# gleb-kov/wordpiece

Hardware: AMD Instinct MI355X
Metric: input MB/s tokenized (bert-base-cased vocab; offline stand-in: synthetic BERT-like vocab) (higher is better)
Workload: dtype int32

## Files before the change

### include/wordpiece_amd.h

```cpp
#ifndef WORDPIECE_AMD_H
#define WORDPIECE_AMD_H

#include <stddef.h>
#include <stdint.h>

#ifdef __cplusplus
extern "C" {
#endif

#define WP_OK 0
#define WP_ERR_EMPTY_WORD 1
#define WP_ERR_TOO_LARGE 2
#define WP_ERR_HIP 3
#define WP_ERR_NO_DEVICE 4
#define WP_ERR_IO 5
#define WP_ERR_ARG 6

typedef struct wp_vocab wp_vocab;

int wp_vocab_create(const char *const *lines, const size_t *line_bytes, size_t n_lines,
                    wp_vocab **out);
int wp_vocab_create_packed(const char *buf, const int64_t *offsets, int64_t n_lines,
                           wp_vocab **out);
int wp_vocab_from_file(const char *vocab_file, wp_vocab **out);
// ... 32 lines not shown
#define WP_TRUNC_ONLY_SECOND 2
typedef struct { int32_t max_len, cls_id, sep_id, pad_id, pairs, truncation, stride, unit; } wp_inputs_spec;
typedef struct { int32_t *input_ids, *token_type_ids, *lengths, *sample; uint32_t *offsets; } wp_inputs;
int wp_linear_encode_inputs(wp_vocab *v, const char *utf8, size_t nbytes, const int64_t *doc_off, size_t n_docs,
                            const wp_inputs_spec *spec, wp_inputs *out, size_t *n_out, size_t *n_samples);
int wp_linear_encode_inputs_device(wp_vocab *v, const void *d_utf8, size_t nbytes, const int64_t *d_doc_off, size_t n_docs,
                                   const wp_inputs_spec *spec, const wp_inputs *d_out, size_t capacity_rows,
                                   size_t *n_out, size_t *n_samples);

typedef struct { int32_t max_len, cls_id, sep_id, pad_id, mask_id, ignore_id, whole_word, reserved;
                 uint64_t select_q32, mask_q32, random_q32, seed, row_base; } wp_mask_spec;
int wp_word_ids(wp_vocab *v, const int32_t *input_ids, const int32_t *lengths, size_t n_rows, const wp_mask_spec *spec,
                int32_t **word_ids);
int wp_word_ids_device(wp_vocab *v, const int32_t *d_input_ids, const int32_t *d_lengths, size_t n_rows,
                       const wp_mask_spec *spec, int32_t *d_word_ids);
int wp_mlm_mask(wp_vocab *v, const int32_t *input_ids, const int32_t *lengths, size_t n_rows, const wp_mask_spec *spec,
                int32_t **masked, int32_t **labels, int32_t **word_ids);
int wp_mlm_mask_device(wp_vocab *v, const int32_t *d_input_ids, const int32_t *d_lengths, size_t n_rows,
                       const wp_mask_spec *spec, int32_t *d_masked, int32_t *d_labels, int32_t *d_word_ids);
typedef struct {
  int64_t n_rows;
  int64_t n_words;
  int64_t n_selected;
  int64_t n_selected_units;
  int64_t n_masked, n_random, n_kept;
  int32_t whole_word, reserved;
} wp_mask_stats;
int wp_get_mask_stats(const wp_vocab *v, wp_mask_stats *out);

typedef struct { int32_t max_len, cleanup, terminator, n_skip; int32_t skip_ids[8]; } wp_detok_spec;
int wp_detokenize(wp_vocab *v, const int32_t *ids, const int64_t *row_splits, const int32_t *lengths, size_t n_rows,
                  const wp_detok_spec *spec, char **text, int64_t **text_off, size_t *n_bytes);
int wp_detokenize_device(wp_vocab *v, const int32_t *d_ids, const int64_t *d_row_splits, const int32_t *d_lengths,
                         size_t n_rows, const wp_detok_spec *spec, const void **d_text, const int64_t **d_text_off,
                         size_t *n_bytes);
int64_t wp_detok_piece(const wp_vocab *v, int64_t id, int form, int cleanup, char *buf, size_t cap);
typedef struct { int64_t n_rows, n_cells, n_kept, n_skipped, n_dropped, n_bytes; } wp_detok_stats;
int wp_get_detok_stats(const wp_vocab *v, wp_detok_stats *out);

int wp_linear_encode_multi(wp_vocab *v, const char *utf8, size_t nbytes, const int *devices,
                           int n_devices, int32_t **ids, size_t *n_ids);

int wp_linear_encode_batch(wp_vocab *v, const char *const *texts, const size_t *nbytes, size_t n_texts,
                           int32_t **ids, size_t *n_ids);

typedef int (*wp_text_source)(void *user, size_t index, const char **utf8, size_t *nbytes);
typedef void (*wp_ids_sink)(void *user, size_t index, const int32_t *ids, size_t n_ids);
int wp_linear_encode_stream(wp_vocab *v, wp_text_source next, wp_ids_sink out, void *user);

int wp_reserve(wp_vocab *v, size_t nbytes);

int wp_trim(wp_vocab *v);

int wp_linear_encode_file(const char *text_file, const char *vocab_file, int32_t **ids,
                          size_t *n_ids);
int wp_linear_encode_external(const char *text_file, const char *vocab_file, const char *out_file,
                              size_t memory_limit);

int wp_fast_encode(wp_vocab *v, const char *utf8, size_t nbytes, int32_t **ids, size_t *n_ids);
int wp_fast_encode_device(wp_vocab *v, const void *d_utf8, size_t nbytes, const int32_t **d_ids,
                          size_t *n_ids);
int wp_fast_encode_file(const char *text_file, const char *vocab_file, int32_t **ids, size_t *n_ids);
int wp_fast_encode_external(const char *text_file, const char *vocab_file, const char *out_file,
                            size_t memory_limit);
int64_t wp_vocab_token_utf8(const wp_vocab *v, int64_t i, char *buf, size_t cap);

#define WP_OPT_FULL_DEPTH 1
#define WP_OPT_DEVICE 2
#define WP_OPT_KEEP_DEBUG 3
#define WP_OPT_STAGE_TIMING 4
#define WP_OPT_LCP_KASAI 5
#define WP_OPT_COVER_ANCHORS 7
#define WP_OPT_ARENA_GUARD 8
#define WP_OPT_DEVICES 9
#define WP_OPT_VOCAB_IN_S 10
#define WP_OPT_SPARSE_EMIT 11
#define WP_OPT_INDEXED_ROUND0 12
#define WP_OPT_SORT_BLANKS 13
#define WP_OPT_NORMALIZE 14
#define WP_NORM_CLEAN 1
#define WP_NORM_LOWER 2
#define WP_NORM_STRIP_ACCENTS 4
#define WP_NORM_BERT_UNCASED 7
int wp_set_option(wp_vocab *v, int option, int64_t value);

int wp_normalize_cp(int flags, uint32_t cp, uint32_t out[3]);
int wp_normalize_device(wp_vocab *v, const void *d_utf8, size_t nbytes, int flags, const void **d_out, size_t *out_bytes);
int wp_normalize(wp_vocab *v, const char *utf8, size_t nbytes, int flags, char **out, size_t *out_bytes);

typedef struct {
  int64_t n_bytes, n_text, n_total, alphabet, longest_token, n_ids;
  int32_t symbol_bits, symbols_per_key, rounds, sorted_depth, full_depth;
  int64_t radix_pass_elems;
  int32_t radix_passes;
  int64_t active_per_round[40];
  double ms_total, ms_decode, ms_sa, ms_lcp, ms_scan, ms_walk;
  double ms_radix_scatter;
  int64_t n_anchors;
  int32_t anchor_mode;
  double ms_h2d, ms_d2h;
  int64_t radix_digit_bytes;
  double ms_host_total;
  int32_t guard_zones;
  int32_t n_devices;
  int32_t vocab_in_s;
  int32_t reserved0;
  int64_t needed_after_round0;
  int32_t key_bits;
  int32_t staged_emit;
  int32_t rank_in_pass;
  int32_t trie_refine;
  int64_t arena_bytes;
  int32_t list_retries;
  int32_t hist_in_keys;
  int64_t radix_pass_bytes;
  int64_t round0_candidates;
  int32_t round0_keys_only;
  int32_t offsets_unit;
  int64_t round0_sorted;
  int64_t n_rows, rows_truncated;
  int32_t rows_route;
} wp_stats;
int wp_get_stats(const wp_vocab *v, wp_stats *out);
typedef struct {
  int32_t normalize;
  int64_t norm_bytes;
  double ms_normalize;
} wp_norm_stats;
int wp_get_norm_stats(const wp_vocab *v, wp_norm_stats *out);
typedef struct {
  int64_t n_wide_words;
  int64_t n_long_words;
  int32_t lean;
  int32_t max_anchor_gap;
} wp_walk_stats;
int wp_get_walk_stats(const wp_vocab *v, wp_walk_stats *out);
typedef struct {
  int64_t n_groups;
  int64_t n_entries;
  int64_t n_large_groups;
  int64_t n_large_entries;
  int64_t trie_nodes;
  int32_t sort_bits;
  int32_t key_lookup;
  int32_t symbol_bytes;
  int32_t reserved;
} wp_refine_stats;
int wp_get_refine_stats(const wp_vocab *v, wp_refine_stats *out);
typedef struct {
  int64_t n_samples, n_out;
  int64_t n_cut;
  int64_t n_windowed;
  int32_t pairs, truncation, stride, reserved;
} wp_inputs_stats;
int wp_get_inputs_stats(const wp_vocab *v, wp_inputs_stats *out);

int wp_linear_debug_fetch(const wp_vocab *v, int which, int32_t *out, size_t capacity,
                          size_t *n_out);

void wp_free(void *p);
const char *wp_last_error(void);
int wp_device_count(void);

#ifdef __cplusplus
}
#endif
#endif
```

### wordpiece_amd/__init__.py

```python
import ctypes as C
import os
import weakref

import numpy as np

_HERE = os.path.dirname(os.path.abspath(__file__))
LIB_PATH = os.environ.get("WP_LIB") or os.path.join(_HERE, "libwordpiece_amd.so")

WP_OPT_FULL_DEPTH, WP_OPT_DEVICE, WP_OPT_KEEP_DEBUG, WP_OPT_STAGE_TIMING, WP_OPT_LCP_KASAI = 1, 2, 3, 4, 5
WP_OPT_COVER_ANCHORS, WP_OPT_ARENA_GUARD, WP_OPT_DEVICES, WP_OPT_VOCAB_IN_S = 7, 8, 9, 10
WP_OPT_SPARSE_EMIT = 11
WP_OPT_INDEXED_ROUND0 = 12
WP_OPT_SORT_BLANKS = 13
WP_OPT_NORMALIZE = 14
WP_NORM_CLEAN, WP_NORM_LOWER, WP_NORM_STRIP_ACCENTS, WP_NORM_BERT_UNCASED = 1, 2, 4, 7
WP_OFFSETS_BYTES, WP_OFFSETS_CODE_POINTS = 0, 1
_OFFSET_UNITS = {"byte": WP_OFFSETS_BYTES, "char": WP_OFFSETS_CODE_POINTS}
WP_TRUNC_LONGEST_FIRST, WP_TRUNC_ONLY_FIRST, WP_TRUNC_ONLY_SECOND = 0, 1, 2
_TRUNCATIONS = {"longest_first": WP_TRUNC_LONGEST_FIRST, "only_first": WP_TRUNC_ONLY_FIRST,
                "only_second": WP_TRUNC_ONLY_SECOND}

ABI_SYMBOLS = [
    "wp_vocab_create", "wp_vocab_create_packed", "wp_vocab_from_file", "wp_vocab_destroy", "wp_vocab_size",
    "wp_vocab_unk_id", "wp_vocab_token_flags", "wp_vocab_token_len", "wp_linear_encode",
    "wp_linear_encode_device", "wp_linear_encode_file", "wp_linear_encode_external", "wp_set_option",
    "wp_get_stats", "wp_linear_debug_fetch", "wp_free", "wp_last_error", "wp_device_count",
    "wp_linear_encode_multi", "wp_reserve", "wp_fast_encode", "wp_fast_encode_device", "wp_fast_encode_file",
    "wp_fast_encode_external", "wp_vocab_token_utf8", "wp_trim", "wp_linear_encode_batch", "wp_linear_encode_stream",
    "wp_linear_encode_offsets", "wp_linear_encode_offsets_device",
    "wp_linear_encode_rows", "wp_linear_encode_rows_device", "wp_linear_encode_padded", "wp_linear_encode_padded_device",
    "wp_normalize_cp", "wp_normalize_device", "wp_normalize", "wp_get_norm_stats", "wp_get_walk_stats",
    "wp_get_refine_stats",
    "wp_linear_encode_inputs", "wp_linear_encode_inputs_device", "wp_get_inputs_stats",
    "wp_word_ids", "wp_word_ids_device", "wp_mlm_mask", "wp_mlm_mask_device", "wp_get_mask_stats",
    "wp_detokenize", "wp_detokenize_device", "wp_detok_piece", "wp_get_detok_stats",
]


class WordPieceError(RuntimeError):
    """Mirrors the std::runtime_error the reference throws (message = wp_last_error())."""


class Stats(C.Structure):
    _fields_ = [("n_bytes", C.c_int64), ("n_text", C.c_int64), ("n_total", C.c_int64), ("alphabet", C.c_int64),
                ("longest_token", C.c_int64), ("n_ids", C.c_int64),
                ("symbol_bits", C.c_int32), ("symbols_per_key", C.c_int32), ("rounds", C.c_int32),
                ("sorted_depth", C.c_int32), ("full_depth", C.c_int32),
                ("radix_pass_elems", C.c_int64), ("radix_passes", C.c_int32),
                ("active_per_round", C.c_int64 * 40),
                ("ms_total", C.c_double), ("ms_decode", C.c_double), ("ms_sa", C.c_double), ("ms_lcp", C.c_double),
                ("ms_scan", C.c_double), ("ms_walk", C.c_double), ("ms_radix_scatter", C.c_double),
                ("n_anchors", C.c_int64), ("anchor_mode", C.c_int32), ("ms_h2d", C.c_double), ("ms_d2h", C.c_double),
                ("radix_digit_bytes", C.c_int64), ("ms_host_total", C.c_double), ("guard_zones", C.c_int32),
                ("n_devices", C.c_int32), ("vocab_in_s", C.c_int32), ("reserved0", C.c_int32),
                ("needed_after_round0", C.c_int64), ("key_bits", C.c_int32), ("staged_emit", C.c_int32),
                ("rank_in_pass", C.c_int32), ("trie_refine", C.c_int32), ("arena_bytes", C.c_int64),
                ("list_retries", C.c_int32), ("hist_in_keys", C.c_int32), ("radix_pass_bytes", C.c_int64),
                ("round0_candidates", C.c_int64), ("round0_keys_only", C.c_int32), ("offsets_unit", C.c_int32),
                ("round0_sorted", C.c_int64), ("n_rows", C.c_int64), ("rows_truncated", C.c_int64),
                ("rows_route", C.c_int32)]

    def as_dict(self):
        d = {k: getattr(self, k) for k, _ in self._fields_ if k != "active_per_round"}
        d["active_per_round"] = [int(x) for x in self.active_per_round[:max(self.rounds, 0)]]
        return d


class NormStats(C.Structure):
    _fields_ = [("normalize", C.c_int32), ("norm_bytes", C.c_int64), ("ms_normalize", C.c_double)]


class WalkStats(C.Structure):
    _fields_ = [("n_wide_words", C.c_int64), ("n_long_words", C.c_int64), ("lean", C.c_int32),
                ("max_anchor_gap", C.c_int32)]


class RefineStats(C.Structure):
    _fields_ = [("n_groups", C.c_int64), ("n_entries", C.c_int64), ("n_large_groups", C.c_int64),
                ("n_large_entries", C.c_int64), ("trie_nodes", C.c_int64), ("sort_bits", C.c_int32),
                ("key_lookup", C.c_int32), ("symbol_bytes", C.c_int32), ("reserved", C.c_int32)]


class InputsSpec(C.Structure):
    _fields_ = [("max_len", C.c_int32), ("cls_id", C.c_int32), ("sep_id", C.c_int32), ("pad_id", C.c_int32),
                ("pairs", C.c_int32), ("truncation", C.c_int32), ("stride", C.c_int32), ("unit", C.c_int32)]


class Inputs(C.Structure):
    _fields_ = [("input_ids", C.c_void_p), ("token_type_ids", C.c_void_p), ("lengths", C.c_void_p), ("sample", C.c_void_p),
                ("offsets", C.c_void_p)]


class InputsStats(C.Structure):
    _fields_ = [("n_samples", C.c_int64), ("n_out", C.c_int64), ("n_cut", C.c_int64), ("n_windowed", C.c_int64),
                ("pairs", C.c_int32), ("truncation", C.c_int32), ("stride", C.c_int32), ("reserved", C.c_int32)]


class MaskSpec(C.Structure):
    _fields_ = [("max_len", C.c_int32), ("cls_id", C.c_int32), ("sep_id", C.c_int32), ("pad_id", C.c_int32),
                ("mask_id", C.c_int32), ("ignore_id", C.c_int32), ("whole_word", C.c_int32), ("reserved", C.c_int32),
                ("select_q32", C.c_uint64), ("mask_q32", C.c_uint64), ("random_q32", C.c_uint64), ("seed", C.c_uint64),
                ("row_base", C.c_uint64)]


class MaskStats(C.Structure):
    _fields_ = [("n_rows", C.c_int64), ("n_words", C.c_int64), ("n_selected", C.c_int64), ("n_selected_units", C.c_int64),
                ("n_masked", C.c_int64), ("n_random", C.c_int64), ("n_kept", C.c_int64), ("whole_word", C.c_int32),
                ("reserved", C.c_int32)]


class DetokSpec(C.Structure):
    _fields_ = [("max_len", C.c_int32), ("cleanup", C.c_int32), ("terminator", C.c_int32), ("n_skip", C.c_int32),
                ("skip_ids", C.c_int32 * 8)]


class DetokStats(C.Structure):
    _fields_ = [("n_rows", C.c_int64), ("n_cells", C.c_int64), ("n_kept", C.c_int64), ("n_skipped", C.c_int64),
                ("n_dropped", C.c_int64), ("n_bytes", C.c_int64)]


_TEXT_SOURCE = C.CFUNCTYPE(C.c_int, C.c_void_p, C.c_size_t, C.POINTER(C.c_void_p), C.POINTER(C.c_size_t))
_IDS_SINK = C.CFUNCTYPE(None, C.c_void_p, C.c_size_t, C.POINTER(C.c_int32), C.c_size_t)

_lib = None


def lib():
    global _lib
    if _lib is None:
        if not os.path.exists(LIB_PATH):
            raise WordPieceError("HIP extension missing: %s (run `python -m wordpiece_amd.build`)" % LIB_PATH)
        L = C.CDLL(LIB_PATH)
        vp, i32p = C.c_void_p, C.POINTER(C.c_int32)
        L.wp_vocab_create.argtypes = [C.POINTER(C.c_char_p), C.POINTER(C.c_size_t), C.c_size_t, C.POINTER(vp)]
        L.wp_vocab_create_packed.argtypes = [C.c_char_p, C.POINTER(C.c_int64), C.c_int64, C.POINTER(vp)]
        L.wp_vocab_from_file.argtypes = [C.c_char_p, C.POINTER(vp)]
        L.wp_vocab_destroy.argtypes = [vp]
        L.wp_vocab_destroy.restype = None
        L.wp_vocab_size.argtypes = [vp]
        L.wp_vocab_size.restype = C.c_int64
        L.wp_vocab_unk_id.argtypes = [vp]
        L.wp_vocab_unk_id.restype = C.c_int32
        L.wp_vocab_token_flags.argtypes = [vp, C.c_int64]
        L.wp_vocab_token_flags.restype = C.c_int32
        L.wp_vocab_token_len.argtypes = [vp, C.c_int64]
        L.wp_vocab_token_len.restype = C.c_int64
        L.wp_linear_encode.argtypes = [vp, C.c_char_p, C.c_size_t, C.POINTER(i32p), C.POINTER(C.c_size_t)]
        L.wp_linear_encode_device.argtypes = [vp, vp, C.c_size_t, C.POINTER(vp), C.POINTER(C.c_size_t)]
        u32p = C.POINTER(C.c_uint32)
        L.wp_linear_encode_offsets.argtypes = [vp, C.c_char_p, C.c_size_t, C.c_int, C.POINTER(i32p), C.POINTER(u32p),
                                               C.POINTER(C.c_size_t)]
        L.wp_linear_encode_offsets_device.argtypes = [vp, vp, C.c_size_t, C.c_int, C.POINTER(vp), C.POINTER(vp),
                                                      C.POINTER(C.c_size_t)]
        i64p = C.POINTER(C.c_int64)
        L.wp_linear_encode_rows.argtypes = [vp, C.c_char_p, C.c_size_t, i64p, C.c_size_t, C.c_int, C.POINTER(i32p),
                                            C.POINTER(i64p), C.POINTER(u32p), C.POINTER(C.c_size_t), C.POINTER(C.c_size_t)]
        L.wp_linear_encode_rows_device.argtypes = [vp, vp, C.c_size_t, vp, C.c_size_t, C.c_int, C.POINTER(vp), C.POINTER(vp),
                                                   C.POINTER(vp), C.POINTER(C.c_size_t), C.POINTER(C.c_size_t)]
        L.wp_linear_encode_padded.argtypes = [vp, C.c_char_p, C.c_size_t, i64p, C.c_size_t, C.c_int, C.c_int32, C.c_int32,
                                              C.c_int32, C.POINTER(i32p), C.POINTER(i32p), C.POINTER(C.c_size_t)]
        L.wp_linear_encode_padded_device.argtypes = [vp, vp, C.c_size_t, vp, C.c_size_t, C.c_int, C.c_int32, C.c_int32,
                                                     C.c_int32, vp, vp, C.c_size_t, C.POINTER(C.c_size_t)]
        L.wp_linear_encode_inputs.argtypes = [vp, C.c_char_p, C.c_size_t, i64p, C.c_size_t, C.POINTER(InputsSpec),
                                              C.POINTER(Inputs), C.POINTER(C.c_size_t), C.POINTER(C.c_size_t)]
        L.wp_linear_encode_inputs_device.argtypes = [vp, vp, C.c_size_t, vp, C.c_size_t, C.POINTER(InputsSpec),
                                                     C.POINTER(Inputs), C.c_size_t, C.POINTER(C.c_size_t),
                                                     C.POINTER(C.c_size_t)]
        L.wp_get_inputs_stats.argtypes = [vp, C.POINTER(InputsStats)]
        L.wp_word_ids.argtypes = [vp, i32p, i32p, C.c_size_t, C.POINTER(MaskSpec), C.POINTER(i32p)]
        L.wp_word_ids_device.argtypes = [vp, vp, vp, C.c_size_t, C.POINTER(MaskSpec), vp]
        L.wp_mlm_mask.argtypes = [vp, i32p, i32p, C.c_size_t, C.POINTER(MaskSpec), C.POINTER(i32p), C.POINTER(i32p),
                                  C.POINTER(i32p)]
        L.wp_mlm_mask_device.argtypes = [vp, vp, vp, C.c_size_t, C.POINTER(MaskSpec), vp, vp, vp]
        L.wp_get_mask_stats.argtypes = [vp, C.POINTER(MaskStats)]
        L.wp_detokenize.argtypes = [vp, i32p, C.POINTER(C.c_int64), i32p, C.c_size_t, C.POINTER(DetokSpec),
                                    C.POINTER(C.c_void_p), C.POINTER(C.POINTER(C.c_int64)), C.POINTER(C.c_size_t)]
        L.wp_detokenize_device.argtypes = [vp, vp, vp, vp, C.c_size_t, C.POINTER(DetokSpec), C.POINTER(C.c_void_p),
                                           C.POINTER(C.c_void_p), C.POINTER(C.c_size_t)]
        L.wp_detok_piece.argtypes = [vp, C.c_int64, C.c_int, C.c_int, C.c_char_p, C.c_size_t]
        L.wp_detok_piece.restype = C.c_int64
        L.wp_get_detok_stats.argtypes = [vp, C.POINTER(DetokStats)]
        L.wp_linear_encode_multi.argtypes = [vp, C.c_char_p, C.c_size_t, C.POINTER(C.c_int), C.c_int, C.POINTER(i32p),
                                             C.POINTER(C.c_size_t)]
        L.wp_reserve.argtypes = [vp, C.c_size_t]
        L.wp_linear_encode_stream.argtypes = [vp, _TEXT_SOURCE, _IDS_SINK, vp]
        L.wp_linear_encode_batch.argtypes = [vp, C.POINTER(C.c_char_p), C.POINTER(C.c_size_t), C.c_size_t, C.POINTER(i32p),
                                             C.POINTER(C.c_size_t)]
        L.wp_trim.argtypes = [vp]
        L.wp_fast_encode.argtypes = [vp, C.c_char_p, C.c_size_t, C.POINTER(i32p), C.POINTER(C.c_size_t)]
        L.wp_fast_encode_device.argtypes = [vp, vp, C.c_size_t, C.POINTER(vp), C.POINTER(C.c_size_t)]
        L.wp_fast_encode_file.argtypes = [C.c_char_p, C.c_char_p, C.POINTER(i32p), C.POINTER(C.c_size_t)]
        L.wp_fast_encode_external.argtypes = [C.c_char_p, C.c_char_p, C.c_char_p, C.c_size_t]
        L.wp_vocab_token_utf8.argtypes = [vp, C.c_int64, C.c_char_p, C.c_size_t]
        L.wp_vocab_token_utf8.restype = C.c_int64
        L.wp_linear_encode_file.argtypes = [C.c_char_p, C.c_char_p, C.POINTER(i32p), C.POINTER(C.c_size_t)]
        L.wp_linear_encode_external.argtypes = [C.c_char_p, C.c_char_p, C.c_char_p, C.c_size_t]
        L.wp_normalize_cp.argtypes = [C.c_int, C.c_uint32, C.POINTER(C.c_uint32)]
        L.wp_normalize_device.argtypes = [vp, vp, C.c_size_t, C.c_int, C.POINTER(vp), C.POINTER(C.c_size_t)]
        L.wp_normalize.argtypes = [vp, C.c_char_p, C.c_size_t, C.c_int, C.POINTER(vp), C.POINTER(C.c_size_t)]
        L.wp_set_option.argtypes = [vp, C.c_int, C.c_int64]
        L.wp_get_stats.argtypes = [vp, C.POINTER(Stats)]
        L.wp_get_norm_stats.argtypes = [vp, C.POINTER(NormStats)]
        L.wp_get_walk_stats.argtypes = [vp, C.POINTER(WalkStats)]
        L.wp_get_refine_stats.argtypes = [vp, C.POINTER(RefineStats)]
        L.wp_linear_debug_fetch.argtypes = [vp, C.c_int, i32p, C.c_size_t, C.POINTER(C.c_size_t)]
        L.wp_free.argtypes = [vp]
        L.wp_free.restype = None
        L.wp_last_error.restype = C.c_char_p
        L.wp_device_count.restype = C.c_int
        _lib = L
    return _lib


def _check(rc):
    if rc != 0:
        raise WordPieceError(lib().wp_last_error().decode("utf8", "replace"))


def _bytes(x):
    return bytes(x) if isinstance(x, (bytes, bytearray, memoryview)) else x.encode("utf8")


class Vocab:

    def __init__(self, lines=None, file=None, device=None, normalize=0):
        self._h = C.c_void_p()
        if file is not None:
            _check(lib().wp_vocab_from_file(_bytes(file), C.byref(self._h)))
        else:
            ls = [_bytes(w) for w in lines]
            off = np.zeros(len(ls) + 1, dtype=np.int64)
            if ls:
                off[1:] = np.cumsum([len(w) for w in ls])
            _check(lib().wp_vocab_create_packed(b"".join(ls), off.ctypes.data_as(C.POINTER(C.c_int64)), len(ls),
                                                C.byref(self._h)))
        self._device = None if device is None else int(device)
        if device is not None:
            self.set_option(WP_OPT_DEVICE, device)
        if normalize:
            self.set_option(WP_OPT_NORMALIZE, normalize)
        self._normalize = int(normalize)

    def __del__(self):
        if getattr(self, "_h", None) and _lib is not None:
            _lib.wp_vocab_destroy(self._h)
            self._h = None

    def __len__(self):
        return lib().wp_vocab_size(self._h)

    @property
    def unk_id(self):
        return lib().wp_vocab_unk_id(self._h)

    def token_flags(self, i):
        return lib().wp_vocab_token_flags(self._h, i)

    def token_len(self, i):
        return lib().wp_vocab_token_len(self._h, i)

    def set_option(self, opt, value):
        _check(lib().wp_set_option(self._h, opt, int(value)))
        if opt == WP_OPT_NORMALIZE:
            self._normalize = int(value)
        if opt == WP_OPT_DEVICE:
            self._device = int(value)

    def normalize(self, text, flags=None):
        b = _bytes(text)
        out = C.c_void_p()
        n = C.c_size_t()
        _check(lib().wp_normalize(self._h, b, len(b), self._normalize if flags is None else int(flags), C.byref(out), C.byref(n)))
        if n.value == 0:
            return b""
        try:
            return C.string_at(out, n.value)
        finally:
            lib().wp_free(out)

    def normalize_tensor(self, text, flags=None, copy=True):
        import torch
        if text.dtype != torch.uint8 or not text.is_cuda or not text.is_contiguous():
            raise WordPieceError("normalize_tensor needs a contiguous uint8 CUDA/HIP tensor")
        nbytes = text.numel()
        if text.data_ptr() % 4 != 0 or nbytes % 4 != 0:
            padded = torch.zeros((nbytes + 19) // 16 * 16, dtype=torch.uint8, device=text.device)
            padded[:nbytes] = text
            text = padded
        torch.cuda.current_stream(text.device).synchronize()
        d_out = C.c_void_p()
        n = C.c_size_t()
        _check(lib().wp_normalize_device(self._h, C.c_void_p(text.data_ptr()), nbytes,
                                         self._normalize if flags is None else int(flags), C.byref(d_out), C.byref(n)))
        if n.value == 0:
            return torch.zeros(0, dtype=torch.uint8, device=text.device)
        view = torch.as_tensor(DeviceIds(d_out.value, n.value, typestr="|u1"), device=text.device)
        return view.clone() if copy else view

    def stats(self):
        s = Stats()
        _check(lib().wp_get_stats(self._h, C.byref(s)))
        d = s.as_dict()
        ns = NormStats()
        _check(lib().wp_get_norm_stats(self._h, C.byref(ns)))
        d.update({k: getattr(ns, k) for k, _ in ns._fields_})
        return d

    def walk_stats(self):
        ws = WalkStats()
        _check(lib().wp_get_walk_stats(self._h, C.byref(ws)))
        return {k: int(getattr(ws, k)) for k, _ in ws._fields_}

    def refine_stats(self):
        rs = RefineStats()
        _check(lib().wp_get_refine_stats(self._h, C.byref(rs)))
        return {k: int(getattr(rs, k)) for k, _ in rs._fields_ if k != "reserved"}

    def encode(self, text):
        b = _bytes(text)
        ids = C.POINTER(C.c_int32)()
        n = C.c_size_t()
        _check(lib().wp_linear_encode(self._h, b, len(b), C.byref(ids), C.byref(n)))
        return _adopt_ids(ids, n.value)

    def encode_with_offsets(self, text, unit="byte"):
        b = _bytes(text)
        ids = C.POINTER(C.c_int32)()
        offs = C.POINTER(C.c_uint32)()
        n = C.c_size_t()
        _check(lib().wp_linear_encode_offsets(self._h, b, len(b), _offset_unit(unit), C.byref(ids), C.byref(offs),
                                              C.byref(n)))
        if n.value == 0:
            return np.zeros(0, dtype=np.int32), np.zeros((0, 2), dtype=np.uint32)
        return _adopt_ids(ids, n.value), _adopt_block(offs, (n.value, 2))

    def encode_device_with_offsets(self, d_ptr, nbytes, unit="byte"):
        d_ids = C.c_void_p()
        d_offs = C.c_void_p()
        n = C.c_size_t()
        _check(lib().wp_linear_encode_offsets_device(self._h, C.c_void_p(d_ptr), nbytes, _offset_unit(unit), C.byref(d_ids),
                                                     C.byref(d_offs), C.byref(n)))
        return d_ids.value, d_offs.value, n.value

    def encode_rows(self, docs=None, text=None, doc_offsets=None, offsets=None):
        b, off = _docs_arg(docs, text, doc_offsets)
        unit = -1 if offsets is None else _offset_unit(offsets)
        ids, splits, offs = C.POINTER(C.c_int32)(), C.POINTER(C.c_int64)(), C.POINTER(C.c_uint32)()
        n, rows = C.c_size_t(), C.c_size_t()
        _check(lib().wp_linear_encode_rows(self._h, b, len(b), _i64_ptr(off), 0 if off is None else len(off) - 1, unit,
                                           C.byref(ids), C.byref(splits), C.byref(offs), C.byref(n), C.byref(rows)))
        out = (_adopt_ids(ids, n.value), _adopt_block(splits, (rows.value + 1,)))
        if offsets is None:
            return out
        return out + (_adopt_block(offs, (n.value, 2)) if n.value else np.zeros((0, 2), dtype=np.uint32),)

    def encode_padded(self, docs=None, text=None, doc_offsets=None, max_len=128, cls_id=None, sep_id=None, pad_id=0):
        b, off = _docs_arg(docs, text, doc_offsets)
        ids, lens = C.POINTER(C.c_int32)(), C.POINTER(C.c_int32)()
        rows = C.c_size_t()
        _check(lib().wp_linear_encode_padded(self._h, b, len(b), _i64_ptr(off), 0 if off is None else len(off) - 1,
                                             int(max_len), _special(cls_id), _special(sep_id), int(pad_id), C.byref(ids),
                                             C.byref(lens), C.byref(rows)))
        if rows.value == 0:
            return np.zeros((0, int(max_len)), dtype=np.int32), np.zeros(0, dtype=np.int32)
        return _adopt_block(ids, (rows.value, int(max_len))), _adopt_block(lens, (rows.value,))

    def _rows_tensor_args(self, text, doc_offsets):
        import torch
        if text.dtype != torch.uint8 or not text.is_cuda or not text.is_contiguous():
            raise WordPieceError("a documents call on tensors needs a contiguous uint8 CUDA/HIP text tensor")
        nbytes = text.numel()
        if text.data_ptr() % 4 != 0 or nbytes % 4 != 0:
            padded = torch.zeros((nbytes + 19) // 16 * 16, dtype=torch.uint8, device=text.device)
            padded[:nbytes] = text
            text = padded
        if doc_offsets is not None:
            if doc_offsets.dtype != torch.int64 or doc_offsets.device != text.device or doc_offsets.dim() != 1 or \
                    doc_offsets.numel() < 1:
                raise WordPieceError("doc_offsets must be a 1-d int64 tensor on the text's device")
            doc_offsets = doc_offsets.contiguous()
        torch.cuda.current_stream(text.device).synchronize()
        return text, nbytes, doc_offsets

    def encode_rows_tensor(self, text, doc_offsets=None, offsets=None, copy=True):
        import torch
        text, nbytes, doc_offsets = self._rows_tensor_args(text, doc_offsets)
        unit = -1 if offsets is None else _offset_unit(offsets)
        d_ids, d_splits, d_offs = C.c_void_p(), C.c_void_p(), C.c_void_p()
        n, rows = C.c_size_t(), C.c_size_t()
        _check(lib().wp_linear_encode_rows_device(
            self._h, C.c_void_p(text.data_ptr()), nbytes, None if doc_offsets is None else C.c_void_p(doc_offsets.data_ptr()),
            0 if doc_offsets is None else doc_offsets.numel() - 1, unit, C.byref(d_ids), C.byref(d_splits), C.byref(d_offs),
            C.byref(n), C.byref(rows)))
        dev = text.device
        ids = torch.as_tensor(DeviceIds(d_ids.value, n.value), device=dev) if n.value else \
            torch.zeros(0, dtype=torch.int32, device=dev)
        splits = torch.as_tensor(DeviceIds(d_splits.value, rows.value + 1, typestr="<i8"), device=dev)
        out = (ids, splits)
        if offsets is not None:
# ... 579 lines not shown
```

### wordpiece_amd/csrc/context.h

```cpp
#pragma once
#include <array>
#include <cstring>
#include <memory>
#include <mutex>
#include <string>
#include <vector>

#include "../../include/wordpiece_amd.h"
#include "code.h"
#include "decode.h"
#include "detok.h"
#include "radix_sort.h"
#include "scanline.h"
#include "suffix_array.h"
#include "vocab.h"

namespace wp {

static thread_local std::string g_last_error;

struct EnvOptions {
  bool arena_guard;
  bool vocab_in_s;
  bool sparse_emit;
// ... 44 lines not shown
__global__ __launch_bounds__(kBlock) void guard_check_kernel(const char *base, const unsigned long long *offs, int count,
                                                             uint32_t *bad) {
  const int z = blockIdx.x;
  if (z >= count) return;
  const uint32_t *g = reinterpret_cast<const uint32_t *>(base + offs[z]);
  const bool broken = threadIdx.x < kGuardBytes / 4 && g[threadIdx.x] != kGuardWord;
  if (__syncthreads_or(broken) && threadIdx.x == 0) {
    atomicAdd(&bad[0], 1u);
    atomicMin(&bad[1], static_cast<uint32_t>(z) + 1u);
  }
}

struct Arena {
  DeviceBuffer *buf;
  size_t off = 0, planned = 0;
  bool planning = true, guard = false;
  std::vector<unsigned long long> zones;
  explicit Arena(DeviceBuffer *b, bool g = false) : buf(b), guard(g) {}
  template <typename T>
  T *take(size_t count) {
    size_t bytes = (count * sizeof(T) + 255) & ~static_cast<size_t>(255);
    size_t o = off;
    off += bytes;
    if (guard) {
      if (!planning) zones.push_back(off);
      off += kGuardBytes;
    }
    if (planning) return nullptr;
    if (off > planned) throw std::logic_error("arena: the allocation sequence differs from the planned one");
    return reinterpret_cast<T *>(static_cast<char *>(buf->p) + o);
  }
  void commit() {
    buf->ensure(off + (guard ? 8 * 512 : 0));
    planned = off;
    off = 0;
    planning = false;
  }
  unsigned long long *zone_table() const {
    return reinterpret_cast<unsigned long long *>(static_cast<char *>(buf->p) + ((off + 255) & ~static_cast<size_t>(255)));
  }
  void arm(hipStream_t st) {
    if (!guard || zones.empty()) return;
    if (zones.size() > 500) throw std::logic_error("arena guard: too many allocations");
    WP_HIP(hipMemcpyAsync(zone_table(), zones.data(), zones.size() * sizeof(unsigned long long), hipMemcpyHostToDevice, st));
    WP_HIP(hipStreamSynchronize(st));
    hipLaunchKernelGGL(guard_fill_kernel, dim3(zones.size()), dim3(kBlock), 0, st, static_cast<char *>(buf->p), zone_table(),
                       static_cast<int>(zones.size()));
  }
  void check(hipStream_t st, uint32_t *bad) const {
    if (!guard || zones.empty()) return;
    hipLaunchKernelGGL(guard_check_kernel, dim3(zones.size()), dim3(kBlock), 0, st, static_cast<const char *>(buf->p),
                       zone_table(), static_cast<int>(zones.size()), bad);
  }
};

static int bit_length(uint64_t v) {
  int b = 0;
  while (v) {
    b++;
    v >>= 1;
  }
  return b;
}

constexpr int kScalars = 56;
constexpr int kScalarCps = 0;
constexpr int kScalarAlphabet = 1;
constexpr int kScalarInvalid = 2;
constexpr int kScalarList = 4;
constexpr int kScalarListEntries = kScalarList + 0;
constexpr int kScalarListGroups = kScalarList + 1;
constexpr int kScalarListLargeGroups = kScalarList + 2;
constexpr int kScalarListLargeEntries = kScalarList + 3;
constexpr int kScalarListWanted = 8;
constexpr int kScalarIds = 9;
constexpr int kScalarAnchors = 10;
constexpr int kScalarAnchorGap = 11;
constexpr int kScalarLongWords = 12;
constexpr int kScalarWideWords = 13;
constexpr int kScalarCps64 = 14;
constexpr int kScalarGuard = 16;
constexpr int kScalarGuardBad = kScalarGuard + 0;
constexpr int kScalarGuardFirst = kScalarGuard + 1;
constexpr int kScalarFree18 = 18;
constexpr int kScalarAlphaWord0 = 20;
constexpr int kScalarRows = 21, kScalarRowsBad = 22, kScalarRowsCut = 23;
constexpr int kScalarCand = 24;
constexpr int kScalarKept = 25;
constexpr int kScalarSrcRows = 26;
constexpr int kScalarInCut = 27, kScalarInRows = 28, kScalarInWindowed = 30;
constexpr int kScalarFree31 = 31;
constexpr int kScalarMask = 32;
constexpr int kScalarDetokLast = 44, kScalarDetokBad = 46;
constexpr int kScalarFree47 = 47;
constexpr int kScalarDetok = 48;
constexpr int kScalarNormBytes = kScalarCps;
constexpr int kScalarNormCps = kScalarAlphabet;
constexpr int kScalarNormSrcCps = kScalarListEntries;
constexpr int kScalarNormBytes64 = kScalarCps64;

struct ScalarRange {
  int first, words;
};
constexpr ScalarRange kScalarLayout[] = {
    {kScalarCps, 1},         {kScalarAlphabet, 1},   {kScalarInvalid, 2},         {kScalarListEntries, 1},
    {kScalarListGroups, 1},  {kScalarListLargeGroups, 1}, {kScalarListLargeEntries, 1}, {kScalarListWanted, 1},
    {kScalarIds, 1},         {kScalarAnchors, 1},    {kScalarAnchorGap, 1},       {kScalarLongWords, 1},
    {kScalarWideWords, 1},   {kScalarCps64, 2},      {kScalarGuardBad, 1},        {kScalarGuardFirst, 1},
    {kScalarFree18, 2},      {kScalarAlphaWord0, 1}, {kScalarRows, 1},            {kScalarRowsBad, 1},
    {kScalarRowsCut, 1},     {kScalarCand, 1},       {kScalarKept, 1},            {kScalarSrcRows, 1},
    {kScalarInCut, 1},       {kScalarInRows, 2},     {kScalarInWindowed, 1},      {kScalarFree31, 1},
    {kScalarMask, 12},       {kScalarDetokLast, 2},  {kScalarDetokBad, 1},        {kScalarFree47, 1},
    {kScalarDetok, 8}};
constexpr int scalar_end(int slot) {
  for (const ScalarRange &r : kScalarLayout) {
    if (slot < r.first + r.words) return r.first + r.words;
  }
  return kScalars;
}
constexpr bool scalar_layout_ok() {
  int at = 0;
  for (const ScalarRange &r : kScalarLayout) {
    if (r.first != at || r.words < 1 || (r.words % 2 == 0 && r.first % 2 != 0)) return false;
    at += r.words;
  }
  return at == kScalars;
}
static_assert(scalar_layout_ok(), "the scalar table must cover d_scalars word by word, 64-bit slots on even words");
static_assert(kScalarList % 2 == 0 && kScalarListLargeGroups % 2 == 0, "both halves of the list block are also read as 64-bit words");

struct RowsCall {
  const long long *d_doc_off = nullptr;
  size_t n_docs = 0;
  int unit = -1;
  size_t capacity = SIZE_MAX;
  size_t n_rows = 0;
  const long long *d_starts = nullptr;
  const long long *d_row_splits = nullptr;
  uint32_t *d_line_cnt = nullptr;
};

enum SideEvent { kEvFork, kEvJoin, kEvScalars, kEvKeysFree, kEvPartition, kEvTrieNodes, kEvLargeSorted, kEvKeysBuilt, kEvCandCount,
                 kEvSpine, kEvKept, kSideEvents };
enum TimingMark { kMarkStart, kMarkCounted, kMarkSymbols, kMarkSorted, kMarkLcp, kMarkScanned, kMarkWalked, kMarkNormStart,
                  kTimingMarks, kMarkNormEnd = kMarkStart };

struct Context {
  int device = 0;
  hipStream_t stream = nullptr;
  hipStream_t stream2 = nullptr;
  hipStream_t stream3 = nullptr;
  hipEvent_t evs[kSideEvents] = {};
  uint32_t *d_stream = nullptr, *d_elig_start = nullptr, *d_elig_info = nullptr, *d_soft = nullptr;
  uint32_t *d_vocab_word_idx = nullptr, *d_vocab_word_bits = nullptr;
  uint8_t *d_cls_bmp = nullptr;
  uint32_t *d_lt_chain_len = nullptr, *d_lt_chain_off = nullptr, *d_lt_child_begin = nullptr, *d_lt_child_cp = nullptr,
           *d_lt_child_node = nullptr, *d_elig_node = nullptr, *d_elig_subtree = nullptr;
  int32_t *d_elig_id = nullptr, *d_tok_len = nullptr;
  uint8_t *d_tok_class = nullptr;
  DetokRec *d_detok_rec = nullptr;
  uint8_t *d_detok_pool = nullptr;
  size_t detok_pool_bytes = 0;
  unsigned long long *d_trie_key = nullptr;
  uint32_t *d_trie_child = nullptr;
  int32_t *d_trie_id = nullptr;
  DeviceBuffer text_buf, a_buf, b_buf, fmt_buf;
  DeviceBuffer text_buf2, ids_stage[2];
  DeviceBuffer rows_in, rows_out, pad_buf;
  DeviceBuffer inputs_buf;
  DeviceBuffer detok_in, detok_aux, detok_out;
  uint16_t *d_norm_index = nullptr;
  uint32_t *d_norm_pages = nullptr, *d_norm_pool = nullptr;
  DeviceBuffer norm_buf, norm_aux, norm_map;
  hipStream_t up_stream = nullptr, down_stream = nullptr;
  hipEvent_t pipe_ev[4] = {};
  uint32_t *d_used = nullptr, *d_lut = nullptr, *d_scan_tmp = nullptr;
  uint32_t *d_scalars = nullptr;
  uint8_t *d_code = nullptr;
  size_t list_hint = 0;
  SymbolCode code_cache;
  bool code_cached = false;
  uint32_t code_alphabet = 0;
  int code_bits = 0, code_lo = 0, code_uses = 0;
  double code_blank_share = 0.0;
  uint8_t *h_code = nullptr;
  uint32_t *d_symhist = nullptr;
  uint32_t *h_scalars = nullptr;
  RadixStats rstats;
  hipEvent_t ev[kTimingMarks] = {};
  const int32_t *d_ids = nullptr;
  const uint32_t *d_offs = nullptr;
  struct {
    const void *sym = nullptr;
    int sym_bytes = 0;
    const uint32_t *sa = nullptr, *cps = nullptr;
    const RankEntry *rank = nullptr;
    const int32_t *lcp = nullptr;
    const uint8_t *cls = nullptr;
    StepTable steps{};
    int32_t *best_scratch = nullptr;
    size_t n = 0, n_text = 0;
  } dbg;
  std::array<DeviceBuffer *, 17> buffers() {
    return {&text_buf, &a_buf,    &b_buf,   &fmt_buf,    &text_buf2, &ids_stage[0], &ids_stage[1], &rows_in,   &rows_out,
            &pad_buf,  &inputs_buf, &norm_buf, &norm_aux, &norm_map, &detok_in,     &detok_aux,    &detok_out};
  }
  Context() = default;
  Context(const Context &) = delete;
  Context &operator=(const Context &) = delete;
  ~Context();
};

struct DeviceGuard {
  int prev = -1;
  DeviceGuard() {
    if (hipGetDevice(&prev) != hipSuccess) prev = -1;
  }
  ~DeviceGuard() {
    if (prev >= 0) (void)hipSetDevice(prev);
  }
  DeviceGuard(const DeviceGuard &) = delete;
  DeviceGuard &operator=(const DeviceGuard &) = delete;
};

#ifdef WP_DEBUG_BOUNDS
static void take_oob(int first, int count, unsigned int *oob) {
  WP_HIP(hipMemcpyFromSymbol(oob, HIP_SYMBOL(g_wp_oob), count * sizeof(unsigned int), first * sizeof(unsigned int)));
  bool any = false;
  for (int i = 0; i < count; i++) any = any || oob[i] != 0;
  if (!any) return;
  const unsigned int zero[kBoundSites] = {};
  WP_HIP(hipMemcpyToSymbol(HIP_SYMBOL(g_wp_oob), zero, count * sizeof(unsigned int), first * sizeof(unsigned int)));
}
#endif

}

using namespace wp;

struct EncodeStats : wp_stats {
  int32_t normalize;
  int64_t norm_bytes;
  double ms_normalize;
  wp_walk_stats walk;
  wp_refine_stats refine;
  wp_inputs_stats inputs;
  int32_t inputs_call;
  wp_mask_stats mask;
  int32_t mask_call;
  wp_detok_stats detok;
  int32_t detok_call;
};

struct wp_vocab {
  HostVocab hv;
  std::unique_ptr<Context> ctx;
  std::vector<std::unique_ptr<Context>> multi;
  int device = -1;
  bool full_depth = false, keep_debug = false, stage_timing = false, lcp_kasai = false, cover_anchors = false;
  bool arena_guard = false;
  bool sparse_emit = false;
  bool vocab_in_s = false;
  bool indexed_round0 = false;
  bool sort_blanks = false;
  int normalize = 0;
  int n_devices = 1;
  EncodeStats stats{};
  ~wp_vocab();
};

namespace wp {

template <typename... T>
static void free_dev(T *&...p) {
  (((p ? (void)hipFree(p) : (void)0), p = nullptr), ...);
}

static void free_vocab_tables(Context *c) {
  free_dev(c->d_stream, c->d_elig_start, c->d_elig_info, c->d_soft, c->d_elig_id, c->d_tok_len, c->d_tok_class, c->d_detok_rec, c->d_detok_pool, c->d_trie_key,
           c->d_trie_child, c->d_trie_id, c->d_vocab_word_idx, c->d_vocab_word_bits, c->d_cls_bmp, c->d_lt_chain_len,
           c->d_lt_chain_off, c->d_lt_child_begin, c->d_lt_child_cp, c->d_lt_child_node, c->d_elig_node, c->d_elig_subtree);
}

template <size_t N>
static void destroy_events(hipEvent_t (&events)[N]) {
  for (auto &e : events) {
    if (e) (void)hipEventDestroy(e);
    e = nullptr;
  }
}

static void destroy_context(Context *c) {
  if (!c) return;
  bool owns = c->stream || c->stream2 || c->stream3 || c->d_used || c->d_lut || c->d_scan_tmp || c->d_scalars || c->d_code ||
              c->d_symhist || c->h_scalars || c->h_code || c->d_stream;
  for (DeviceBuffer *b : c->buffers()) owns = owns || b->p;
  if (!owns) return;
  DeviceGuard keep;
  (void)hipSetDevice(c->device);
  free_vocab_tables(c);
  free_dev(c->d_used, c->d_lut, c->d_scan_tmp, c->d_scalars, c->d_code, c->d_symhist, c->d_norm_index, c->d_norm_pages, c->d_norm_pool);
  if (c->h_scalars) (void)hipHostFree(c->h_scalars);
  if (c->h_code) (void)hipHostFree(c->h_code);
  c->h_scalars = nullptr;
  c->h_code = nullptr;
  for (DeviceBuffer *b : c->buffers()) b->release();
  destroy_events(c->pipe_ev);
  destroy_events(c->ev);
  destroy_events(c->evs);
  for (hipStream_t *s : {&c->up_stream, &c->down_stream, &c->stream3, &c->stream2, &c->stream}) {
    if (*s) (void)hipStreamDestroy(*s);
    *s = nullptr;
  }
}
Context::~Context() { destroy_context(this); }

template <typename T>
static T *upload(const std::vector<T> &v, hipStream_t st) {
  T *d = nullptr;
  WP_HIP(hipMalloc(&d, std::max<size_t>(v.size(), 1) * sizeof(T)));
  if (!v.empty()) WP_HIP(hipMemcpyAsync(d, v.data(), v.size() * sizeof(T), hipMemcpyHostToDevice, st));
  return d;
}

static constexpr size_t kPoolArenaBytes = size_t(256) << 20;
static constexpr size_t kPoolContexts = 4;
static std::mutex g_pool_mu;
static std::vector<std::unique_ptr<Context>> &context_pool() {
  static auto *pool = new std::vector<std::unique_ptr<Context>>();
  return *pool;
}

static void release_arenas(Context *c) {
  for (DeviceBuffer *b : c->buffers()) b->release();
  c->d_ids = nullptr;
  c->d_offs = nullptr;
  c->dbg = {};
}

static void park_context(std::unique_ptr<Context> c) {
  if (!c) return;
  const bool no_pool = EnvOptions::get().no_pool;
  DeviceGuard keep;
  (void)hipSetDevice(c->device);
  if (!no_pool && hipStreamSynchronize(c->stream) == hipSuccess && hipStreamSynchronize(c->stream2) == hipSuccess &&
      hipStreamSynchronize(c->stream3) == hipSuccess) {
    free_vocab_tables(c.get());
// ... 112 lines not shown
```

### wordpiece_amd/csrc/encoder.hip

```cpp
#include <fcntl.h>
#include <sys/mman.h>
#include <sys/stat.h>
#include <unistd.h>

#include <atomic>
#include <chrono>
#include <cstring>
#include <fstream>
#include <functional>
#include <future>
#include <memory>
#include <mutex>
#include <thread>
#include <unordered_map>
#include <vector>

#include "../../include/wordpiece_amd.h"
#include "context.h"
#include "detok.h"
#include "fast_path.h"
#include "format.h"
#include "inputs.h"
#include "linear_path.h"
#include "mask.h"
// ... 51 lines not shown
  }
  try {
  std::unique_ptr<wp_vocab> v(new wp_vocab());
  if (const char *e = getenv("WP_DEVICES")) {
    v->n_devices = std::strcmp(e, "all") == 0 ? -1 : std::max(1, atoi(e));
  }
  std::string err = v->hv.build(lines);
  if (!err.empty()) {
    g_last_error = err;
    return WP_ERR_EMPTY_WORD;
  }
  *out = v.release();
  return WP_OK;
  } catch (const std::exception &e) {
    g_last_error = e.what();
    return WP_ERR_ARG;
  } catch (...) {
    g_last_error = "unknown exception while building the vocabulary";
    return WP_ERR_ARG;
  }
}

extern "C" {

int wp_vocab_create(const char *const *lines, const size_t *line_bytes, size_t n_lines, wp_vocab **out) {
  std::vector<std::pair<const char *, size_t>> ls;
  ls.reserve(n_lines);
  for (size_t i = 0; i < n_lines; i++) ls.emplace_back(lines[i], line_bytes[i]);
  return vocab_from_lines(ls, out);
}

int wp_vocab_create_packed(const char *buf, const int64_t *offsets, int64_t n_lines, wp_vocab **out) {
  std::vector<std::pair<const char *, size_t>> ls;
  ls.reserve(static_cast<size_t>(n_lines));
  for (int64_t i = 0; i < n_lines; i++) ls.emplace_back(buf + offsets[i], static_cast<size_t>(offsets[i + 1] - offsets[i]));
  return vocab_from_lines(ls, out);
}

int wp_vocab_from_file(const char *vocab_file, wp_vocab **out) {
  std::ifstream fin(vocab_file);
  std::vector<std::string> words;
  std::string w;
  while (std::getline(fin, w)) words.push_back(w);
  std::vector<std::pair<const char *, size_t>> ls;
  for (auto &s : words) ls.emplace_back(s.data(), s.size());
  return vocab_from_lines(ls, out);
}

void wp_vocab_destroy(wp_vocab *v) {
  if (!v) return;
  try {
    delete v;
  } catch (...) {
  }
}
int64_t wp_vocab_size(const wp_vocab *v) { return static_cast<int64_t>(v->hv.tokens.size()); }
int32_t wp_vocab_unk_id(const wp_vocab *v) { return v->hv.unk_id; }
int32_t wp_vocab_token_flags(const wp_vocab *v, int64_t i) {
  return token_flags(v->hv.tokens[static_cast<size_t>(i)]);
}
int64_t wp_vocab_token_len(const wp_vocab *v, int64_t i) {
  return static_cast<int64_t>(v->hv.tokens[static_cast<size_t>(i)].word.size());
}

int wp_set_option(wp_vocab *v, int option, int64_t value) {
  switch (option) {
    case WP_OPT_FULL_DEPTH: v->full_depth = value != 0; return WP_OK;
    case WP_OPT_DEVICE:
      if (v->ctx) {
        g_last_error = "device already bound";
        return WP_ERR_ARG;
      }
      v->device = static_cast<int>(value);
      return WP_OK;
    case WP_OPT_KEEP_DEBUG: v->keep_debug = value != 0; return WP_OK;
    case WP_OPT_STAGE_TIMING: v->stage_timing = value != 0; return WP_OK;
    case WP_OPT_LCP_KASAI: v->lcp_kasai = value != 0; return WP_OK;
    case WP_OPT_COVER_ANCHORS: v->cover_anchors = value != 0; return WP_OK;
    case WP_OPT_ARENA_GUARD: v->arena_guard = value != 0; return WP_OK;
    case WP_OPT_VOCAB_IN_S: v->vocab_in_s = value != 0; return WP_OK;
    case WP_OPT_SPARSE_EMIT: v->sparse_emit = value != 0; return WP_OK;
    case WP_OPT_INDEXED_ROUND0: v->indexed_round0 = value != 0; return WP_OK;
    case WP_OPT_SORT_BLANKS: v->sort_blanks = value != 0; return WP_OK;
    case WP_OPT_NORMALIZE:
      if (!known_norm_flags(value)) {
        g_last_error = "WP_OPT_NORMALIZE: unknown flag bits (WP_NORM_CLEAN | WP_NORM_LOWER | WP_NORM_STRIP_ACCENTS)";
        return WP_ERR_ARG;
      }
      v->normalize = static_cast<int>(value);
      return WP_OK;
    case WP_OPT_DEVICES: v->n_devices = value < 0 ? -1 : static_cast<int>(std::max<int64_t>(value, 1)); return WP_OK;
  }
  g_last_error = "unknown option";
  return WP_ERR_ARG;
}

int wp_normalize_cp(int flags, uint32_t cp, uint32_t out[3]) {
  if (!known_norm_flags(flags) || cp >= 0x110000u || (cp >= 0xd800u && cp < 0xe000u)) return -1;
  uint32_t o[3] = {0, 0, 0};
  const int n = norm_cp(host_norm_tables(), flags, cp, o);
  for (int i = 0; i < n; i++) out[i] = o[i];
  return n;
}

int wp_normalize_device(wp_vocab *v, const void *d_utf8, size_t nbytes, int flags, const void **d_out, size_t *out_bytes) {
  return guarded([&] {
    *d_out = nullptr;
    *out_bytes = 0;
    if (!known_norm_flags(flags)) throw std::invalid_argument("normalize: unknown flag bits");
    if (nbytes == 0) return;
    check_device_text(d_utf8);
    Context *c = get_context(v);
    NormResult r;
    normalize_on_device(c, static_cast<const uint8_t *>(d_utf8), nbytes, flags, false, false, r);
    WP_HIP(hipStreamSynchronize(c->stream));
    *d_out = r.nbytes ? r.text : nullptr;
    *out_bytes = r.nbytes;
  });
}

int wp_get_stats(const wp_vocab *v, wp_stats *out) {
  *out = v->stats;
  return WP_OK;
}

int wp_get_norm_stats(const wp_vocab *v, wp_norm_stats *out) {
  out->normalize = v->stats.normalize;
  out->norm_bytes = v->stats.norm_bytes;
  out->ms_normalize = v->stats.ms_normalize;
  return WP_OK;
}

int wp_get_walk_stats(const wp_vocab *v, wp_walk_stats *out) {
  *out = v->stats.walk;
  return WP_OK;
}

int wp_get_refine_stats(const wp_vocab *v, wp_refine_stats *out) {
  *out = v->stats.refine;
  return WP_OK;
}

int wp_get_inputs_stats(const wp_vocab *v, wp_inputs_stats *out) {
  *out = v->stats.inputs;
  if (!v->stats.inputs_call) out->n_out = -1;
  return WP_OK;
}

int wp_linear_encode_device(wp_vocab *v, const void *d_utf8, size_t nbytes, const int32_t **d_ids, size_t *n_ids) {
  return guarded([&] {
    check_device_text(d_utf8);
    size_t n = 0;
    Context *c = get_context(v);
    encode_on_device(v, c, static_cast<const uint8_t *>(d_utf8), nbytes, &n, v->stats);
    v->stats.n_devices = 1;
    *d_ids = n ? c->d_ids : nullptr;
    *n_ids = n;
  });
}

}

namespace {
struct PinnedPool {
  std::mutex mu;
  std::unordered_map<void *, size_t> owned;
  std::vector<std::pair<size_t, void *>> pooled;
  static constexpr size_t kMaxPooledBlocks = 4;
  static constexpr size_t kMaxPooledBytes = size_t(6) << 30;
  void *take(size_t bytes) {
    {
      std::lock_guard<std::mutex> g(mu);
      size_t best = pooled.size();
      for (size_t i = 0; i < pooled.size(); i++) {
        if (pooled[i].first >= bytes && (best == pooled.size() || pooled[i].first < pooled[best].first)) best = i;
      }
      if (best != pooled.size()) {
        void *p = pooled[best].second;
        pooled.erase(pooled.begin() + static_cast<long>(best));
        return p;
      }
    }
    void *p = nullptr;
    const size_t want = bytes + bytes / 8 + 4096;
    WP_HIP(hipHostMalloc(&p, want));
    std::lock_guard<std::mutex> g(mu);
    owned[p] = want;
    return p;
  }
  bool give_back(void *p) {
    size_t cap = 0;
    {
      std::lock_guard<std::mutex> g(mu);
      auto it = owned.find(p);
      if (it == owned.end()) return false;
      cap = it->second;
      size_t bytes = cap;
      for (auto &b : pooled) bytes += b.first;
      if (pooled.size() < kMaxPooledBlocks && bytes <= kMaxPooledBytes) {
        pooled.emplace_back(cap, p);
        return true;
      }
      owned.erase(it);
    }
    (void)hipHostFree(p);
    return true;
  }
  void trim() {
    std::vector<std::pair<size_t, void *>> drop;
    {
      std::lock_guard<std::mutex> g(mu);
      drop.swap(pooled);
      for (auto &b : drop) owned.erase(b.second);
    }
    for (auto &b : drop) (void)hipHostFree(b.second);
  }
};
PinnedPool &id_pool() {
  static PinnedPool *pool = new PinnedPool();
  return *pool;
}
struct PinnedBlock {
// ... 1346 lines not shown
  }
  DeviceBuffer *tb[2] = {&c->text_buf, &c->text_buf2};
  const int device = c->device;
  std::atomic<long long> up_us{0};
  auto upload = [&](const char *text, size_t len, int slot) -> std::string {
    try {
      if (len == 0) return "";
      const auto t_up = wp_clock::now();
      WP_HIP(hipSetDevice(device));
      upload_text(*tb[slot], c->up_stream, text, len);
      WP_HIP(hipStreamSynchronize(c->up_stream));
      up_us += static_cast<long long>(ms_since(t_up) * 1e3);
      return "";
    } catch (const std::exception &e) {
      return e.what()[0] ? e.what() : "upload failed";
    }
  };
  EncodeStats total{};
  const char *cur_text = nullptr, *next_text = nullptr;
  size_t cur_len = 0, next_len = 0;
  bool have = next(0, &cur_text, &cur_len);
  if (have) {
    tb[0]->ensure(text_room(cur_len));
    const std::string err = upload(cur_text, cur_len, 0);
    if (!err.empty()) throw HipError(err);
  }
  std::unique_ptr<PinnedBlock> in_flight;
  size_t in_flight_n = 0, in_flight_i = 0;
  int in_flight_slot = 0;
  for (size_t i = 0; have; i++) {
    const int slot = static_cast<int>(i & 1);
    const bool more = next(i + 1, &next_text, &next_len);
    std::future<std::string> next_up;
    if (more) {
      tb[slot ^ 1]->ensure(text_room(next_len));
      next_up = std::async(std::launch::async, upload, next_text, next_len, slot ^ 1);
    }
    struct Wait {
      std::future<std::string> &f;
      ~Wait() {
        if (f.valid()) f.wait();
      }
    } wait_up{next_up};
    size_t n = 0;
    EncodeStats st{};
    if (cur_len) encode_on_device(v, c, static_cast<const uint8_t *>(tb[slot]->p), cur_len, &n, st);
    std::unique_ptr<PinnedBlock> blk(new PinnedBlock(std::max<size_t>(n, 1) * sizeof(int32_t)));
    if (n) {
      c->ids_stage[slot].ensure(n * sizeof(int32_t));
      WP_HIP(hipMemcpyAsync(c->ids_stage[slot].p, c->d_ids, n * sizeof(int32_t), hipMemcpyDeviceToDevice, c->stream));
      WP_HIP(hipEventRecord(c->pipe_ev[slot], c->stream));
      WP_HIP(hipStreamWaitEvent(c->down_stream, c->pipe_ev[slot], 0));
      WP_HIP(hipMemcpyAsync(blk->p, c->ids_stage[slot].p, n * sizeof(int32_t), hipMemcpyDeviceToHost, c->down_stream));
      WP_HIP(hipEventRecord(c->pipe_ev[2 + slot], c->down_stream));
    }
    if (in_flight) {
      if (in_flight_n) WP_HIP(hipEventSynchronize(c->pipe_ev[2 + in_flight_slot]));
      deliver(in_flight_i, *in_flight, in_flight_n);
    }
    in_flight = std::move(blk);
    in_flight_n = n;
    in_flight_i = i;
    in_flight_slot = slot;
    total.n_bytes += st.n_bytes;
    total.n_text += st.n_text;
    total.n_total += st.n_total;
    total.n_ids += st.n_ids;
    total.ms_total += st.ms_total;
    total.normalize = std::max(total.normalize, st.normalize);
    total.norm_bytes += st.norm_bytes;
    total.ms_normalize += st.ms_normalize;
    total.walk.n_wide_words += st.walk.n_wide_words;
    total.walk.n_long_words += st.walk.n_long_words;
    total.walk.max_anchor_gap = std::max(total.walk.max_anchor_gap, st.walk.max_anchor_gap);
    if (i == 0) total.walk.lean = st.walk.lean;
    {
      const wp_refine_stats sum = total.refine;
      if (i == 0) total.refine = st.refine;
      total.refine.n_groups = sum.n_groups + st.refine.n_groups;
      total.refine.n_entries = sum.n_entries + st.refine.n_entries;
      total.refine.n_large_groups = sum.n_large_groups + st.refine.n_large_groups;
      total.refine.n_large_entries = sum.n_large_entries + st.refine.n_large_entries;
    }
    total.rounds = std::max(total.rounds, st.rounds);
    if (next_up.valid()) {
      const std::string err = next_up.get();
      if (!err.empty()) throw HipError(err);
    }
    have = more;
    cur_text = next_text;
    cur_len = next_len;
  }
  if (in_flight) {
    if (in_flight_n) WP_HIP(hipEventSynchronize(c->pipe_ev[2 + in_flight_slot]));
    deliver(in_flight_i, *in_flight, in_flight_n);
  }
  v->stats = total;
  v->stats.n_devices = 1;
  v->stats.ms_h2d = static_cast<double>(up_us.load()) / 1e3;
  v->stats.ms_host_total = ms_since(t_all);
}
}

extern "C" {

int wp_linear_encode_batch(wp_vocab *v, const char *const *texts, const size_t *nbytes, size_t n_texts, int32_t **ids,
                           size_t *n_ids) {
  return guarded([&] {
    for (size_t i = 0; i < n_texts; i++) {
      ids[i] = nullptr;
      n_ids[i] = 0;
    }
    std::vector<void *> got(n_texts, nullptr);
    try {
      encode_pipeline(
          v,
          [&](size_t i, const char **t, size_t *len) {
            if (i >= n_texts) return false;
            *t = texts[i];
            *len = nbytes[i];
            return true;
          },
          [&](size_t i, PinnedBlock &blk, size_t n) {
            n_ids[i] = n;
            if (n) got[i] = blk.release();
          });
    } catch (...) {
      for (void *p : got) {
        if (p) id_pool().give_back(p);
      }
      for (size_t i = 0; i < n_texts; i++) n_ids[i] = 0;
      throw;
    }
    for (size_t i = 0; i < n_texts; i++) ids[i] = static_cast<int32_t *>(got[i]);
  });
}

int wp_linear_encode_stream(wp_vocab *v, wp_text_source next, wp_ids_sink out, void *user) {
  return guarded([&] {
    if (!next || !out) throw std::invalid_argument("wp_linear_encode_stream: null callback");
    encode_pipeline(
        v, [&](size_t i, const char **t, size_t *len) { return next(user, i, t, len) != 0; },
        [&](size_t i, PinnedBlock &blk, size_t n) { out(user, i, n ? static_cast<const int32_t *>(blk.p) : nullptr, n); });
  });
}

int wp_trim(wp_vocab *v) {
  return guarded([&] {
    auto drop = [](Context *c) {
      if (!c) return;
      WP_HIP(hipSetDevice(c->device));
      WP_HIP(hipStreamSynchronize(c->stream));
      WP_HIP(hipStreamSynchronize(c->stream2));
      release_arenas(c);
    };
    if (v) {
      drop(v->ctx.get());
      for (auto &c : v->multi) drop(c.get());
    }
    {
      std::lock_guard<std::mutex> g(g_pool_mu);
      for (auto &c : context_pool()) drop(c.get());
    }
    id_pool().trim();
  });
}
// ... 294 lines not shown
```

### wordpiece_amd/csrc/linear_path.h

```cpp
#pragma once
#include <functional>

#include "context.h"
#include "local_sort.h"
#include "prune.h"
#include "trie.h"
#include "offsets.h"
#include "normalize.h"
#include "rows.h"
#include "walk.h"

namespace wp {

struct ListOverflow {
  size_t wanted;
};

__global__ void needed_list_clamp_kernel(uint32_t *__restrict__ totals, uint32_t cap, uint32_t *__restrict__ wanted) {
  if (totals[0] > cap) {
    *wanted = totals[0];
    totals[0] = 0;
    totals[1] = 0;
  }
}

constexpr double kBlankDropMinShare = 1.0 / 16;

#ifdef WP_DEBUG_BOUNDS
__device__ unsigned int g_wp_sorted_sig[6];
__global__ __launch_bounds__(kBlock) void sorted_check_kernel(const uint32_t *__restrict__ sorted, size_t n_sorted,
                                                              const uint32_t *__restrict__ unsorted, size_t n,
                                                              const uint8_t *__restrict__ cls, size_t n_text,
                                                              const uint32_t *__restrict__ blank_bits) {
  __shared__ uint32_t acc[7];
  if (threadIdx.x < 7) acc[threadIdx.x] = 0u;
  __syncthreads();
  uint32_t bad = 0, cnt[2] = {0, 0}, sum[2] = {0, 0}, x[2] = {0, 0};
  const size_t first = static_cast<size_t>(blockIdx.x) * kBlock + threadIdx.x, stride = static_cast<size_t>(gridDim.x) * kBlock;
  for (size_t i = first; i < n_sorted; i += stride) {
    const uint32_t k = sorted[i];
    if (i + 1 < n_sorted && k > sorted[i + 1]) bad++;
    if (blank_bits && key_is_blank(blank_bits, k)) bad++;
    cnt[0]++;
    sum[0] += k;
    x[0] ^= k;
  }
  for (size_t i = first; i < n; i += stride) {
    if (blank_bits && i < n_text && (cls[i] & kClsSpace)) continue;
    const uint32_t k = unsorted[i];
    cnt[1]++;
    sum[1] += k;
    x[1] ^= k;
  }
  if (bad) atomicAdd(&acc[6], bad);
  for (int s = 0; s < 2; s++) {
    if (cnt[s]) {
      atomicAdd(&acc[3 * s], cnt[s]);
      atomicAdd(&acc[3 * s + 1], sum[s]);
      atomicXor(&acc[3 * s + 2], x[s]);
    }
  }
  __syncthreads();
  if (threadIdx.x < 6 && acc[threadIdx.x]) {
    if (threadIdx.x % 3 == 2) {
      atomicXor(&g_wp_sorted_sig[threadIdx.x], acc[threadIdx.x]);
    } else {
      atomicAdd(&g_wp_sorted_sig[threadIdx.x], acc[threadIdx.x]);
    }
  }
  if (threadIdx.x == 6 && acc[6]) atomicAdd(&g_wp_oob[kSiteSortOrder], acc[6]);
}
__global__ void sorted_check_close_kernel() {
  bool same = true;
  for (int j = 0; j < 3; j++) same = same && g_wp_sorted_sig[j] == g_wp_sorted_sig[3 + j];
  wp_in_bounds(same, kSiteSortOrder);
  for (int j = 0; j < 6; j++) g_wp_sorted_sig[j] = 0u;
}
#endif

template <typename SymT>
struct LinearPath {
  const wp_vocab *v;
  Context *c;
  EncodeStats &S;
  Arena &ar, &aa;
  const uint8_t *d_text;
  size_t nbytes;
  const uint32_t *d_tile_prefix;
  size_t n_text, n;
  uint32_t *d_cps;
  uint8_t *d_cls;
  int bits;
  bool text_only;
  int offs_unit;
  RowsCall *rows;
  const NormMap *nmap;

  hipStream_t st, st2;
  const HostVocab &hv;
  bool full, prune, use_trie, key_lookup, keys_only, window_store, use_digit_bytes, staged_possible, sparse_emit;
  bool wide_ran = false;
  uint32_t need_depth;
  int M, P, P_cap, bucket_shift, bucket_shift_all, key_shift, key_shift_all, hb_n, win_mid;
  unsigned sl_tiles, sl_groups, nbuckets, nbuckets_all, nkbuckets, nkbuckets_all;
  size_t radix_words, emit_tiles, walk_blocks, claim_size, list_cap;

  SymT *d_sym = nullptr, *d_vsym = nullptr;
  Key0 *KA = nullptr, *KB = nullptr;
  uint32_t *VA = nullptr, *VB = nullptr;
  uint32_t *X0 = nullptr, *X1 = nullptr;
  uint8_t *DG0 = nullptr, *DG1 = nullptr;
  RankEntry *d_rank = nullptr;
  uint32_t *d_node_of_slot = nullptr;
  int32_t *d_lcp = nullptr;
  uint32_t *d_sa = nullptr, *d_gdepth = nullptr;
  RankEntry *d_hd_n = nullptr;
  int32_t *d_emit = nullptr, *d_dbg_best = nullptr;
  uint32_t *d_anchors = nullptr, *d_anchor_cnt = nullptr, *d_anchor_tmp = nullptr, *d_emit_cnt = nullptr, *d_emit_tmp = nullptr,
           *d_blk_cnt = nullptr, *d_blk_off = nullptr, *d_tile_scratch = nullptr;
  uint32_t *AS0 = nullptr, *AS1 = nullptr, *AG = nullptr, *AD0 = nullptr, *AD1 = nullptr, *LA = nullptr, *LB = nullptr, *d_tdep = nullptr;
  uint64_t *LK0 = nullptr, *LK1 = nullptr, *LK2 = nullptr;
  uint32_t *LV0 = nullptr, *LV1 = nullptr, *LPOS = nullptr;
  uint32_t *d_ghead = nullptr, *d_gneed0 = nullptr, *d_gneed1 = nullptr, *d_lg_head = nullptr, *d_lg_off = nullptr;
  RerankAgg *d_agg = nullptr, *d_chunk_agg = nullptr;
  uint32_t *d_claim = nullptr, *d_claim_need = nullptr, *d_gclaim = nullptr, *d_gfirst = nullptr, *d_gdep = nullptr, *d_gnode = nullptr,
           *d_gdone = nullptr, *d_rng_lo = nullptr, *d_rng_hi = nullptr, *d_child_sym = nullptr, *d_radix_tmp = nullptr,
           *d_radix_tmp2 = nullptr;
  uint8_t *d_rng_long = nullptr;
  uint32_t *d_mslot0 = nullptr, *d_mslot1 = nullptr, *d_midx0 = nullptr, *d_midx1 = nullptr, *d_minfo = nullptr, *d_tile_mlo = nullptr;
  int32_t *d_mid = nullptr, *d_rf = nullptr, *d_rb = nullptr, *d_cover_f = nullptr, *d_cover_b = nullptr;
  int32_t *d_tmin_f = nullptr, *d_tmin_b = nullptr, *d_gmin_f = nullptr, *d_gmin_b = nullptr, *d_pval_p = nullptr, *d_pval_s = nullptr;
  uint32_t *d_ps0 = nullptr, *d_ps1 = nullptr, *d_pv0 = nullptr, *d_pv1 = nullptr, *d_bidx = nullptr;
  int2 *d_bfast = nullptr, *d_bfast_all = nullptr;
  uint32_t *d_bidx_all = nullptr;
  uint32_t *d_gend = nullptr, *d_kstart = nullptr, *d_kbidx = nullptr, *d_kbidx_all = nullptr;
  int32_t *d_kval_p = nullptr, *d_kval_s = nullptr;
  int2 *d_kbfast = nullptr, *d_kbfast_all = nullptr;
  unsigned long long *d_cand_table = nullptr;
  uint32_t *d_cand_filter = nullptr, *d_cand_lo = nullptr, *d_cand_hi = nullptr, *d_gcand = nullptr;
  uint32_t *d_cand_bcnt = nullptr, *d_cand_boff = nullptr, *d_cand_scan = nullptr;
  int cand_bits = 0;
  uint32_t *d_blank_bits = nullptr;
  uint2 *d_ospill = nullptr, *d_cspan = nullptr, *d_offs = nullptr;
  uint32_t *d_byte_of = nullptr;
  long long *d_line_starts = nullptr, *d_row_splits = nullptr;
  uint32_t *d_row_base = nullptr;

  SymbolCode code;
  DevCode dcode{};
  DigitBytes db;
  RadixPlan sort_plan;
  bool hist_in_keys = false;
  bool drop_blanks = false;
  size_t n_sorted = 0;
  int cur = 0, rounds = 1;
  Key0 *keys = nullptr, *other_keys = nullptr;
  uint32_t *vals = nullptr, *other_vals = nullptr, *slots = nullptr, *other_slots = nullptr, *adep = nullptr, *other_dep = nullptr;
  uint32_t *avals = nullptr, *spare_vals = nullptr;
  bool classified = false, anchors_queued = false;
  size_t n_act = 0, n_large = 0, n_large_groups = 0, n_groups = 0;
  StepTable steps{}, steps_all{};
  StepTable ksteps{}, ksteps_all{};
  CandSet cand{};
  CandRuns cand_runs{};
  size_t n_cand = 0;

  LinearPath(const wp_vocab *v_, Context *c_, EncodeStats &S_, Arena &ar_, Arena &aa_, const uint8_t *text, size_t nb,
             const uint32_t *tile_prefix, size_t n_text_, size_t n_, uint32_t *cps, uint8_t *cls, int bits_, bool text_only_,
             int offs_unit_, RowsCall *rows_ = nullptr, const NormMap *nmap_ = nullptr)
      : v(v_), c(c_), S(S_), ar(ar_), aa(aa_), d_text(text), nbytes(nb), d_tile_prefix(tile_prefix), n_text(n_text_), n(n_),
        d_cps(cps), d_cls(cls), bits(bits_), text_only(text_only_), offs_unit(offs_unit_), rows(rows_), nmap(nmap_), st(c_->stream), st2(c_->stream2),
        hv(v_->hv) {
    full = v->full_depth || hv.n_dup_eligible > 0 || v->lcp_kasai;
    need_depth = static_cast<uint32_t>(std::min<int64_t>(hv.longest + 1, 0x7fffffff));
    M = static_cast<int>(hv.elig_id.size());
    prune = !full && (M > 0 || text_only);
    use_trie = text_only && !full && M > 0;
    key_lookup = use_trie && !v->keep_debug && kKeyBits <= 32;
    keys_only = key_lookup && !v->indexed_round0 && sizeof(SymT) == 1;
    sl_tiles = cdiv(n, kSlTile);
    sl_groups = cdiv(sl_tiles, kSlGroup);
    P = kStepsPerMark * M + 1;
    P_cap = P + 2 * M + 2;
    const int bucket_bits = std::min(kStepBucketBitsMax, std::max(kStepBucketBits, bit_length(4 * static_cast<size_t>(P))));
    bucket_shift = std::max(0, bit_length(n) - bucket_bits);
    nbuckets = static_cast<unsigned>(((n - 1) >> bucket_shift) + 1);
    bucket_shift_all = std::max(0, bit_length(n) - kStepBucketBits);
    nbuckets_all = static_cast<unsigned>(((n - 1) >> bucket_shift_all) + 1);
    const int kb = std::min(kKeyBits, std::max(1, bit_length(n - 1) - bucket_shift));
    const int kb_all = std::min(kKeyBits, std::max(1, bit_length(n - 1) - bucket_shift_all));
    key_shift = kKeyBits - kb;
    key_shift_all = kKeyBits - kb_all;
    nkbuckets = 1u << kb;
    nkbuckets_all = 1u << kb_all;
    radix_words = std::max(radix_tmp_words<uint64_t>(n), radix_tmp_words<uint32_t>(std::max<size_t>(n, static_cast<size_t>(P_cap))));
    emit_tiles = cdiv(std::max<size_t>(n_text, 1), kScanTile);
    walk_blocks = cdiv(std::max<size_t>(n_text, 1), kBlock);
    sparse_emit = v->sparse_emit || EnvOptions::get().sparse_emit;
    staged_possible = !sparse_emit && !v->cover_anchors && hv.soft.empty();
    use_digit_bytes = n > kRadixSmallN;
    claim_size = 1024;
    while (claim_size < 2 * static_cast<size_t>(std::max(M, 1))) claim_size *= 2;
    cand_bits = bit_length(claim_size - 1);
    hb_n = bit_length(n - 1);
    window_store = n >= (1u << 22);
    win_mid = hb_n - kWinBits <= kRadixBits ? hb_n : kWinBits + (hb_n - kWinBits + 1) / 2;
    if (!prune) {
      list_cap = n;
    } else {
      const size_t guess = c->list_hint ? c->list_hint : n / 8;
      list_cap = std::min(n, guess + guess / 4 + 65536);
    }
    S.symbol_bits = bits;
    S.full_depth = full;
    S.trie_refine = use_trie ? 1 : 0;
    S.key_bits = kKeyBits;
    S.round0_keys_only = keys_only ? 1 : 0;
    S.round0_candidates = keys_only ? 0 : -1;
    n_sorted = n;
    S.round0_sorted = static_cast<int64_t>(n);
  }

  void fork() {
    WP_HIP(hipEventRecord(c->evs[kEvFork], st));
    WP_HIP(hipStreamWaitEvent(st2, c->evs[kEvFork], 0));
  }
  void join() {
    WP_HIP(hipEventRecord(c->evs[kEvJoin], st2));
    WP_HIP(hipStreamWaitEvent(st, c->evs[kEvJoin], 0));
  }

  void plan() {
    const bool ref = !text_only;
    const bool want_lcp = ref || v->keep_debug;
    const size_t lc = list_cap, lg = lc / 2 + static_cast<size_t>(M) + 8;
    const size_t rr_tiles_l = cdiv(lc, kRrTile);
    const size_t rtiles = cdiv(std::max<size_t>(n_text, 1), kReachTile);
    for (int pass = 0; pass < 2; pass++) {
      d_sym = ar.take<SymT>(n + 16);
      KA = ar.take<Key0>(n + 16);
      KB = ar.take<Key0>(n + 16);
      VA = ar.take<uint32_t>(n + 16);
      VB = ar.take<uint32_t>(n + 16);
      X0 = ar.take<uint32_t>(n + 16);
      X1 = ar.take<uint32_t>(n + 16);
      DG0 = use_digit_bytes ? ar.take<uint8_t>(n + 64) : nullptr;
      DG1 = use_digit_bytes ? ar.take<uint8_t>(n + 64) : nullptr;
      d_rank = ar.take<RankEntry>(n);
      d_node_of_slot = use_trie ? ar.take<uint32_t>(n) : nullptr;
      d_lcp = want_lcp ? ar.take<int32_t>(n) : nullptr;
      d_sa = (v->keep_debug || v->lcp_kasai) ? ar.take<uint32_t>(n) : nullptr;
      d_gdepth = (use_trie && !want_lcp) ? nullptr : ar.take<uint32_t>(n);
      d_hd_n = (want_lcp || !prune) ? ar.take<RankEntry>(n + 16) : nullptr;
      d_dbg_best = v->keep_debug ? ar.take<int32_t>(2 * n) : nullptr;
      d_emit = ar.take<int32_t>(n_text + 1);
      d_anchors = ar.take<uint32_t>(n_text + 1);
      d_anchor_cnt = ar.take<uint32_t>(emit_tiles + 1);
      d_anchor_tmp = ar.take<uint32_t>(cdiv(emit_tiles, kScanTile) + 8);
      d_emit_cnt = ar.take<uint32_t>(emit_tiles + 1);
      d_emit_tmp = ar.take<uint32_t>(cdiv(walk_blocks, kScanTile) + 8);
      d_blk_cnt = ar.take<uint32_t>(walk_blocks + 2);
      d_blk_off = ar.take<uint32_t>(walk_blocks + 2);
      d_tile_scratch = ar.take<uint32_t>(5 * (rtiles + 2) + 4 * (n_text / kMaxAnchorGap + 4));
      AS0 = ar.take<uint32_t>(lc);
      AS1 = ar.take<uint32_t>(lc);
      AG = ar.take<uint32_t>(lc);
      AD0 = ar.take<uint32_t>(lc);
      AD1 = ar.take<uint32_t>(lc);
      LA = ar.take<uint32_t>(lc);
      LB = ar.take<uint32_t>(lc);
      d_tdep = ar.take<uint32_t>(lc + 2);
      LK0 = ar.take<uint64_t>(lc + 2);
      LK1 = ar.take<uint64_t>(lc + 2);
      LK2 = ar.take<uint64_t>(lc + 2);
      LV0 = ar.take<uint32_t>(lc);
      LV1 = ar.take<uint32_t>(lc);
      LPOS = ar.take<uint32_t>(lc + 16);
      d_ghead = ar.take<uint32_t>(lg);
      d_gneed0 = use_trie ? nullptr : ar.take<uint32_t>(lg);
      d_gneed1 = use_trie ? nullptr : ar.take<uint32_t>(lg);
      d_lg_head = ar.take<uint32_t>(lc / kLsMaxGroup + 4);
      d_lg_off = ar.take<uint32_t>(lc / kLsMaxGroup + 4);
      d_agg = ar.take<RerankAgg>(rr_tiles_l + 1);
      d_chunk_agg = ar.take<RerankAgg>(cdiv(rr_tiles_l, kRrChunk) + 1);
      d_radix_tmp = ar.take<uint32_t>(radix_words);
      d_radix_tmp2 = use_trie ? ar.take<uint32_t>(std::max(radix_tmp_words<uint64_t>(lc), keys_only ? radix_tmp_words<uint32_t>(n) : 0))
                              : nullptr;
      d_claim = ar.take<uint32_t>(claim_size);
      d_claim_need = ar.take<uint32_t>(claim_size);
      d_gclaim = ar.take<uint32_t>(M + 4);
      d_gfirst = ar.take<uint32_t>(M + 4);
      d_gdep = ar.take<uint32_t>(M + 4);
      d_gnode = ar.take<uint32_t>(M + 4);
      d_gdone = ar.take<uint32_t>(M + 4);
      d_rng_lo = ar.take<uint32_t>(M + 1);
      d_rng_hi = ar.take<uint32_t>(M + 1);
      d_rng_long = ar.take<uint8_t>(M + 1);
      d_vsym = use_trie ? ar.take<SymT>(hv.stream.size() + 16) : nullptr;
      d_child_sym = use_trie ? ar.take<uint32_t>(hv.lt_child_cp.size() + 1) : nullptr;
      d_mslot0 = ar.take<uint32_t>(M + 1);
      d_mslot1 = ar.take<uint32_t>(M + 1);
      d_midx0 = ar.take<uint32_t>(M + 1);
      d_midx1 = ar.take<uint32_t>(M + 1);
      d_mid = ar.take<int32_t>(M + 1);
      d_minfo = ar.take<uint32_t>(M + 1);
      d_rf = ar.take<int32_t>(M + 1);
      d_cover_f = ar.take<int32_t>(2 * static_cast<size_t>(M) + 2);
      d_cover_b = ar.take<int32_t>(2 * static_cast<size_t>(M) + 2);
      d_rb = ar.take<int32_t>(M + 1);
      d_tile_mlo = ref ? ar.take<uint32_t>(sl_tiles + 2) : nullptr;
      d_tmin_f = ref ? ar.take<int32_t>(sl_tiles + 1) : nullptr;
      d_tmin_b = ref ? ar.take<int32_t>(sl_tiles + 1) : nullptr;
      d_gmin_f = ref ? ar.take<int32_t>(sl_groups + 1) : nullptr;
      d_gmin_b = ref ? ar.take<int32_t>(sl_groups + 1) : nullptr;
      d_ps0 = ar.take<uint32_t>(P_cap + 1);
      d_ps1 = ar.take<uint32_t>(P_cap + 1);
      d_pv0 = ar.take<uint32_t>(P_cap + 1);
      d_pv1 = ar.take<uint32_t>(P_cap + 1);
      d_pval_p = ar.take<int32_t>(P_cap + 1);
      d_pval_s = ar.take<int32_t>(P_cap + 1);
      d_bidx = ar.take<uint32_t>(static_cast<size_t>(nbuckets) + 2);
      d_bfast = ar.take<int2>(static_cast<size_t>(nbuckets) + 1);
      d_bidx_all = bucket_shift_all != bucket_shift ? ar.take<uint32_t>(static_cast<size_t>(nbuckets_all) + 2) : nullptr;
      d_bfast_all = bucket_shift_all != bucket_shift ? ar.take<int2>(static_cast<size_t>(nbuckets_all) + 1) : nullptr;
      d_gend = key_lookup ? ar.take<uint32_t>(M + 4) : nullptr;
      d_kstart = key_lookup ? ar.take<uint32_t>(P_cap + 1) : nullptr;
      d_kval_p = key_lookup ? ar.take<int32_t>(P_cap + 1) : nullptr;
      d_kval_s = key_lookup ? ar.take<int32_t>(P_cap + 1) : nullptr;
      d_kbidx = key_lookup ? ar.take<uint32_t>(static_cast<size_t>(nkbuckets) + 2) : nullptr;
      d_kbfast = key_lookup ? ar.take<int2>(static_cast<size_t>(nkbuckets) + 1) : nullptr;
      d_kbidx_all = (key_lookup && key_shift_all != key_shift) ? ar.take<uint32_t>(static_cast<size_t>(nkbuckets_all) + 2) : nullptr;
      d_kbfast_all = (key_lookup && key_shift_all != key_shift) ? ar.take<int2>(static_cast<size_t>(nkbuckets_all) + 1) : nullptr;
      d_cand_table = keys_only ? ar.take<unsigned long long>(claim_size) : nullptr;
      d_cand_filter = keys_only ? ar.take<uint32_t>(kCandFilterWords) : nullptr;
      d_cand_lo = keys_only ? ar.take<uint32_t>(claim_size) : nullptr;
      d_cand_hi = keys_only ? ar.take<uint32_t>(claim_size) : nullptr;
      d_gcand = keys_only ? ar.take<uint32_t>(M + 4) : nullptr;
      d_cand_bcnt = keys_only ? ar.take<uint32_t>(cdiv(n, kKeyTile) + 2) : nullptr;
      d_cand_boff = keys_only ? ar.take<uint32_t>(cdiv(n, kKeyTile) + 2) : nullptr;
      d_cand_scan = keys_only ? ar.take<uint32_t>(cdiv(cdiv(n, kKeyTile), kScanTile) + 8) : nullptr;
      d_blank_bits = keys_only ? ar.take<uint32_t>(kBlankWords) : nullptr;
      const bool offs = offs_unit >= 0;
      d_ospill = offs ? ar.take<uint2>(n_text + 16) : nullptr;
      d_cspan = offs ? ar.take<uint2>(n_text + 16) : nullptr;
      d_offs = offs ? ar.take<uint2>(n_text + 1) : nullptr;
      d_byte_of = ((offs_unit == WP_OFFSETS_BYTES && !nmap) || rows) ? ar.take<uint32_t>(n_text + 1) : nullptr;
      d_line_starts = (rows && (!rows->d_doc_off || nmap)) ? ar.take<long long>(rows->n_rows + 1) : nullptr;
      d_row_splits = rows ? ar.take<long long>(rows->n_rows + 1) : nullptr;
      d_row_base = (rows && rows->unit >= 0) ? ar.take<uint32_t>(rows->n_rows + 1) : nullptr;
      if (pass == 0) ar.commit();
    }
    ar.arm(st);
  }

  void launch_anchors(hipStream_t as) {
    anchors_queued = true;
    const unsigned atiles = cdiv(n_text, kAnchorTile);
    if (!staged_possible) WP_HIP(hipMemsetAsync(d_emit, 0x80, n_text * sizeof(int32_t), as));
    hipLaunchKernelGGL(anchor_count_kernel, dim3(atiles), dim3(kBlock), 0, as, d_cls, static_cast<const uint8_t *>(nullptr),
                       n_text, d_anchor_cnt);
    device_exclusive_scan(d_anchor_cnt, d_anchor_cnt, atiles, d_anchor_tmp, c->d_scalars + kScalarAnchors, as);
    hipLaunchKernelGGL(anchor_write_kernel, dim3(atiles), dim3(kBlock), 0, as, d_cls, static_cast<const uint8_t *>(nullptr),
                       n_text, d_anchor_cnt, d_anchors);
    hipLaunchKernelGGL(anchor_gap_kernel, dim3(std::min<size_t>(atiles, 1024)), dim3(kBlock), 0, as, d_anchors,
                       c->d_scalars + kScalarAnchors, n_text, d_cls, hv.soft.empty() ? 1 : 0, c->d_scalars + kScalarAnchorGap);
  }

  void symbols_and_keys() {
    const int lo_bits = sizeof(SymT) == 1 ? 0 : std::max(0, bits - 8);
    constexpr int kCodeReuse = 64;
    const bool reuse_code = c->code_cached && c->code_alphabet == static_cast<uint32_t>(S.alphabet) && c->code_bits == bits &&
                            c->code_lo == lo_bits && c->code_uses < kCodeReuse;
    if (!reuse_code) WP_HIP(hipMemsetAsync(c->d_symhist, 0, sizeof(uint32_t) * 256, st));
    constexpr uint32_t kBlankCpRuns[3][2] = {{0x09, 7}, {0x20, 2}, {kSpaceToken, 2}};
    uint32_t h_blank_lut[3][7] = {};
    hipLaunchKernelGGL(HIP_KERNEL_NAME(decode_write_kernel<SymT>), dim3(cdiv(nbytes, kDecTile)), dim3(kBlock), 0, st, d_text,
                       nbytes, d_tile_prefix, c->d_lut, d_sym, d_cls, d_cps, c->d_cls_bmp, c->d_soft,
                       static_cast<int>(hv.soft.size()), reuse_code ? nullptr : c->d_symhist, lo_bits);
    hipLaunchKernelGGL(HIP_KERNEL_NAME(map_vocab_symbols_kernel<SymT>), dim3(cdiv(n - n_text, kBlock)), dim3(kBlock), 0, st,
                       c->d_stream, n_text, n, c->d_lut, d_sym);
    if (reuse_code) {
      code = c->code_cache;
      c->code_uses++;
    } else {
      std::vector<uint32_t> h32(256);
      WP_HIP(hipMemcpyAsync(h32.data(), c->d_symhist, sizeof(uint32_t) * 256, hipMemcpyDeviceToHost, st));
      if (sizeof(SymT) == 1) {
        for (int r = 0; r < 3; r++) {
          WP_HIP(hipMemcpyAsync(h_blank_lut[r], c->d_lut + kBlankCpRuns[r][0], sizeof(uint32_t) * kBlankCpRuns[r][1],
                                hipMemcpyDeviceToHost, st));
        }
      }
      WP_HIP(hipStreamSynchronize(st));
      const size_t nitems = (static_cast<size_t>(S.alphabet) >> lo_bits) + 1;
      std::vector<uint64_t> freq(nitems);
      for (size_t i = 0; i < nitems; i++) freq[i] = h32[i];
      code = build_symbol_code(freq, bits, true);
      if (!code.uniform_bits) {
        code.lo_bits = lo_bits;
        code.avg_bits += lo_bits;
      }
      c->code_cache = code;
      c->code_cached = true;
      c->code_alphabet = static_cast<uint32_t>(S.alphabet);
      c->code_bits = bits;
      c->code_lo = lo_bits;
      c->code_uses = 0;
      uint64_t all = 0, blank = 0;
      for (size_t i = 0; i < nitems; i++) all += freq[i];
      if (sizeof(SymT) == 1) {
        for (int r = 0; r < 3; r++) {
          for (uint32_t k = 0; k + 1 < kBlankCpRuns[r][1]; k++) {
            const uint32_t cp = kBlankCpRuns[r][0] + k, s = h_blank_lut[r][k] + 1u;
            if (is_space(cp) && h_blank_lut[r][k + 1] != h_blank_lut[r][k] && s < nitems) blank += freq[s];
          }
        }
      }
      c->code_blank_share = all ? static_cast<double>(blank) / static_cast<double>(all) : 0.0;
      if (!code.uniform_bits) {
        const size_t blob_bytes = 512 + 256 + kDecodeTableBytes;
// ... 45 lines not shown
                           dcode, KA, DG0, cand);
      } else {
        hipLaunchKernelGGL(HIP_KERNEL_NAME(build_keys0_kernel<SymT, false>), dim3(cdiv(n, kKeyTile)), dim3(kBlock), 0, st, d_sym, n,
                           dcode, KA, DG0, cand);
      }
    }
    if (keys_only) {
      WP_HIP(hipEventRecord(c->evs[kEvKeysBuilt], st));
      WP_HIP(hipStreamWaitEvent(st2, c->evs[kEvKeysBuilt], 0));
      device_exclusive_scan(d_cand_bcnt, d_cand_boff, cand_blocks, d_cand_scan, c->d_scalars + kScalarCand, st2);
      hipLaunchKernelGGL(cand_compact_kernel, dim3(cand_blocks), dim3(kBlock), 0, st2, VA, VB, d_cand_bcnt, d_cand_boff, cand.tile, n,
                         X1, d_node_of_slot);
      WP_HIP(hipMemcpyAsync(c->h_scalars + kScalarCand, c->d_scalars + kScalarCand, sizeof(uint32_t), hipMemcpyDeviceToHost, st2));
      WP_HIP(hipEventRecord(c->evs[kEvCandCount], st2));
    }
    WP_LAUNCH_CHECK();
  }

  void sort_round0() {
    db.dg0 = DG0;
    db.dg1 = DG1;
    db.dg0_ready = DG0 != nullptr && !hist_in_keys;
    if (key_lookup) {
      Key0 *sk = reinterpret_cast<Key0 *>(X0);
      RadixDrop drop;
      drop.blank_bits = d_blank_bits;
      drop.d_kept = c->d_scalars + kScalarKept;
      drop.h_kept = c->h_scalars + kScalarKept;
      drop.side = st2;
      drop.spine_done = c->evs[kEvSpine];
      drop.copied = c->evs[kEvKept];
      cur = radix_sort_pairs<Key0>(sk, keys_only ? nullptr : VA, KB, keys_only ? nullptr : VB, n, 0, kKeyBits, d_radix_tmp, radix_words,
                                   st, &c->rstats, true, code.uniform_bits ? 0 : 8, db, true, hist_in_keys ? &sort_plan : nullptr, KA,
                                   drop_blanks ? &drop : nullptr);
      if (drop_blanks) n_sorted = drop.kept;
      S.round0_sorted = static_cast<int64_t>(n_sorted);
      S.hist_in_keys = hist_in_keys ? 1 : 0;
      keys = cur ? KB : sk;
      other_keys = cur ? sk : KB;
#ifdef WP_DEBUG_BOUNDS
      if constexpr (sizeof(Key0) == 4) {
        hipLaunchKernelGGL(sorted_check_kernel, dim3(std::min<size_t>(cdiv(n, kBlock), 1024)), dim3(kBlock), 0, st,
                           reinterpret_cast<const uint32_t *>(keys), n_sorted, reinterpret_cast<const uint32_t *>(KA), n, d_cls, n_text,
                           drop_blanks ? d_blank_bits : static_cast<const uint32_t *>(nullptr));
        hipLaunchKernelGGL(sorted_check_close_kernel, dim3(1), dim3(1), 0, st);
        WP_LAUNCH_CHECK();
      }
#endif
      vals = keys_only ? nullptr : (cur ? VB : VA);
      other_vals = keys_only ? nullptr : (cur ? VA : VB);
      if (keys_only) sort_candidates();
      slots = AS0;
      other_slots = AS1;
      adep = AD0;
      other_dep = AD1;
      avals = LA;
      spare_vals = LB;
      return;
    }
    if (window_store) {
      db.tail_bit = kWinBits;
      db.tail_mask = (1u << (win_mid - kWinBits)) - 1u;
      db.tail_from_val = true;
    }
    cur = radix_sort_pairs<Key0>(KA, VA, KB, VB, n, 0, kKeyBits, d_radix_tmp, radix_words, st, &c->rstats, true,
                                 code.uniform_bits ? 0 : 8, db, true, hist_in_keys ? &sort_plan : nullptr);
    S.hist_in_keys = hist_in_keys ? 1 : 0;
    keys = cur ? KB : KA;
    other_keys = cur ? KA : KB;
    vals = cur ? VB : VA;
    other_vals = cur ? VA : VB;
    slots = AS0;
    other_slots = AS1;
    adep = AD0;
    other_dep = AD1;
    avals = LA;
    spare_vals = LB;
  }

  void sort_candidates() {
    WP_HIP(hipEventSynchronize(c->evs[kEvCandCount]));
    n_cand = c->h_scalars[kScalarCand];
    S.round0_candidates = static_cast<int64_t>(n_cand);
    WP_HIP(hipMemsetAsync(d_cand_lo, 0, claim_size * sizeof(uint32_t), st2));
    WP_HIP(hipMemsetAsync(d_cand_hi, 0, claim_size * sizeof(uint32_t), st2));
    const uint32_t *sorted_slot = X1, *sorted_pos = d_node_of_slot;
    if (n_cand > 1) {
      const int cc = radix_sort_pairs<uint32_t>(X1, d_node_of_slot, VA, VB, n_cand, 0, cand_bits, d_radix_tmp2,
                                                std::max(radix_tmp_words<uint64_t>(list_cap), radix_tmp_words<uint32_t>(n)), st2, nullptr,
                                                false, cand_bits, DigitBytes(), true);
      sorted_slot = cc ? VA : X1;
      sorted_pos = cc ? VB : d_node_of_slot;
    }
    if (n_cand > 0) {
      hipLaunchKernelGGL(cand_runs_kernel, dim3(cdiv(n_cand, kBlock)), dim3(kBlock), 0, st2, sorted_slot, n_cand, d_cand_lo, d_cand_hi);
    }
    WP_LAUNCH_CHECK();
    cand_runs.table = d_cand_table;
    cand_runs.bits = cand_bits;
    cand_runs.lo = d_cand_lo;
    cand_runs.hi = d_cand_hi;
    cand_runs.pos = sorted_pos;
  }

  bool classify_groups(size_t list_len) {
    if (list_len <= static_cast<size_t>(kLsMaxGroup)) return false;
    const size_t cap = list_len / 2 + 1;
    clear_scalars(c, kScalarListLargeGroups, kScalarListLargeEntries, st2);
    hipLaunchKernelGGL(large_groups_kernel, dim3(std::min<size_t>(cdiv(cap, kBlock), 2048)), dim3(kBlock), 0, st2, d_ghead,
                       c->d_scalars + kScalarListGroups, reinterpret_cast<unsigned long long *>(c->d_scalars + kScalarListLargeGroups),
                       d_lg_head, d_lg_off);
    hipLaunchKernelGGL(large_groups_close_kernel, dim3(1), dim3(1), 0, st2, c->d_scalars + kScalarListLargeGroups, d_lg_off);
    return true;
  }

  void store_ranks(uint32_t *dst, uint32_t *val, uint32_t *t_dst, uint32_t *t_val, size_t m) {
    if (val && m >= (1u << 22)) {
      const int hb = bit_length(n - 1);
      const int bc = radix_sort_pairs<uint32_t>(dst, val, t_dst, t_val, m, std::max(0, hb - 8), hb, d_radix_tmp, radix_words, st,
                                                nullptr, false, hb + 1, DigitBytes(), true);
      hipLaunchKernelGGL(scatter_pairs_kernel, dim3(cdiv(m, kSpTile)), dim3(kBlock), 0, st, bc ? t_dst : dst, bc ? t_val : val, m,
                         d_rank, n, 1);
    } else {
      hipLaunchKernelGGL(scatter_pairs_kernel, dim3(cdiv(m, kSpTile)), dim3(kBlock), 0, st, dst, val, m, d_rank, n, 0);
    }
  }

  void store_ranks_round0(uint32_t *dst, uint32_t *val, uint8_t *dig, uint8_t *other, const std::function<void()> &before_second,
                          const std::function<void()> &before_window) {
    WP_HIP(hipFuncSetAttribute(reinterpret_cast<const void *>(window_store_kernel), hipFuncAttributeMaxDynamicSharedMemorySize,
                               static_cast<int>(kWinLdsBytes)));
    uint32_t *a_dst = X0, *a_val = X1, *b_dst = other_vals, *b_val = reinterpret_cast<uint32_t *>(keys);
    DigitBytes d1;
    d1.dg0 = dig;
    d1.dg1 = other;
    d1.dg0_ready = dig != nullptr;
    if (win_mid < hb_n) {
      d1.tail_bit = win_mid;
      d1.tail_mask = (1u << (hb_n - win_mid)) - 1u;
    }
    radix_sort_pairs<uint32_t>(dst, val, a_dst, a_val, n, kWinBits, win_mid, d_radix_tmp, radix_words, st, &c->rstats,
                               val == nullptr, 0, d1, true);
    if (before_second) before_second();
    const uint32_t *f_dst = a_dst, *f_val = a_val;
    if (win_mid < hb_n) {
      DigitBytes d2;
      d2.dg0 = dig ? d1.tail_out(1) : nullptr;
      d2.dg1 = dig ? dig : nullptr;
      d2.dg0_ready = dig != nullptr;
      radix_sort_pairs<uint32_t>(a_dst, a_val, b_dst, b_val, n, win_mid, hb_n, d_radix_tmp, radix_words, st, &c->rstats, false, 0,
                                 d2);
      f_dst = b_dst;
      f_val = b_val;
    }
    if (before_window) before_window();
    hipLaunchKernelGGL(window_store_kernel, dim3(cdiv(n, size_t(1) << kWinBits)), dim3(kWinThreads), kWinLdsBytes, st, f_dst, f_val,
                       n, d_rank);
  }

  void ranks_round0() {
    const DepthRule rule{need_depth, full ? 1 : 0, nullptr, nullptr, 0, nullptr};
    const unsigned tiles = cdiv(n, kRrTile);
    const bool slot_ranks = text_only && !d_lcp;
    uint8_t *dig = DG0 ? db.tail_out(cur) : nullptr, *dig_other = DG0 ? db.tail_out(cur ^ 1) : nullptr;
    auto enqueue_needed_groups = [&](hipEvent_t start_after) {
      if (start_after) WP_HIP(hipStreamWaitEvent(st2, start_after, 0));
      WP_HIP(hipMemsetAsync(d_claim, 0xff, claim_size * sizeof(uint32_t), st2));
      WP_HIP(hipMemsetAsync(d_claim_need, 0, claim_size * sizeof(uint32_t), st2));
      NeededList nl{slots, avals, AG, adep, d_ghead, d_gfirst, d_gdep, reinterpret_cast<unsigned long long *>(c->d_scalars + kScalarList),
                    static_cast<uint32_t *>(nullptr), need_depth, d_claim_need, d_gclaim, d_gneed0,
                    keys_only ? d_gcand : nullptr, keys_only ? cand_runs.pos : nullptr, keys_only ? n_cand : 0};
      const TokenTrie trie{c->d_lt_chain_len, c->d_lt_chain_off, c->d_lt_child_begin, c->d_lt_child_node, d_child_sym};
      if (use_trie) {
        const size_t ns = hv.stream.size(), nc = hv.lt_child_cp.size();
        hipLaunchKernelGGL(HIP_KERNEL_NAME(trie_map_symbols_kernel<SymT>), dim3(cdiv(std::max<size_t>(std::max(ns, nc), 1), kBlock)),
                           dim3(kBlock), 0, st2, c->d_stream, ns, c->d_lt_child_cp, nc, c->d_lut, d_vsym, d_child_sym);
      }
      if (M > 0) {
        hipLaunchKernelGGL(HIP_KERNEL_NAME(need_groups_kernel<SymT>), dim3(cdiv(static_cast<size_t>(M) * kWave, kBlock)),
                           dim3(kBlock), 0, st2, keys, vals, n_sorted, n, d_sym, c->d_stream, c->d_elig_start, c->d_elig_info, M, c->d_lut, dcode,
                           d_claim, static_cast<uint32_t>(claim_size - 1), nl, text_only ? d_rng_lo : nullptr, d_rng_hi, d_rng_long,
                           cand_runs);
      }
      hipLaunchKernelGGL(needed_list_clamp_kernel, dim3(1), dim3(1), 0, st2, c->d_scalars + kScalarList, static_cast<uint32_t>(list_cap),
                         c->d_scalars + kScalarListWanted);
      hipLaunchKernelGGL(needed_list_close_kernel, dim3(1), dim3(1), 0, st2, c->d_scalars + kScalarList, d_ghead);
      if (key_lookup) {
        hipLaunchKernelGGL(group_starts_kernel, dim3(cdiv(M, kBlock)), dim3(kBlock), 0, st2, d_gfirst, d_ghead, c->d_scalars + kScalarList,
                           n_sorted, d_ps0 + P, d_gend);
      }
      if (M > 0) {
        if (!use_trie) hipLaunchKernelGGL(needed_need_kernel, dim3(cdiv(M, kBlock)), dim3(kBlock), 0, st2, nl);
        hipLaunchKernelGGL(needed_fill_kernel, dim3(1024), dim3(kBlock), 0, st2, nl, vals, n_sorted);
        if (use_trie) {
          hipLaunchKernelGGL(HIP_KERNEL_NAME(trie_group_start_kernel<SymT>), dim3(cdiv(M, kBlock)), dim3(kBlock), 0, st2, vals,
                             keys_only ? cand_runs.pos : nullptr, d_gcand, d_gfirst,
                             d_gdep, c->d_scalars + kScalarList, d_sym, n, d_vsym, trie, d_gnode, d_gdone);
        }
      }
      WP_HIP(hipEventRecord(c->evs[kEvKeysFree], st2));
      if (use_trie) trie_round_sizes();
    };
    if (key_lookup) {
      fork();
      enqueue_needed_groups(nullptr);
      trie_round_sort();
      if (n_text > 0) launch_anchors(st);
      WP_LAUNCH_CHECK();
      trie_round_finish();
      return;
    }
    if (prune) {
      fork();
      enqueue_needed_groups(nullptr);
      if (!slot_ranks) {
        hipLaunchKernelGGL(round0_rank_kernel<true>, dim3(cdiv(n, kR0Tile)), dim3(kBlock), 0, st, keys, vals, n, dcode.first_len,
                           dcode.uniform_bits, d_sa, d_hd_n, d_lcp, d_gdepth);
      }
    } else {
      hipLaunchKernelGGL(widen_keys_kernel, dim3(std::min<size_t>(cdiv(n, kBlock), 8192)), dim3(kBlock), 0, st, keys, LK2, n);
      hipLaunchKernelGGL(HIP_KERNEL_NAME(rerank_agg_kernel<true>), dim3(tiles), dim3(kBlock), 0, st, LK2, vals, n,
                         static_cast<const uint32_t *>(nullptr), static_cast<const RankEntry *>(nullptr),
                         static_cast<const uint32_t *>(nullptr), n, dcode.first_len, dcode.uniform_bits, rule, d_tdep, d_agg);
      hipLaunchKernelGGL(rerank_chunk_kernel, dim3(cdiv(tiles, kRrChunk)), dim3(kBlock), 0, st, d_agg, tiles, d_chunk_agg);
      hipLaunchKernelGGL(rerank_prefix_kernel, dim3(cdiv(tiles, kRrChunk)), dim3(kBlock), 0, st, d_agg, d_chunk_agg, tiles);
      hipLaunchKernelGGL(HIP_KERNEL_NAME(rerank_apply_kernel<SymT, true>), dim3(tiles), dim3(kBlock), 0, st, LK2, vals,
                         static_cast<const uint32_t *>(nullptr), static_cast<const uint32_t *>(nullptr), d_tdep, n, d_agg, d_sym, n,
                         dcode.first_len, dcode.uniform_bits, rule, d_sa, d_hd_n, d_lcp, slots, avals, AG, adep, d_ghead, d_gdepth,
                         c->d_scalars + kScalarList);
    }
    uint32_t *rank_vals = slot_ranks ? nullptr : reinterpret_cast<uint32_t *>(d_hd_n);
    auto keys_free = [&] {
      if (prune) WP_HIP(hipStreamWaitEvent(st, c->evs[kEvKeysFree], 0));
    };
    auto start_trie_round = [&] {
      if (!use_trie) return;
      WP_HIP(hipEventRecord(c->evs[kEvPartition], st));
      WP_HIP(hipStreamWaitEvent(st2, c->evs[kEvPartition], 0));
      trie_round_sort();
    };
    if (window_store) {
      store_ranks_round0(vals, rank_vals, dig, dig_other, keys_free, start_trie_round);
    } else {
      keys_free();
      start_trie_round();
      store_ranks(vals, rank_vals, X0, X1, n);
    }
    WP_LAUNCH_CHECK();
    if (use_trie) {
      trie_round_finish();
    } else {
      if (prune) join();
      fork();
      classified = classify_groups(std::min(n, list_cap));
      join();
    }
  }

  int trie_rb() const { return bit_length(hv.lt_chain_len.size() + 1); }
  void trie_round_sizes() {
    classified = classify_groups(list_cap);
    queue_scalars(c, kScalarAnchorGap, st2);
    WP_HIP(hipEventRecord(c->evs[kEvScalars], st2));
  }
  void trie_round_sort() {
    const TokenTrie trie{c->d_lt_chain_len, c->d_lt_chain_off, c->d_lt_child_begin, c->d_lt_child_node, d_child_sym};
    hipLaunchKernelGGL(HIP_KERNEL_NAME(trie_walk_kernel<SymT>), dim3(std::min<size_t>(cdiv(list_cap, kBlock), 16384)), dim3(kBlock), 0,
                       st2, avals, AG, d_gnode, d_gdone, c->d_scalars + kScalarList, d_sym, n, d_vsym, trie, adep);
    WP_HIP(hipEventRecord(c->evs[kEvTrieNodes], st2));
    hipLaunchKernelGGL(local_sort_kernel, dim3(cdiv(list_cap, kLsT)), dim3(kBlock), 0, st2, avals, AG, adep, c->d_scalars + kScalarList,
                       d_ghead, d_rank, n, trie_rb(), LK0, spare_vals, adep);
  }
  void refine_stats(size_t groups, int rbits) {
    S.refine.n_groups = static_cast<int64_t>(groups);
    S.refine.n_entries = static_cast<int64_t>(n_act);
    S.refine.n_large_groups = static_cast<int64_t>(n_large_groups);
    S.refine.n_large_entries = static_cast<int64_t>(n_large);
    S.refine.trie_nodes = static_cast<int64_t>(hv.lt_chain_len.size());
    S.refine.sort_bits = rbits;
    S.refine.key_lookup = key_lookup ? 1 : 0;
    S.refine.symbol_bytes = static_cast<int32_t>(sizeof(SymT));
  }
  void trie_round_finish() {
    WP_HIP(hipEventSynchronize(c->evs[kEvScalars]));
    n_act = c->h_scalars[kScalarListEntries];
    n_groups = c->h_scalars[kScalarListGroups];
    n_large_groups = classified ? c->h_scalars[kScalarListLargeGroups] : 0;
    n_large = classified ? c->h_scalars[kScalarListLargeEntries] : 0;
    if (c->h_scalars[kScalarListWanted] > list_cap) throw ListOverflow{c->h_scalars[kScalarListWanted]};
    S.active_per_round[0] = static_cast<int64_t>(n);
    refine_stats(n_groups, trie_rb());
    uint64_t *skeys = LK0;
    RankEntry *hd = reinterpret_cast<RankEntry *>(LK1);
    if (n_act > 0) {
      S.active_per_round[1] = static_cast<int64_t>(n_act);
      const int rb = trie_rb();
      if (n_large > 0) {
        hipStream_t st3 = c->stream3;
        WP_HIP(hipStreamWaitEvent(st3, c->evs[kEvTrieNodes], 0));
        const int lgb = bit_length(n_large_groups > 0 ? n_large_groups - 1 : 0);
        hipLaunchKernelGGL(large_extract_kernel, dim3(cdiv(cdiv(n_large, kLxSpan), kBlock / kWave)), dim3(kBlock), 0, st3, avals, adep,
                           d_lg_head, d_lg_off, static_cast<uint32_t>(n_large_groups), n_large, d_rank, n, rb, LK1, LV0, LPOS, adep);
        const int lc = radix_sort_pairs<uint64_t>(LK1, LV0, LK2, LV1, n_large, 0, rb + lgb, d_radix_tmp2,
                                                  radix_tmp_words<uint64_t>(list_cap), st3, nullptr);
        hipLaunchKernelGGL(large_writeback_kernel, dim3(std::min<size_t>(cdiv(n_large, kBlock), 8192)), dim3(kBlock), 0, st3,
                           lc ? LK2 : LK1, lc ? LV1 : LV0, LPOS, n_large, AG, rb, skeys, spare_vals);
        WP_HIP(hipEventRecord(c->evs[kEvLargeSorted], st3));
        WP_HIP(hipStreamWaitEvent(st2, c->evs[kEvLargeSorted], 0));
      }
      DepthRule rrule{need_depth, 0, nullptr, nullptr, 1, d_node_of_slot};
      const unsigned tiles = cdiv(n_act, kRrTile);
      hipLaunchKernelGGL(HIP_KERNEL_NAME(rerank_agg_kernel<false>), dim3(tiles), dim3(kBlock), 0, st2, skeys, spare_vals, n_act, adep,
                         d_rank, d_gdepth, n, dcode.first_len, dcode.uniform_bits, rrule, d_tdep, d_agg);
      hipLaunchKernelGGL(rerank_chunk_kernel, dim3(cdiv(tiles, kRrChunk)), dim3(kBlock), 0, st2, d_agg, tiles, d_chunk_agg);
      hipLaunchKernelGGL(rerank_prefix_kernel, dim3(cdiv(tiles, kRrChunk)), dim3(kBlock), 0, st2, d_agg, d_chunk_agg, tiles);
      hipLaunchKernelGGL(HIP_KERNEL_NAME(rerank_apply_kernel<SymT, false>), dim3(tiles), dim3(kBlock), 0, st2, skeys, spare_vals, slots,
                         adep, d_tdep, n_act, d_agg, d_sym, n, dcode.first_len, dcode.uniform_bits, rrule, d_sa, hd, d_lcp,
                         other_slots, avals, AG, other_dep, d_ghead, d_gdepth, c->d_scalars + kScalarList);
    }
    join();
    if (n_act > 0) {
      store_ranks(spare_vals, hd, reinterpret_cast<uint32_t *>(hd) + list_cap + 2, reinterpret_cast<uint32_t *>(skeys), n_act);
      rounds = 2;
    }
    WP_LAUNCH_CHECK();
  }

  void next_round_begin(size_t upper, int rb) {
    queue_scalars(c, kScalarAnchorGap, st);
    WP_HIP(hipEventRecord(c->evs[kEvScalars], st));
    fork();
    if (upper > 0) {
      hipLaunchKernelGGL(local_sort_kernel, dim3(cdiv(upper, kLsT)), dim3(kBlock), 0, st, avals, AG, adep, c->d_scalars + kScalarList, d_ghead,
                         d_rank, n, rb, LK0, spare_vals, static_cast<const uint32_t *>(nullptr));
    }
    WP_HIP(hipEventSynchronize(c->evs[kEvScalars]));
    n_act = c->h_scalars[kScalarListEntries];
    n_large_groups = classified ? c->h_scalars[kScalarListLargeGroups] : 0;
    n_large = classified ? c->h_scalars[kScalarListLargeEntries] : 0;
    if (c->h_scalars[kScalarListWanted] > list_cap) throw ListOverflow{c->h_scalars[kScalarListWanted]};
  }

  void refine() {
    if (!use_trie) doubling_rounds();
    S.rounds = rounds;
    const int max_len = code.uniform_bits ? code.uniform_bits : kMaxCodeLen + code.lo_bits;
    const int32_t key_syms = std::max(1, kKeyBits / max_len);
    S.sorted_depth = full ? 0x7fffffff
                          : (prune ? std::min<int32_t>(static_cast<int32_t>(need_depth), key_syms) : static_cast<int32_t>(need_depth));
    S.needed_after_round0 = prune ? (rounds > 1 ? S.active_per_round[1] : 0) : -1;
    if (prune && rounds > 1) c->list_hint = static_cast<size_t>(S.active_per_round[1]);
  }

  void doubling_rounds() {
    const int rb = bit_length(n);
    const DepthRule rule{need_depth, full ? 1 : 0, nullptr, nullptr, 0, nullptr};
    next_round_begin(std::min(n, list_cap), rb);
    S.active_per_round[0] = static_cast<int64_t>(n);
    refine_stats(c->h_scalars[kScalarListGroups], rb);
    uint32_t *gneed_cur = d_gneed0, *gneed_nxt = d_gneed1;
    const bool group_need = prune && M > 0;
    while (n_act > 0) {
      DepthRule rrule = rule;
      if (group_need) {
        rrule.gneed_in = gneed_cur;
        rrule.gneed_out = gneed_nxt;
        std::swap(gneed_cur, gneed_nxt);
      }
      if (static_cast<uint64_t>(rounds) > 80 + (full ? 0ull : static_cast<uint64_t>(need_depth))) {
        throw HipError("prefix doubling did not converge (internal error)");
      }
      if (rounds < 40) S.active_per_round[rounds] = static_cast<int64_t>(n_act);
      uint64_t *skeys = LK0, *kfree = LK1;
      uint32_t *svals = spare_vals, *nvals = avals;
      if (n_large > 0) {
        const int lgb = bit_length(n_large_groups > 0 ? n_large_groups - 1 : 0);
        hipLaunchKernelGGL(large_extract_kernel, dim3(cdiv(cdiv(n_large, kLxSpan), kBlock / kWave)), dim3(kBlock), 0, st2, avals, adep,
                           d_lg_head, d_lg_off, static_cast<uint32_t>(n_large_groups), n_large, d_rank, n, rb, LK1, LV0, LPOS,
                           static_cast<const uint32_t *>(nullptr));
        const int lc = radix_sort_pairs<uint64_t>(LK1, LV0, LK2, LV1, n_large, 0, rb + lgb, d_radix_tmp, radix_words, st2, nullptr);
        hipLaunchKernelGGL(large_writeback_kernel, dim3(std::min<size_t>(cdiv(n_large, kBlock), 8192)), dim3(kBlock), 0, st2,
                           lc ? LK2 : LK1, lc ? LV1 : LV0, LPOS, n_large, AG, rb, skeys, svals);
        join();
      }
      const unsigned tiles = cdiv(n_act, kRrTile);
      RankEntry *hd = reinterpret_cast<RankEntry *>(kfree);
      hipLaunchKernelGGL(HIP_KERNEL_NAME(rerank_agg_kernel<false>), dim3(tiles), dim3(kBlock), 0, st, skeys, svals, n_act, adep,
                         d_rank, d_gdepth, n, dcode.first_len, dcode.uniform_bits, rrule, d_tdep, d_agg);
      hipLaunchKernelGGL(rerank_chunk_kernel, dim3(cdiv(tiles, kRrChunk)), dim3(kBlock), 0, st, d_agg, tiles, d_chunk_agg);
      hipLaunchKernelGGL(rerank_prefix_kernel, dim3(cdiv(tiles, kRrChunk)), dim3(kBlock), 0, st, d_agg, d_chunk_agg, tiles);
      hipLaunchKernelGGL(HIP_KERNEL_NAME(rerank_apply_kernel<SymT, false>), dim3(tiles), dim3(kBlock), 0, st, skeys, svals, slots,
                         adep, d_tdep, n_act, d_agg, d_sym, n, dcode.first_len, dcode.uniform_bits, rrule, d_sa, hd, d_lcp,
                         other_slots, nvals, AG, other_dep, d_ghead, d_gdepth, c->d_scalars + kScalarList);
      fork();
      store_ranks(svals, hd, reinterpret_cast<uint32_t *>(hd) + list_cap + 2, reinterpret_cast<uint32_t *>(skeys), n_act);
      WP_LAUNCH_CHECK();
      rounds++;
      classified = classify_groups(n_act);
      join();
      std::swap(slots, other_slots);
      std::swap(adep, other_dep);
      avals = nvals;
      spare_vals = svals;
      next_round_begin(n_act, rb);
    }
  }

  void scanlines() {
    if (n_text > 0) fork();
    MarkView mv{};
    const int pack_steps = (hv.longest < kStepMaxLen && hv.tokens.size() < (size_t(1) << kStepIdBits)) ? 1 : 0;
    const size_t vocab_base = n_text + 1;
    uint32_t *mslot = d_mslot0, *midx = d_midx0;
    if (text_only) {
      if (M > 0) {
        hipLaunchKernelGGL(trie_token_range_kernel, dim3(cdiv(M, kBlock)), dim3(kBlock), 0, st, d_node_of_slot, c->d_elig_node,
                           c->d_elig_subtree, M, d_rng_lo, d_rng_hi, d_rng_long);
        hipLaunchKernelGGL(virtual_marks_kernel, dim3(cdiv(M, kBlock)), dim3(kBlock), 0, st, d_rng_lo, d_rng_hi, M, c->d_elig_id,
                           c->d_elig_info, d_mslot0, d_mid, d_minfo, d_rf, d_rb);
      }
      mv = MarkView{mslot, d_mid, d_minfo, d_rf, d_rb, M, d_cover_f, d_cover_b};
    } else {
      if (M > 0) {
        hipLaunchKernelGGL(mark_slots_kernel, dim3(cdiv(M, kBlock)), dim3(kBlock), 0, st, c->d_elig_start, M, vocab_base, d_rank,
                           d_mslot0, d_midx0);
        int mc = radix_sort_pairs<uint32_t>(d_mslot0, d_midx0, d_mslot1, d_midx1, M, 0, bit_length(n), d_radix_tmp, radix_words, st,
                                            nullptr);
        mslot = mc ? d_mslot1 : d_mslot0;
        midx = mc ? d_midx1 : d_midx0;
        hipLaunchKernelGGL(mark_gather_kernel, dim3(cdiv(M, kBlock)), dim3(kBlock), 0, st, midx, M, c->d_elig_id, c->d_elig_info,
                           d_mid, d_minfo);
      }
      hipLaunchKernelGGL(tile_mlo_kernel, dim3(cdiv(sl_tiles + 1, kBlock)), dim3(kBlock), 0, st, mslot, M, n, sl_tiles, d_tile_mlo);
      hipLaunchKernelGGL(sl_summary_kernel, dim3(sl_tiles), dim3(kBlock), 0, st, d_lcp, n, mslot, d_minfo, d_tile_mlo, d_tmin_f,
                         d_tmin_b, d_rf, d_rb);
      hipLaunchKernelGGL(sl_group_min_kernel, dim3(cdiv(static_cast<size_t>(sl_groups) * kWave, kBlock)), dim3(kBlock), 0, st,
                         d_tmin_f, d_tmin_b, sl_tiles, sl_groups, d_gmin_f, d_gmin_b);
      mv = MarkView{mslot, d_mid, d_minfo, d_rf, d_rb, M, d_cover_f, d_cover_b};
      if (M > 0) {
        hipLaunchKernelGGL(sl_reach_global_kernel, dim3(cdiv(static_cast<size_t>(M) * kWave, kBlock)), dim3(kBlock), 0, st, d_lcp, n,
                           sl_tiles, sl_groups, mslot, d_minfo, M, d_tmin_f, d_tmin_b, d_gmin_f, d_gmin_b, d_rf, d_rb);
      }
    }
    if (M > 0) {
      hipLaunchKernelGGL(mark_cover_kernel, dim3(4), dim3(kCoverThreads), 0, st, d_minfo, d_rf, d_rb, M, d_cover_f, d_cover_b);
    }
    if (n_text > 0 && !anchors_queued) launch_anchors(st2);
    hipLaunchKernelGGL(piece_starts_kernel, dim3(cdiv(std::max(M, 1), kBlock)), dim3(kBlock), 0, st, mv, n_sorted, d_ps0);
    const int P = this->P + (key_lookup ? 2 * static_cast<int>(n_groups) : 0);
    const int pc = radix_sort_pairs<uint32_t>(d_ps0, d_pv0, d_ps1, d_pv1, P, 0, bit_length(n), d_radix_tmp, radix_words, st, nullptr);
    nbuckets = static_cast<unsigned>(((n_sorted - 1) >> bucket_shift) + 1);
    nbuckets_all = static_cast<unsigned>(((n_sorted - 1) >> bucket_shift_all) + 1);
    uint32_t *pstart = pc ? d_ps1 : d_ps0;
    hipLaunchKernelGGL(piece_values_kernel, dim3(cdiv(static_cast<size_t>(P) * kWave, kBlock)), dim3(kBlock), 0, st, mv, pstart, P,
                       d_pval_p, d_pval_s, pack_steps);
    hipLaunchKernelGGL(piece_bucket_kernel, dim3(cdiv(nbuckets + 1, kBlock)), dim3(kBlock), 0, st, pstart, P, bucket_shift, nbuckets,
                       d_bidx);
    hipLaunchKernelGGL(piece_bucket_fast_kernel, dim3(cdiv(nbuckets, kBlock)), dim3(kBlock), 0, st, d_bidx, d_pval_p, d_pval_s, nbuckets,
                       d_bfast);
    WP_LAUNCH_CHECK();
    steps = StepTable{pstart, d_pval_p, d_pval_s, d_bidx, bucket_shift, pack_steps, d_bfast};
    steps_all = steps;
    if (bucket_shift_all != bucket_shift) {
      hipLaunchKernelGGL(piece_bucket_kernel, dim3(cdiv(nbuckets_all + 1, kBlock)), dim3(kBlock), 0, st, pstart, P, bucket_shift_all,
                         nbuckets_all, d_bidx_all);
      hipLaunchKernelGGL(piece_bucket_fast_kernel, dim3(cdiv(nbuckets_all, kBlock)), dim3(kBlock), 0, st, d_bidx_all, d_pval_p, d_pval_s,
                         nbuckets_all, d_bfast_all);
      WP_LAUNCH_CHECK();
      steps_all = StepTable{pstart, d_pval_p, d_pval_s, d_bidx_all, bucket_shift_all, pack_steps, d_bfast_all};
    }
    if (key_lookup) key_steps(pstart, P, pack_steps);
  }

  void key_steps(const uint32_t *pstart, int P, int pack_steps) {
    const uint32_t *skeys = reinterpret_cast<const uint32_t *>(keys);
    hipLaunchKernelGGL(key_steps_kernel, dim3(cdiv(P, kBlock)), dim3(kBlock), 0, st, pstart, d_pval_p, d_pval_s, P, skeys, d_kstart,
                       d_kval_p, d_kval_s);
    if (n_groups > 0) {
      hipLaunchKernelGGL(key_steps_needed_kernel, dim3(cdiv(n_groups, kBlock)), dim3(kBlock), 0, st, d_gfirst, d_gend,
                         static_cast<uint32_t>(n_groups), pstart, P, d_kval_p, d_kval_s);
    }
#ifdef WP_DEBUG_BOUNDS
    hipLaunchKernelGGL(key_steps_check_kernel, dim3(cdiv(P, kBlock)), dim3(kBlock), 0, st, pstart, P, skeys, d_kval_p, d_kval_s);
#endif
    hipLaunchKernelGGL(piece_bucket_kernel, dim3(cdiv(nkbuckets + 1, kBlock)), dim3(kBlock), 0, st, d_kstart, P, key_shift, nkbuckets,
                       d_kbidx);
    hipLaunchKernelGGL(piece_bucket_fast_kernel, dim3(cdiv(nkbuckets, kBlock)), dim3(kBlock), 0, st, d_kbidx, d_kval_p, d_kval_s,
                       nkbuckets, d_kbfast);
    ksteps = StepTable{d_kstart, d_kval_p, d_kval_s, d_kbidx, key_shift, pack_steps, d_kbfast};
    ksteps_all = ksteps;
    if (key_shift_all != key_shift) {
      hipLaunchKernelGGL(piece_bucket_kernel, dim3(cdiv(nkbuckets_all + 1, kBlock)), dim3(kBlock), 0, st, d_kstart, P, key_shift_all,
                         nkbuckets_all, d_kbidx_all);
      hipLaunchKernelGGL(piece_bucket_fast_kernel, dim3(cdiv(nkbuckets_all, kBlock)), dim3(kBlock), 0, st, d_kbidx_all, d_kval_p,
                         d_kval_s, nkbuckets_all, d_kbfast_all);
      ksteps_all = StepTable{d_kstart, d_kval_p, d_kval_s, d_kbidx_all, key_shift_all, pack_steps, d_kbfast_all};
    }
    WP_LAUNCH_CHECK();
  }

// ... 181 lines not shown
                         static_cast<const uint32_t *>(rows->d_line_cnt), n_rows, d_line_starts);
      d_starts = d_line_starts;
    }
    if (n_ids > 0) {
      hipLaunchKernelGGL(cp_byte_kernel, dim3(cdiv(nbytes, kDecTile)), dim3(kBlock), 0, st, d_text, nbytes, d_tile_prefix, n_text,
                         d_byte_of);
      if (nmap && rows->d_doc_off) {
        hipLaunchKernelGGL(norm_doc_starts_kernel, dim3(cdiv(n_rows + 1, kBlock)), dim3(kBlock), 0, st, rows->d_doc_off, n_rows, *nmap,
                           static_cast<const uint32_t *>(d_byte_of), nbytes, d_line_starts);
        d_starts = d_line_starts;
      }
      hipLaunchKernelGGL(row_splits_kernel, dim3(cdiv(n_rows + 1, kBlock)), dim3(kBlock), 0, st, d_starts, n_rows,
                         static_cast<const uint32_t *>(d_byte_of), n_text, static_cast<const uint2 *>(d_offs), n_ids, rows->unit,
                         d_row_splits, d_row_base);
      if (nmap && d_row_base) {
        hipLaunchKernelGGL(norm_row_base_kernel, dim3(cdiv(n_rows + 1, kBlock)), dim3(kBlock), 0, st, d_starts, n_rows,
                           static_cast<const uint32_t *>(d_byte_of), n_text, *nmap, rows->unit, d_row_base);
      }
    } else {
      WP_HIP(hipMemsetAsync(d_row_splits, 0, (n_rows + 1) * sizeof(long long), st));
    }
    WP_LAUNCH_CHECK();
    rows->d_starts = d_starts;
    rows->d_row_splits = d_row_splits;
  }

  void finish(int32_t *d_ids, size_t *n_ids_out) {
    c->d_offs = nullptr;
    if (offs_unit >= 0 && n_text > 0) {
      fetch_scalars(c, kScalarIds);
      const size_t n_ids = c->h_scalars[kScalarIds];
      if (rows) row_structure(n_ids);
      if (nmap) {
        if (n_ids > 0 && (!rows || rows->unit >= 0)) {
          hipLaunchKernelGGL(span_source_kernel, dim3(cdiv(n_ids, kBlock)), dim3(kBlock), 0, st, d_offs, n_ids, *nmap, offs_unit);
          WP_LAUNCH_CHECK();
        }
      } else if (offs_unit == WP_OFFSETS_BYTES && n_ids > 0) {
        if (!rows) {
          hipLaunchKernelGGL(cp_byte_kernel, dim3(cdiv(nbytes, kDecTile)), dim3(kBlock), 0, st, d_text, nbytes, d_tile_prefix, n_text,
                             d_byte_of);
        }
        hipLaunchKernelGGL(span_bytes_kernel, dim3(cdiv(n_ids, kBlock)), dim3(kBlock), 0, st, d_offs, n_ids,
                           static_cast<const uint32_t *>(d_byte_of), d_text, n_text);
        WP_LAUNCH_CHECK();
      }
      if (rows && rows->unit >= 0 && n_ids > 0) {
        hipLaunchKernelGGL(rebase_kernel, dim3(cdiv(n_ids, kRebaseTile)), dim3(kBlock), 0, st, d_offs, n_ids,
                           static_cast<const long long *>(d_row_splits), rows->n_rows, static_cast<const uint32_t *>(d_row_base));
        WP_LAUNCH_CHECK();
      }
      c->d_offs = reinterpret_cast<const uint32_t *>(d_offs);
    } else if (rows) {
      row_structure(0);
    }
    if (ar.guard) {
      static const uint32_t init[2] = {0u, 0xffffffffu};
      WP_HIP(hipMemcpyAsync(c->d_scalars + kScalarGuard, init, sizeof(init), hipMemcpyHostToDevice, st));
      ar.check(st, c->d_scalars + kScalarGuard);
      aa.check(st, c->d_scalars + kScalarGuard);
      fetch_scalars(c, kScalarGuardFirst);
      if (c->h_scalars[kScalarGuardBad] != 0) {
        throw HipError("arena guard: " + std::to_string(c->h_scalars[kScalarGuardBad]) + " guard zone(s) overwritten, first behind allocation #" +
                       std::to_string(c->h_scalars[kScalarGuardFirst] - 1));
      }
      S.guard_zones = static_cast<int32_t>(ar.zones.size() + aa.zones.size());
    }
#ifdef WP_DEBUG_BOUNDS
    {
      unsigned int oob[kBoundSites] = {};
      WP_HIP(hipStreamSynchronize(st));
      take_oob(0, kBoundSites, oob);
      if (oob[0] | oob[1] | oob[2] | oob[3] | oob[4] | oob[5] | oob[6] | oob[7] | oob[8]) {
        throw HipError("debug bounds: out-of-range addresses skipped: radix scatter " + std::to_string(oob[0]) + ", rank store " +
                       std::to_string(oob[1]) + ", token id " + std::to_string(oob[2]) + ", list slot " + std::to_string(oob[3]) +
                       "; key-space step starts inside a run of equal keys " + std::to_string(oob[4]) +
                       "; candidate runs unlike their group " + std::to_string(oob[5]) + "; offsets " + std::to_string(oob[6]) +
                       "; step values used at blanks " + std::to_string(oob[7]) +
                       "; round-0 sorted array: descents, blank keys left, multiset unlike the kept keys " + std::to_string(oob[8]));
      }
      S.reserved0 = 1;
    }
#endif
    fetch_scalars(c, kScalarFree18);
    const size_t n_ids = n_text > 0 ? c->h_scalars[kScalarIds] : 0;
    S.n_ids = static_cast<int64_t>(n_ids);
    S.walk.n_wide_words = wide_ran ? static_cast<int64_t>(c->h_scalars[kScalarWideWords]) : 0;
    S.radix_passes = c->rstats.passes;
    S.radix_pass_elems = c->rstats.elems;
    S.radix_digit_bytes = c->rstats.digit_bytes;
    S.radix_pass_bytes = c->rstats.bytes;
    S.arena_bytes = static_cast<int64_t>(c->a_buf.cap + c->b_buf.cap);
    if (v->stage_timing) {
      auto span = [&](int a, int b) {
        float ms = 0;
        WP_HIP(hipEventElapsedTime(&ms, c->ev[a], c->ev[b]));
        return static_cast<double>(ms);
      };
      S.ms_decode = span(kMarkStart, kMarkSymbols);
      S.ms_sa = span(kMarkSymbols, kMarkSorted);
      S.ms_lcp = span(kMarkSorted, kMarkLcp);
      S.ms_scan = span(kMarkLcp, kMarkScanned);
      S.ms_walk = span(kMarkScanned, kMarkWalked);
      S.ms_total = span(kMarkStart, kMarkWalked) + S.ms_normalize;
      S.ms_radix_scatter = c->rstats.spans.resolve();
    }
    c->d_ids = d_ids;
    c->dbg.sym = d_sym;
    c->dbg.sym_bytes = sizeof(SymT);
    c->dbg.sa = d_sa;
    c->dbg.rank = d_rank;
    c->dbg.lcp = d_lcp;
    c->dbg.steps = steps;
    c->dbg.best_scratch = d_dbg_best;
    c->dbg.cps = d_cps;
    c->dbg.cls = v->keep_debug ? d_cls : nullptr;
    c->dbg.n = n;
    c->dbg.n_text = n_text;
    *n_ids_out = n_ids;
  }

  void run(size_t *n_ids_out) {
    plan();
    symbols_and_keys();
    if (v->stage_timing) WP_HIP(hipEventRecord(c->ev[kMarkSymbols], st));
    sort_round0();
    ranks_round0();
    refine();
    if (v->stage_timing) WP_HIP(hipEventRecord(c->ev[kMarkSorted], st));
    if (v->lcp_kasai) {
      const size_t chunk = 64;
      hipLaunchKernelGGL(HIP_KERNEL_NAME(kasai_kernel<SymT>), dim3(cdiv(cdiv(n, chunk), kBlock)), dim3(kBlock), 0, st, d_sym, d_sa,
                         d_rank, n, chunk, d_lcp);
      WP_LAUNCH_CHECK();
    }
    if (v->stage_timing) WP_HIP(hipEventRecord(c->ev[kMarkLcp], st));
    scanlines();
    if (v->stage_timing) WP_HIP(hipEventRecord(c->ev[kMarkScanned], st));
    size_t n_ids = 0;
    int32_t *d_ids = walk(&n_ids);
    if (v->stage_timing) WP_HIP(hipEventRecord(c->ev[kMarkWalked], st));
    finish(d_ids, n_ids_out);
  }
};

static void encode_on_device(const wp_vocab *v, Context *c, const uint8_t *d_text, size_t nbytes, size_t *n_ids_out,
                             EncodeStats &S, int offs_unit = -1, RowsCall *rows = nullptr) {
  hipStream_t st = c->stream;
  const HostVocab &hv = v->hv;
  std::memset(&S, 0, sizeof(S));
  S.offsets_unit = -1;
  S.n_rows = -1;
  S.rows_route = -1;
  S.n_bytes = static_cast<int64_t>(nbytes);
  S.longest_token = hv.longest;
  c->d_ids = nullptr;
  c->d_offs = nullptr;
  c->dbg = {};
  *n_ids_out = 0;
  if (nbytes == 0) return;
  const bool guard = v->arena_guard || EnvOptions::get().arena_guard;
  S.offsets_unit = offs_unit;
  c->d_offs = nullptr;

  const uint8_t *src_text = d_text;
  const size_t src_bytes = nbytes;
  NormResult norm;
  const NormMap *nmap = nullptr;
  if (v->normalize != 0) {
    normalize_on_device(c, d_text, nbytes, v->normalize, offs_unit >= 0, v->stage_timing, norm);
    S.normalize = v->normalize;
    S.norm_bytes = static_cast<int64_t>(norm.nbytes);
    S.ms_normalize = norm.ms;
    if (norm.nbytes == 0) {
      if (!rows) return;
      WP_HIP(hipMemsetAsync(c->norm_buf.p, 0x20, 1, st));
      norm.nbytes = 1;
    }
    d_text = norm.text;
    nbytes = norm.nbytes;
    if (offs_unit >= 0) nmap = &norm.map;
  }

  c->rstats.passes = 0;
  c->rstats.elems = 0;
  c->rstats.digit_bytes = 0;
  c->rstats.bytes = 0;
  c->rstats.spans.on = v->stage_timing;
  c->rstats.spans.used = 0;
  if (v->stage_timing) WP_HIP(hipEventRecord(c->ev[kMarkStart], st));

  const unsigned dec_tiles = cdiv(nbytes, kDecTile);
  Arena aa(&c->a_buf, guard);
  uint32_t *d_tile_cnt = nullptr, *d_cnt_tmp = nullptr, *d_cps = nullptr;
  uint8_t *d_cls = nullptr;
  const unsigned line_tiles = cdiv(nbytes, kLineTile), src_line_tiles = cdiv(src_bytes, kLineTile);
  uint32_t *d_line_tmp = nullptr, *d_src_line_cnt = nullptr;
  for (int pass = 0; pass < 2; pass++) {
    d_tile_cnt = aa.take<uint32_t>(dec_tiles + 1);
    d_cnt_tmp = aa.take<uint32_t>(cdiv(dec_tiles, kScanTile) + 8);
    d_cps = v->keep_debug ? aa.take<uint32_t>(nbytes + 1) : nullptr;
    d_cls = aa.take<uint8_t>(nbytes + 32);
    if (rows && !rows->d_doc_off) {
      rows->d_line_cnt = aa.take<uint32_t>(line_tiles + 1);
      d_line_tmp = aa.take<uint32_t>(cdiv(line_tiles, kScanTile) + 8);
      if (v->normalize != 0) d_src_line_cnt = aa.take<uint32_t>(src_line_tiles + 1 + cdiv(src_line_tiles, kScanTile) + 8);
    }
    if (pass == 0) aa.commit();
  }
// ... 89 lines not shown
```

### wordpiece_amd/csrc/prune.h

```cpp
#pragma once
#include "decode.h"
#include "primitives.h"

namespace wp {

constexpr uint32_t kClaimEmpty = 0xffffffffu;

__device__ inline bool wave_token_key(const uint32_t *__restrict__ cps, uint32_t len, const uint32_t *__restrict__ lut_excl,
                                      const DevCode &code, uint64_t &key_out, int &bits_out, uint32_t &whole_out) {
  const int ub = code.uniform_bits > 0 ? code.uniform_bits : 0;
  const int lo = code.uniform_bits < 0 ? -code.uniform_bits : 0;
  const uint32_t lomask = (1u << lo) - 1u;
  const uint32_t lane = static_cast<uint32_t>(lane_id());
  uint32_t l = 0;
  uint64_t c = 0;
  if (lane < len) {
    const uint32_t sv = lut_excl[cps[lane]] + 1u;
    if (ub) {
      l = static_cast<uint32_t>(ub);
      c = sv;
    } else {
      const uint32_t hi = sv >> lo;
      l = static_cast<uint32_t>(code.len[hi]) + static_cast<uint32_t>(lo);
      c = (static_cast<uint64_t>(code.cw[hi]) << lo) | (sv & lomask);
// ... 91 lines not shown
                                                             uint32_t *__restrict__ rng_hi,
                                                             uint8_t *__restrict__ rng_long, CandRuns cr) {
  const int m = static_cast<int>((static_cast<size_t>(blockIdx.x) * kBlock + threadIdx.x) >> 6);
  const int lane = lane_id();
  if (m >= M) return;
  uint64_t key = 0;
  int bits = 0;
  const uint32_t len = tok_info[m] & 0x0fffffffu;
  const uint32_t *cps = vocab_cps + tok_start[m];
  uint32_t whole = 0;
  const bool is_long = wave_token_key(cps, len, lut_excl, code, key, bits, whole);
  if (!is_long) {
    if (!rng_lo) return;
    const size_t lb = wave_key_lower_bound(keys, 0, ns, key, 2);
    const uint64_t step = 1ull << (kKeyBits - bits);
    const uint64_t above = key + step;
    const size_t ubd = (bits == 0 || (above >> kKeyBits) != 0) ? ns : wave_key_gallop(keys, lb, ns, above);
    if (lane == 0) {
      rng_lo[m] = static_cast<uint32_t>(lb);
      rng_hi[m] = static_cast<uint32_t>(ubd);
      rng_long[m] = 0;
    }
    return;
  }
  const size_t first = wave_key_lower_bound(keys, 0, ns, key, 2);
  const size_t last = wave_key_gallop(keys, first, ns, key + 1);
  uint32_t crun = 0;
  if (cr.pos && lane == 0 && last > first) {
    const uint32_t s = cand_find(cr.table, cr.bits, static_cast<uint32_t>(key));
    const bool found = s != ~0u;
    crun = found ? cr.lo[s] : 0u;
    wp_in_bounds(found && cr.hi[s] - cr.lo[s] == last - first, kSiteCandRun);
  }
  if (last - first < 2) {
    if (rng_lo && lane == 0) {
      size_t lb = first, ubd = first;
      if (last > first) {
        const int cmp = suffix_vs_token(sym, n, cr.pos ? cr.pos[crun] : vals[first], cps, len, lut_excl);
        lb = cmp < 0 ? first + 1 : first;
        ubd = cmp <= 0 ? first + 1 : first;
      }
      rng_lo[m] = static_cast<uint32_t>(lb);
      rng_hi[m] = static_cast<uint32_t>(ubd);
      rng_long[m] = 0;
    }
    return;
  }
  if (rng_lo && lane == 0) {
    rng_lo[m] = static_cast<uint32_t>(first);
    rng_hi[m] = static_cast<uint32_t>(last);
    rng_long[m] = 1;
  }
  unsigned long long got = ~0ull;
  uint32_t depth = 0, claim_slot = 0;
  if (lane == 0) {
    uint32_t h = (static_cast<uint32_t>(first) * 2654435761u) & claim_mask;
    bool won = false;
    for (;;) {
      const uint32_t old = atomicCAS(&claim[h], kClaimEmpty, static_cast<uint32_t>(first));
      if (old == kClaimEmpty) {
        won = true;
        break;
      }
      if (old == static_cast<uint32_t>(first)) break;
      h = (h + 1) & claim_mask;
    }
    atomicMax(&out.claim_need[h], min(len, out.need_depth - 1u) + 1u);
    claim_slot = h;
    if (won) {
      depth = whole;
      if (depth < out.need_depth) {
        got = atomicAdd(out.totals, (1ull << 32) | static_cast<unsigned long long>(last - first));
      }
    }
  }
  if (lane == 0 && got != ~0ull) {
    const uint32_t g = static_cast<uint32_t>(got >> 32);
    out.ghead[g] = static_cast<uint32_t>(got);
    out.gfirst[g] = static_cast<uint32_t>(first);
    out.gdepth[g] = depth;
    out.gclaim[g] = claim_slot;
    if (out.gcand) out.gcand[g] = crun;
  }
}

__global__ __launch_bounds__(kBlock) void needed_need_kernel(NeededList out) {
  const uint32_t g = blockIdx.x * kBlock + threadIdx.x;
  if (g < reinterpret_cast<const uint32_t *>(out.totals)[1]) out.gneed[g] = out.claim_need[out.gclaim[g]];
}

__global__ __launch_bounds__(kBlock) void needed_fill_kernel(NeededList out, const uint32_t *__restrict__ sorted_vals,
                                                             size_t n) {
  const uint32_t *t32 = reinterpret_cast<const uint32_t *>(out.totals);
  const uint32_t n_act = t32[0], n_groups = t32[1];
  const int lane = lane_id();
  for (size_t p0 = (static_cast<size_t>(blockIdx.x) * kBlock + threadIdx.x) & ~static_cast<size_t>(kWave - 1); p0 < n_act;
       p0 += static_cast<size_t>(gridDim.x) * kBlock) {
    const size_t p = p0 + lane;
    uint32_t a = 0, b = n_groups - 1;
    while (a < b) {
      const uint32_t st = (b - a) / kWave + 1;
      const uint32_t idx = a + static_cast<uint32_t>(lane) * st;
      const bool gt = idx < b ? out.ghead[idx + 1] > p0 : true;
      const uint64_t mm = __ballot(gt);
      if (!mm) {
        a += (kWave - 1) * st + 1;
        continue;
      }
      const uint32_t t = static_cast<uint32_t>(__ffsll(static_cast<long long>(mm)) - 1);
      const uint32_t first = a + t * st;
      if (t) a += (t - 1) * st + 1;
      b = first < b ? first : b;
      if (!t) b = a;
    }
    if (p >= n_act) continue;
    uint32_t lo = a, hi = min(n_groups, a + static_cast<uint32_t>(kWave));
    while (hi - lo > 1) {
      const uint32_t md = (lo + hi) >> 1;
      if (out.ghead[md] <= p) lo = md; else hi = md;
    }
    const uint32_t k = out.gfirst[lo] + static_cast<uint32_t>(p - out.ghead[lo]);
    if (!wp_in_bounds(k < n, kSiteListSlot)) continue;
    uint32_t v;
    if (out.cand_pos) {
      const size_t ci = static_cast<size_t>(out.gcand[lo]) + (p - out.ghead[lo]);
      if (!wp_in_bounds(ci < out.cand_cap, kSiteListSlot) || ci >= out.cand_cap) continue;
      v = out.cand_pos[ci];
    } else {
      v = sorted_vals[k];
    }
    out.slots[p] = k;
    out.vals[p] = v;
    out.gid[p] = lo;
    out.dep[p] = out.gdepth[lo];
    if (out.sa) out.sa[k] = v;
  }
}

__global__ void needed_list_close_kernel(const uint32_t *__restrict__ totals, uint32_t *__restrict__ ghead) {
  ghead[totals[1]] = totals[0];
}

__global__ __launch_bounds__(kBlock) void virtual_marks_kernel(const uint32_t *__restrict__ rng_lo,
                                                               const uint32_t *__restrict__ rng_hi, int M,
                                                               const int32_t *__restrict__ tok_id,
                                                               const uint32_t *__restrict__ tok_info,
                                                               uint32_t *__restrict__ mslot, int32_t *__restrict__ mid,
                                                               uint32_t *__restrict__ minfo,
                                                               int32_t *__restrict__ reach_fwd,
                                                               int32_t *__restrict__ reach_bwd) {
  const int m = blockIdx.x * kBlock + threadIdx.x;
  if (m >= M) return;
  const uint32_t lo = rng_lo[m];
  mslot[m] = lo;
  mid[m] = tok_id[m];
  minfo[m] = tok_info[m];
  reach_fwd[m] = static_cast<int32_t>(max(rng_hi[m], lo));
  reach_bwd[m] = static_cast<int32_t>(lo);
}

}
```

### wordpiece_amd/csrc/suffix_array.h

```cpp
#pragma once
#include "decode.h"
#include "primitives.h"
#include "radix_sort.h"

namespace wp {

constexpr int kRrItems = 8;
constexpr int kRrTile = kBlock * kRrItems;

using RankEntry = uint32_t;
__host__ __device__ inline uint32_t rank_of(RankEntry e) { return e; }
constexpr uint32_t kRankUnchanged = 0xffffffffu;

struct RerankAgg {
  uint32_t last_flag;
  uint32_t n_active;
  uint32_t n_heads;
};

struct DepthRule {
  uint32_t need;
  int full;
  const uint32_t *gneed_in;
  uint32_t *gneed_out;
// ... 134 lines not shown
  if (t < tiles) mine = agg[t];
  const int lane = lane_id(), w = wave_id();
  uint32_t ia = mine.n_active, ih = mine.n_heads, im = mine.last_flag;
#pragma unroll
  for (int d = 1; d < kWave; d <<= 1) {
    const uint32_t ta = __shfl_up(ia, d, kWave), th = __shfl_up(ih, d, kWave), tm = __shfl_up(im, d, kWave);
    if (lane >= d) {
      ia += ta;
      ih += th;
      im = max(im, tm);
    }
  }
  if (lane == kWave - 1) {
    wa[w] = ia;
    wh[w] = ih;
    wm[w] = im;
  }
  __syncthreads();
  RerankAgg o = before;
  for (int q = 0; q < w; q++) {
    o.n_active += wa[q];
    o.n_heads += wh[q];
    o.last_flag = max(o.last_flag, wm[q]);
  }
  const uint32_t pm = __shfl_up(im, 1, kWave);
  o.n_active += ia - mine.n_active;
  o.n_heads += ih - mine.n_heads;
  if (lane > 0) o.last_flag = max(o.last_flag, pm);
  if (t < tiles) agg[t] = o;
}

template <typename SymT>
__device__ __forceinline__ int32_t lcp_compare(const SymT *__restrict__ sym, size_t n, size_t a, size_t b,
                                               int32_t maxlen) {
  const size_t hi = a > b ? a : b;
  if (hi >= n) return 0;
  const int32_t lim = static_cast<int32_t>(min(static_cast<size_t>(maxlen), n - hi));
  int32_t t = 0;
  if (sizeof(SymT) == 1) {
    const uint8_t *pa = reinterpret_cast<const uint8_t *>(sym) + a, *pb = reinterpret_cast<const uint8_t *>(sym) + b;
    while (t < lim) {
      uint64_t wa, wb;
      __builtin_memcpy(&wa, pa + t, 8);
      __builtin_memcpy(&wb, pb + t, 8);
      const uint64_t x = wa ^ wb;
      if (x) {
        t += (__ffsll(static_cast<long long>(x)) - 1) >> 3;
        break;
      }
      t += 8;
    }
    return min(t, lim);
  }
  while (t < lim && sym[a + t] == sym[b + t]) t++;
  return t;
}

#ifndef WP_SP_ITEMS
#define WP_SP_ITEMS 1
#endif
constexpr int kSpItems = WP_SP_ITEMS;
constexpr int kSpTile = kBlock * kSpItems;
__global__ __launch_bounds__(kBlock) void scatter_pairs_kernel(const uint32_t *__restrict__ dst,
                                                               const RankEntry *__restrict__ val, size_t m,
                                                               RankEntry *__restrict__ out, size_t out_n, int xcd) {
  unsigned b = blockIdx.x;
  if (xcd) {
    const unsigned nb = gridDim.x, q = nb / 8, r = nb % 8, x = b % 8;
    b = (x < r ? x * (q + 1) : r * (q + 1) + (x - r) * q) + b / 8;
  }
  const size_t base = static_cast<size_t>(b) * kSpTile + threadIdx.x;
  uint32_t d[kSpItems];
  RankEntry v[kSpItems];
#pragma unroll
  for (int j = 0; j < kSpItems; j++) {
    const size_t k = base + static_cast<size_t>(j) * kBlock;
    v[j] = k < m ? (val ? val[k] : static_cast<RankEntry>(k)) : kRankUnchanged;
    d[j] = k < m ? dst[k] : 0u;
  }
#pragma unroll
  for (int j = 0; j < kSpItems; j++) {
    if (v[j] != kRankUnchanged && wp_in_bounds(d[j] < out_n, kSiteRankStore)) out[d[j]] = v[j];
  }
}

constexpr int kWinBits = 15;
constexpr int kWinThreads = 1024;
constexpr size_t kWinLdsBytes = sizeof(RankEntry) << kWinBits;
__global__ __launch_bounds__(kWinThreads) void window_store_kernel(const uint32_t *__restrict__ dst,
                                                                   const RankEntry *__restrict__ val, size_t m,
                                                                   RankEntry *__restrict__ out) {
  extern __shared__ RankEntry win[];
  const size_t w0 = static_cast<size_t>(blockIdx.x) << kWinBits;
  const uint32_t cnt = static_cast<uint32_t>(min(static_cast<size_t>(1) << kWinBits, m - w0));
  const uint32_t lo = static_cast<uint32_t>(w0);
  auto place = [&](uint32_t d, RankEntry v) {
    const bool ok = d - lo < cnt;
    wp_in_bounds(ok, kSiteRankStore);
    if (ok) win[d - lo] = v;
  };
  for (uint32_t k = threadIdx.x * 4; k < cnt; k += kWinThreads * 4) {
    if (k + 4 <= cnt) {
      const uint4 d = *reinterpret_cast<const uint4 *>(dst + w0 + k);
      const uint4 v = *reinterpret_cast<const uint4 *>(val + w0 + k);
      place(d.x, v.x);
      place(d.y, v.y);
      place(d.z, v.z);
      place(d.w, v.w);
    } else {
      for (uint32_t j = k; j < cnt; j++) place(dst[w0 + j], val[w0 + j]);
    }
  }
  __syncthreads();
  for (uint32_t k = threadIdx.x * 4; k < cnt; k += kWinThreads * 4) {
    if (k + 4 <= cnt) {
      *reinterpret_cast<uint4 *>(out + w0 + k) = *reinterpret_cast<const uint4 *>(win + k);
    } else {
      for (uint32_t j = k; j < cnt; j++) out[w0 + j] = win[j];
    }
  }
}

struct RrTile {
  uint64_t bfs[kRrRounds], bas[kRrRounds], bss[kRrRounds], bos[kRrRounds];
  uint64_t mes[kRrRounds];
  uint32_t nds[kRrRounds];
  uint32_t na, nh, last;
};

template <bool ROUND0, bool OWN_DEPTH>
__device__ __forceinline__ void rr_first_half(RrTile &T, const uint64_t *__restrict__ keys, size_t m, size_t wave_base,
                                              const uint32_t *__restrict__ tdep, const uint32_t *__restrict__ vals,
                                              const uint32_t *__restrict__ adep, const RankEntry *__restrict__ rd,
                                              const uint32_t *__restrict__ gdepth_in, size_t n, const uint8_t *s_fl,
                                              int uniform_bits, DepthRule rule) {
  const int lane = lane_id();
  T.na = T.nh = T.last = 0;
#pragma unroll
  for (int r = 0; r < kRrRounds; r++) {
    const size_t k = wave_base + static_cast<size_t>(r) * kWave + lane;
    bool f = false, sg = false, act = false, same_old = false;
    uint64_t me = 0;
    uint32_t nd = 0;
    if (k < m) {
      me = keys[k];
      const uint64_t prev = k > 0 ? keys[k - 1] : ~me;
      const uint64_t next = k + 1 < m ? keys[k + 1] : ~me;
      f = prev != me;
      sg = f && next != me;
      if (!sg) {
        if (!OWN_DEPTH) {
          nd = tdep[k];
        } else if (ROUND0) {
          nd = static_cast<uint32_t>(count_key_symbols(me, kKeyBits, s_fl, uniform_bits));
        } else if (rule.final_round) {
          nd = 0u;
        } else {
          const uint32_t d = adep[k];
          const uint32_t r2 = static_cast<uint32_t>(me);
          const uint32_t dj = r2 ? gdepth_in[r2 - 1u] : 0u;
          nd = min(d + dj, 0x7fffffffu);
        }
        act = rr_stays_active(rule, nd, ROUND0 ? 0u : static_cast<uint32_t>(me >> 32));
      }
      if (ROUND0) {
        nd = min(nd, 0xffffu);
// ... 337 lines not shown
```

### wordpiece_amd/csrc/trie.h

```cpp
#pragma once
#include "decode.h"
#include "primitives.h"

namespace wp {

struct TokenTrie {
  const uint32_t *chain_len;
  const uint32_t *chain_off;
  const uint32_t *child_begin;
  const uint32_t *child_node;
  const uint32_t *child_sym;
};

template <typename SymT>
__global__ __launch_bounds__(kBlock) void trie_map_symbols_kernel(const uint32_t *__restrict__ stream_cps, size_t n_stream,
                                                                  const uint32_t *__restrict__ child_cps, size_t n_child,
                                                                  const uint32_t *__restrict__ lut_excl,
                                                                  SymT *__restrict__ vsym, uint32_t *__restrict__ child_sym) {
  const size_t i = static_cast<size_t>(blockIdx.x) * kBlock + threadIdx.x;
  if (i < n_stream) vsym[i] = static_cast<SymT>(lut_excl[stream_cps[i]] + 1u);
  if (i < n_child) child_sym[i] = lut_excl[child_cps[i]] + 1u;
}

template <typename SymT>
__device__ __forceinline__ uint32_t trie_chain_match(const SymT *__restrict__ sym, size_t n, size_t pos,
                                                     const SymT *__restrict__ label, uint32_t len) {
  if (pos >= n) return 0u;
  const uint32_t lim = static_cast<uint32_t>(min(static_cast<size_t>(len), n - pos));
  uint32_t t = 0;
  if (sizeof(SymT) == 1) {
    const uint8_t *pa = reinterpret_cast<const uint8_t *>(sym) + pos, *pb = reinterpret_cast<const uint8_t *>(label);
    while (t < lim) {
      uint64_t wa, wb;
      __builtin_memcpy(&wa, pa + t, 8);
      __builtin_memcpy(&wb, pb + t, 8);
      const uint64_t x = wa ^ wb;
      if (x) {
        t += static_cast<uint32_t>(__ffsll(static_cast<long long>(x)) - 1) >> 3;
        break;
      }
      t += 8;
    }
    return min(t, lim);
  }
  while (t < lim && sym[pos + t] == label[t]) t++;
  return t;
}

template <typename SymT>
__device__ __forceinline__ uint32_t trie_descend(const TokenTrie &t, const SymT *__restrict__ sym, size_t n,
                                                 const SymT *__restrict__ vsym, uint32_t node, size_t pos, uint32_t limit,
                                                 uint32_t &left_out) {
  uint32_t left = limit ? limit : 0xffffffffu;
  for (;;) {
    const uint32_t len = t.chain_len[node];
    if (len) {
      const uint32_t want = min(len, left);
      const uint32_t l = trie_chain_match(sym, n, pos, vsym + t.chain_off[node], want);
      node += l;
      pos += l;
      left -= l;
      if (l < len) break;
    }
    if (left == 0) break;
    uint32_t lo = t.child_begin[node], hi = t.child_begin[node + 1];
    if (lo == hi || pos >= n) break;
    const uint32_t s = static_cast<uint32_t>(sym[pos]), end = hi;
    while (lo < hi) {
      const uint32_t md = (lo + hi) >> 1;
      if (t.child_sym[md] < s) lo = md + 1; else hi = md;
    }
    if (lo == end || t.child_sym[lo] != s) break;
    node = t.child_node[lo];
    pos++;
    left--;
  }
  left_out = limit ? left : 0u;
  return node;
}

template <typename SymT>
__global__ __launch_bounds__(kBlock) void trie_group_start_kernel(const uint32_t *__restrict__ sorted_vals,
                                                                  const uint32_t *__restrict__ cand_pos,
                                                                  const uint32_t *__restrict__ gcand,
                                                                  const uint32_t *__restrict__ gfirst,
                                                                  const uint32_t *__restrict__ gdepth,
                                                                  const uint32_t *__restrict__ sizes_dev,
                                                                  const SymT *__restrict__ sym, size_t n,
                                                                  const SymT *__restrict__ vsym, TokenTrie t,
                                                                  uint32_t *__restrict__ gnode, uint32_t *__restrict__ gdone) {
  const uint32_t g = blockIdx.x * kBlock + threadIdx.x;
  if (g >= sizes_dev[1]) return;
  const uint32_t d = gdepth[g];
  uint32_t left = 0, node = 0;
  if (d) {
    const uint32_t member = cand_pos ? cand_pos[gcand[g]] : sorted_vals[gfirst[g]];
    node = trie_descend(t, sym, n, vsym, 0u, static_cast<size_t>(member), d, left);
  }
  gnode[g] = node;
  gdone[g] = d - left;
}

template <typename SymT>
__global__ __launch_bounds__(kBlock) void trie_walk_kernel(const uint32_t *__restrict__ vals,
                                                           const uint32_t *__restrict__ gid,
                                                           const uint32_t *__restrict__ gnode,
                                                           const uint32_t *__restrict__ gdone,
                                                           const uint32_t *__restrict__ sizes_dev,
                                                           const SymT *__restrict__ sym, size_t n,
                                                           const SymT *__restrict__ vsym, TokenTrie t,
                                                           uint32_t *__restrict__ node_out) {
  const size_t m = sizes_dev[0];
  for (size_t p = static_cast<size_t>(blockIdx.x) * kBlock + threadIdx.x; p < m; p += static_cast<size_t>(gridDim.x) * kBlock) {
    const uint32_t g = gid[p];
    uint32_t unused;
    node_out[p] = trie_descend(t, sym, n, vsym, gnode[g], static_cast<size_t>(vals[p]) + gdone[g], 0u, unused);
  }
}


__global__ __launch_bounds__(kBlock) void trie_token_range_kernel(const uint32_t *__restrict__ node_of_slot,
                                                                  const uint32_t *__restrict__ tok_node,
                                                                  const uint32_t *__restrict__ tok_subtree, int M,
                                                                  uint32_t *__restrict__ rng_lo, uint32_t *__restrict__ rng_hi,
                                                                  const uint8_t *__restrict__ rng_long) {
  const int m = blockIdx.x * kBlock + threadIdx.x;
  if (m >= M || !rng_long[m]) return;
  const uint32_t glo = rng_lo[m], ghi = rng_hi[m];
  const uint32_t a = tok_node[m], b = a + tok_subtree[m];
  uint32_t lo = glo, hi = ghi;
  while (lo < hi) {
    const uint32_t md = lo + ((hi - lo) >> 1);
    if (node_of_slot[md] < a) lo = md + 1; else hi = md;
  }
  const uint32_t first = lo;
  hi = ghi;
  while (lo < hi) {
    const uint32_t md = lo + ((hi - lo) >> 1);
    if (node_of_slot[md] < b) lo = md + 1; else hi = md;
  }
  rng_lo[m] = first;
  rng_hi[m] = lo;
}

}
```

Before: 29260.

## Start trie refinement before round-0 sort completes, overlapping it on side stream

Adds an early-refine schedule for the keys-only path. Needed groups are built from candidate runs before the full suffix sort finishes, so the trie walk and rerank run on the side stream in parallel with the main sort. Group ranks are then rebased with a scatter kernel once group starts are known, and token ranges are resolved per group list. It also merges three memsets into one and adds new kernels and events, at the cost of more complex stream synchronisation.

```diff
diff --git a/include/wordpiece_amd.h b/include/wordpiece_amd.h
--- a/include/wordpiece_amd.h
+++ b/include/wordpiece_amd.h
@@ -138,6 +138,7 @@
 #define WP_NORM_LOWER 2
 #define WP_NORM_STRIP_ACCENTS 4
 #define WP_NORM_BERT_UNCASED 7
+#define WP_OPT_LATE_REFINE 15
 int wp_set_option(wp_vocab *v, int option, int64_t value);
 
 int wp_normalize_cp(int flags, uint32_t cp, uint32_t out[3]);
@@ -204,6 +205,12 @@
 } wp_refine_stats;
 int wp_get_refine_stats(const wp_vocab *v, wp_refine_stats *out);
 typedef struct {
+  int32_t early;
+  int32_t reserved;
+  double ms_sort_to_scan;
+} wp_refine_sched;
+int wp_get_refine_sched(const wp_vocab *v, wp_refine_sched *out);
+typedef struct {
   int64_t n_samples, n_out;
   int64_t n_cut;
   int64_t n_windowed;
diff --git a/wordpiece_amd/__init__.py b/wordpiece_amd/__init__.py
--- a/wordpiece_amd/__init__.py
+++ b/wordpiece_amd/__init__.py
@@ -13,6 +13,7 @@
 WP_OPT_INDEXED_ROUND0 = 12
 WP_OPT_SORT_BLANKS = 13
 WP_OPT_NORMALIZE = 14
+WP_OPT_LATE_REFINE = 15
 WP_NORM_CLEAN, WP_NORM_LOWER, WP_NORM_STRIP_ACCENTS, WP_NORM_BERT_UNCASED = 1, 2, 4, 7
 WP_OFFSETS_BYTES, WP_OFFSETS_CODE_POINTS = 0, 1
 _OFFSET_UNITS = {"byte": WP_OFFSETS_BYTES, "char": WP_OFFSETS_CODE_POINTS}
@@ -30,7 +31,7 @@
     "wp_linear_encode_offsets", "wp_linear_encode_offsets_device",
     "wp_linear_encode_rows", "wp_linear_encode_rows_device", "wp_linear_encode_padded", "wp_linear_encode_padded_device",
     "wp_normalize_cp", "wp_normalize_device", "wp_normalize", "wp_get_norm_stats", "wp_get_walk_stats",
-    "wp_get_refine_stats",
+    "wp_get_refine_stats", "wp_get_refine_sched",
     "wp_linear_encode_inputs", "wp_linear_encode_inputs_device", "wp_get_inputs_stats",
     "wp_word_ids", "wp_word_ids_device", "wp_mlm_mask", "wp_mlm_mask_device", "wp_get_mask_stats",
     "wp_detokenize", "wp_detokenize_device", "wp_detok_piece", "wp_get_detok_stats",
@@ -79,6 +80,10 @@
     _fields_ = [("n_groups", C.c_int64), ("n_entries", C.c_int64), ("n_large_groups", C.c_int64),
                 ("n_large_entries", C.c_int64), ("trie_nodes", C.c_int64), ("sort_bits", C.c_int32),
                 ("key_lookup", C.c_int32), ("symbol_bytes", C.c_int32), ("reserved", C.c_int32)]
+
+
+class RefineSched(C.Structure):
+    _fields_ = [("early", C.c_int32), ("reserved", C.c_int32), ("ms_sort_to_scan", C.c_double)]
 
 
 class InputsSpec(C.Structure):
@@ -203,6 +208,8 @@
         L.wp_get_norm_stats.argtypes = [vp, C.POINTER(NormStats)]
         L.wp_get_walk_stats.argtypes = [vp, C.POINTER(WalkStats)]
         L.wp_get_refine_stats.argtypes = [vp, C.POINTER(RefineStats)]
+        if hasattr(L, "wp_get_refine_sched"):
+            L.wp_get_refine_sched.argtypes = [vp, C.POINTER(RefineSched)]
         L.wp_linear_debug_fetch.argtypes = [vp, C.c_int, i32p, C.c_size_t, C.POINTER(C.c_size_t)]
         L.wp_free.argtypes = [vp]
         L.wp_free.restype = None
@@ -315,6 +322,11 @@
         rs = RefineStats()
         _check(lib().wp_get_refine_stats(self._h, C.byref(rs)))
         return {k: int(getattr(rs, k)) for k, _ in rs._fields_ if k != "reserved"}
+
+    def refine_sched(self):
+        rs = RefineSched()
+        _check(lib().wp_get_refine_sched(self._h, C.byref(rs)))
+        return {"early": int(rs.early), "ms_sort_to_scan": float(rs.ms_sort_to_scan)}
 
     def encode(self, text):
         b = _bytes(text)
diff --git a/wordpiece_amd/csrc/context.h b/wordpiece_amd/csrc/context.h
--- a/wordpiece_amd/csrc/context.h
+++ b/wordpiece_amd/csrc/context.h
@@ -150,7 +150,7 @@
 constexpr int kScalarGuard = 16;
 constexpr int kScalarGuardBad = kScalarGuard + 0;
 constexpr int kScalarGuardFirst = kScalarGuard + 1;
-constexpr int kScalarFree18 = 18;
+constexpr int kScalarSplitTotals = 18;
 constexpr int kScalarAlphaWord0 = 20;
 constexpr int kScalarRows = 21, kScalarRowsBad = 22, kScalarRowsCut = 23;
 constexpr int kScalarCand = 24;
@@ -175,7 +175,7 @@
     {kScalarListGroups, 1},  {kScalarListLargeGroups, 1}, {kScalarListLargeEntries, 1}, {kScalarListWanted, 1},
     {kScalarIds, 1},         {kScalarAnchors, 1},    {kScalarAnchorGap, 1},       {kScalarLongWords, 1},
     {kScalarWideWords, 1},   {kScalarCps64, 2},      {kScalarGuardBad, 1},        {kScalarGuardFirst, 1},
-    {kScalarFree18, 2},      {kScalarAlphaWord0, 1}, {kScalarRows, 1},            {kScalarRowsBad, 1},
+    {kScalarSplitTotals, 2},      {kScalarAlphaWord0, 1}, {kScalarRows, 1},            {kScalarRowsBad, 1},
     {kScalarRowsCut, 1},     {kScalarCand, 1},       {kScalarKept, 1},            {kScalarSrcRows, 1},
     {kScalarInCut, 1},       {kScalarInRows, 2},     {kScalarInWindowed, 1},      {kScalarFree31, 1},
     {kScalarMask, 12},       {kScalarDetokLast, 2},  {kScalarDetokBad, 1},        {kScalarFree47, 1},
@@ -209,9 +209,9 @@
 };
 
 enum SideEvent { kEvFork, kEvJoin, kEvScalars, kEvKeysFree, kEvPartition, kEvTrieNodes, kEvLargeSorted, kEvKeysBuilt, kEvCandCount,
-                 kEvSpine, kEvKept, kSideEvents };
+                 kEvSpine, kEvKept, kEvSorted, kEvListBuilt, kEvRoundDone, kSideEvents };
 enum TimingMark { kMarkStart, kMarkCounted, kMarkSymbols, kMarkSorted, kMarkLcp, kMarkScanned, kMarkWalked, kMarkNormStart,
-                  kTimingMarks, kMarkNormEnd = kMarkStart };
+                  kMarkRound0, kTimingMarks, kMarkNormEnd = kMarkStart };
 
 struct Context {
   int device = 0;
@@ -312,6 +312,7 @@
   double ms_normalize;
   wp_walk_stats walk;
   wp_refine_stats refine;
+  wp_refine_sched sched;
   wp_inputs_stats inputs;
   int32_t inputs_call;
   wp_mask_stats mask;
@@ -319,6 +320,10 @@
   wp_detok_stats detok;
   int32_t detok_call;
 };
+
+#ifndef WP_LATE_REFINE_DEFAULT
+#define WP_LATE_REFINE_DEFAULT 0
+#endif
 
 struct wp_vocab {
   HostVocab hv;
@@ -331,6 +336,7 @@
   bool vocab_in_s = false;
   bool indexed_round0 = false;
   bool sort_blanks = false;
+  bool late_refine = WP_LATE_REFINE_DEFAULT != 0;
   int normalize = 0;
   int n_devices = 1;
   EncodeStats stats{};
diff --git a/wordpiece_amd/csrc/encoder.hip b/wordpiece_amd/csrc/encoder.hip
--- a/wordpiece_amd/csrc/encoder.hip
+++ b/wordpiece_amd/csrc/encoder.hip
@@ -157,6 +157,7 @@
     case WP_OPT_SPARSE_EMIT: v->sparse_emit = value != 0; return WP_OK;
     case WP_OPT_INDEXED_ROUND0: v->indexed_round0 = value != 0; return WP_OK;
     case WP_OPT_SORT_BLANKS: v->sort_blanks = value != 0; return WP_OK;
+    case WP_OPT_LATE_REFINE: v->late_refine = value != 0; return WP_OK;
     case WP_OPT_NORMALIZE:
       if (!known_norm_flags(value)) {
         g_last_error = "WP_OPT_NORMALIZE: unknown flag bits (WP_NORM_CLEAN | WP_NORM_LOWER | WP_NORM_STRIP_ACCENTS)";
@@ -213,6 +214,15 @@
 
 int wp_get_refine_stats(const wp_vocab *v, wp_refine_stats *out) {
   *out = v->stats.refine;
+  return WP_OK;
+}
+
+int wp_get_refine_sched(const wp_vocab *v, wp_refine_sched *out) {
+  if (!v || !out) {
+    g_last_error = "wp_get_refine_sched: NULL handle or out pointer";
+    return WP_ERR_ARG;
+  }
+  *out = v->stats.sched;
   return WP_OK;
 }
 
@@ -1725,6 +1735,7 @@
       total.refine.n_large_groups = sum.n_large_groups + st.refine.n_large_groups;
       total.refine.n_large_entries = sum.n_large_entries + st.refine.n_large_entries;
     }
+    if (i == 0) total.sched = st.sched;
     total.rounds = std::max(total.rounds, st.rounds);
     if (next_up.valid()) {
       const std::string err = next_up.get();
diff --git a/wordpiece_amd/csrc/linear_path.h b/wordpiece_amd/csrc/linear_path.h
--- a/wordpiece_amd/csrc/linear_path.h
+++ b/wordpiece_amd/csrc/linear_path.h
@@ -99,6 +99,7 @@
   hipStream_t st, st2;
   const HostVocab &hv;
   bool full, prune, use_trie, key_lookup, keys_only, window_store, use_digit_bytes, staged_possible, sparse_emit;
+  bool early_refine;
   bool wide_ran = false;
   uint32_t need_depth;
   int M, P, P_cap, bucket_shift, bucket_shift_all, key_shift, key_shift_all, hb_n, win_mid;
@@ -138,6 +139,7 @@
   int2 *d_kbfast = nullptr, *d_kbfast_all = nullptr;
   unsigned long long *d_cand_table = nullptr;
   uint32_t *d_cand_filter = nullptr, *d_cand_lo = nullptr, *d_cand_hi = nullptr, *d_gcand = nullptr;
+  uint32_t *d_tok_group = nullptr;
   uint32_t *d_cand_bcnt = nullptr, *d_cand_boff = nullptr, *d_cand_scan = nullptr;
   int cand_bits = 0;
   uint32_t *d_blank_bits = nullptr;
@@ -178,6 +180,7 @@
     use_trie = text_only && !full && M > 0;
     key_lookup = use_trie && !v->keep_debug && kKeyBits <= 32;
     keys_only = key_lookup && !v->indexed_round0 && sizeof(SymT) == 1;
+    early_refine = keys_only && !v->late_refine;
     sl_tiles = cdiv(n, kSlTile);
     sl_groups = cdiv(sl_tiles, kSlGroup);
     P = kStepsPerMark * M + 1;
@@ -287,7 +290,14 @@
       d_radix_tmp2 = use_trie ? ar.take<uint32_t>(std::max(radix_tmp_words<uint64_t>(lc), keys_only ? radix_tmp_words<uint32_t>(n) : 0))
                               : nullptr;
       d_claim = ar.take<uint32_t>(claim_size);
-      d_claim_need = ar.take<uint32_t>(claim_size);
+      if (keys_only) {
+        uint32_t *zeroed = ar.take<uint32_t>(3 * claim_size);
+        d_cand_lo = zeroed;
+        d_cand_hi = zeroed ? zeroed + claim_size : nullptr;
+        d_claim_need = zeroed ? zeroed + 2 * claim_size : nullptr;
+      } else {
+        d_claim_need = ar.take<uint32_t>(claim_size);
+      }
       d_gclaim = ar.take<uint32_t>(M + 4);
       d_gfirst = ar.take<uint32_t>(M + 4);
       d_gdep = ar.take<uint32_t>(M + 4);
@@ -333,9 +343,8 @@
       d_kbfast_all = (key_lookup && key_shift_all != key_shift) ? ar.take<int2>(static_cast<size_t>(nkbuckets_all) + 1) : nullptr;
       d_cand_table = keys_only ? ar.take<unsigned long long>(claim_size) : nullptr;
       d_cand_filter = keys_only ? ar.take<uint32_t>(kCandFilterWords) : nullptr;
-      d_cand_lo = keys_only ? ar.take<uint32_t>(claim_size) : nullptr;
-      d_cand_hi = keys_only ? ar.take<uint32_t>(claim_size) : nullptr;
       d_gcand = keys_only ? ar.take<uint32_t>(M + 4) : nullptr;
+      d_tok_group = keys_only ? ar.take<uint32_t>(M + 1) : nullptr;
       d_cand_bcnt = keys_only ? ar.take<uint32_t>(cdiv(n, kKeyTile) + 2) : nullptr;
       d_cand_boff = keys_only ? ar.take<uint32_t>(cdiv(n, kKeyTile) + 2) : nullptr;
       d_cand_scan = keys_only ? ar.take<uint32_t>(cdiv(cdiv(n, kKeyTile), kScanTile) + 8) : nullptr;
@@ -547,8 +556,7 @@
     WP_HIP(hipEventSynchronize(c->evs[kEvCandCount]));
     n_cand = c->h_scalars[kScalarCand];
     S.round0_candidates = static_cast<int64_t>(n_cand);
-    WP_HIP(hipMemsetAsync(d_cand_lo, 0, claim_size * sizeof(uint32_t), st2));
-    WP_HIP(hipMemsetAsync(d_cand_hi, 0, claim_size * sizeof(uint32_t), st2));
+    WP_HIP(hipMemsetAsync(d_cand_lo, 0, 3 * claim_size * sizeof(uint32_t), st2));
     const uint32_t *sorted_slot = X1, *sorted_pos = d_node_of_slot;
     if (n_cand > 1) {
       const int cc = radix_sort_pairs<uint32_t>(X1, d_node_of_slot, VA, VB, n_cand, 0, cand_bits, d_radix_tmp2,
@@ -631,7 +639,7 @@
     auto enqueue_needed_groups = [&](hipEvent_t start_after) {
       if (start_after) WP_HIP(hipStreamWaitEvent(st2, start_after, 0));
       WP_HIP(hipMemsetAsync(d_claim, 0xff, claim_size * sizeof(uint32_t), st2));
-      WP_HIP(hipMemsetAsync(d_claim_need, 0, claim_size * sizeof(uint32_t), st2));
+      if (!keys_only) WP_HIP(hipMemsetAsync(d_claim_need, 0, claim_size * sizeof(uint32_t), st2));
       NeededList nl{slots, avals, AG, adep, d_ghead, d_gfirst, d_gdep, reinterpret_cast<unsigned long long *>(c->d_scalars + kScalarList),
                     static_cast<uint32_t *>(nullptr), need_depth, d_claim_need, d_gclaim, d_gneed0,
                     keys_only ? d_gcand : nullptr, keys_only ? cand_runs.pos : nullptr, keys_only ? n_cand : 0};
@@ -666,6 +674,10 @@
       WP_HIP(hipEventRecord(c->evs[kEvKeysFree], st2));
       if (use_trie) trie_round_sizes();
     };
+    if (early_refine) {
+      refine_early();
+      return;
+    }
     if (key_lookup) {
       fork();
       enqueue_needed_groups(nullptr);
@@ -720,6 +732,39 @@
       classified = classify_groups(std::min(n, list_cap));
       join();
     }
+  }
+
+  void refine_early() {
+    WP_HIP(hipMemsetAsync(d_claim, 0xff, claim_size * sizeof(uint32_t), st2));
+    NeededList nl{slots, avals, AG, adep, d_ghead, static_cast<uint32_t *>(nullptr), d_gdep,
+                  reinterpret_cast<unsigned long long *>(c->d_scalars + kScalarList), static_cast<uint32_t *>(nullptr), need_depth,
+                  d_claim_need, d_gclaim, d_gneed0, d_gcand, cand_runs.pos, n_cand};
+    const TokenTrie trie{c->d_lt_chain_len, c->d_lt_chain_off, c->d_lt_child_begin, c->d_lt_child_node, d_child_sym};
+    const size_t ns = hv.stream.size(), nc = hv.lt_child_cp.size();
+    const unsigned tok_blocks = cdiv(static_cast<size_t>(M) * kWave, kBlock);
+    hipLaunchKernelGGL(HIP_KERNEL_NAME(trie_map_symbols_kernel<SymT>), dim3(cdiv(std::max<size_t>(std::max(ns, nc), 1), kBlock)),
+                       dim3(kBlock), 0, st2, c->d_stream, ns, c->d_lt_child_cp, nc, c->d_lut, d_vsym, d_child_sym);
+    hipLaunchKernelGGL(HIP_KERNEL_NAME(need_groups_early_kernel<SymT>), dim3(tok_blocks), dim3(kBlock), 0, st2, n, d_sym, c->d_stream,
+                       c->d_elig_start, c->d_elig_info, M, c->d_lut, dcode, d_claim, nl, d_rng_lo, d_rng_hi, d_rng_long, cand_runs);
+    hipLaunchKernelGGL(needed_list_clamp_kernel, dim3(1), dim3(1), 0, st2, c->d_scalars + kScalarList, static_cast<uint32_t>(list_cap),
+                       c->d_scalars + kScalarListWanted);
+    hipLaunchKernelGGL(needed_list_close_kernel, dim3(1), dim3(1), 0, st2, c->d_scalars + kScalarList, d_ghead);
+    hipLaunchKernelGGL(needed_fill_kernel, dim3(1024), dim3(kBlock), 0, st2, nl, static_cast<const uint32_t *>(nullptr), n_sorted);
+    hipLaunchKernelGGL(HIP_KERNEL_NAME(trie_group_start_kernel<SymT>), dim3(cdiv(M, kBlock)), dim3(kBlock), 0, st2,
+                       static_cast<const uint32_t *>(nullptr), cand_runs.pos, d_gcand, static_cast<const uint32_t *>(nullptr), d_gdep,
+                       c->d_scalars + kScalarList, d_sym, n, d_vsym, trie, d_gnode, d_gdone);
+    WP_HIP(hipEventRecord(c->evs[kEvListBuilt], st2));
+    trie_round_sizes();
+    trie_round_sort();
+    S.sched.early = 1;
+    WP_HIP(hipEventRecord(c->evs[kEvSorted], st));
+    WP_HIP(hipStreamWaitEvent(st, c->evs[kEvListBuilt], 0));
+    hipLaunchKernelGGL(need_ranges_kernel, dim3(tok_blocks), dim3(kBlock), 0, st, keys, n_sorted, c->d_stream, c->d_elig_start,
+                       c->d_elig_info, M, c->d_lut, dcode, d_claim, d_gfirst, d_rng_lo, d_rng_hi, d_rng_long, d_tok_group);
+    hipLaunchKernelGGL(group_starts_kernel, dim3(cdiv(M, kBlock)), dim3(kBlock), 0, st, d_gfirst, d_ghead, c->d_scalars + kScalarList,
+                       n_sorted, d_ps0 + P, d_gend);
+    WP_LAUNCH_CHECK();
+    trie_round_finish();
   }
 
   int trie_rb() const { return bit_length(hv.lt_chain_len.size() + 1); }
@@ -781,7 +826,28 @@
       hipLaunchKernelGGL(rerank_prefix_kernel, dim3(cdiv(tiles, kRrChunk)), dim3(kBlock), 0, st2, d_agg, d_chunk_agg, tiles);
       hipLaunchKernelGGL(HIP_KERNEL_NAME(rerank_apply_kernel<SymT, false>), dim3(tiles), dim3(kBlock), 0, st2, skeys, spare_vals, slots,
                          adep, d_tdep, n_act, d_agg, d_sym, n, dcode.first_len, dcode.uniform_bits, rrule, d_sa, hd, d_lcp,
-                         other_slots, avals, AG, other_dep, d_ghead, d_gdepth, c->d_scalars + kScalarList);
+                         other_slots, avals, AG, other_dep, d_ghead, d_gdepth,
+                         c->d_scalars + (early_refine ? kScalarSplitTotals : kScalarList));
+    }
+    if (early_refine) {
+      WP_HIP(hipEventRecord(c->evs[kEvRoundDone], st2));
+      if (n_text > 0) {
+        WP_HIP(hipStreamWaitEvent(st2, c->evs[kEvSorted], 0));
+        launch_anchors(st2);
+      }
+      WP_HIP(hipStreamWaitEvent(st, c->evs[kEvRoundDone], 0));
+      if (n_act > 0) {
+        if (n_act >= (1u << 22)) {
+          hipLaunchKernelGGL(list_rank_base_kernel, dim3(cdiv(n_act, kBlock)), dim3(kBlock), 0, st, hd, AG, d_gfirst, d_ghead, n_act);
+          store_ranks(spare_vals, hd, reinterpret_cast<uint32_t *>(hd) + list_cap + 2, reinterpret_cast<uint32_t *>(skeys), n_act);
+        } else {
+          hipLaunchKernelGGL(scatter_list_ranks_kernel, dim3(cdiv(n_act, kBlock)), dim3(kBlock), 0, st, spare_vals, hd, AG, d_gfirst,
+                             d_ghead, n_act, d_rank, n);
+        }
+        rounds = 2;
+      }
+      WP_LAUNCH_CHECK();
+      return;
     }
     join();
     if (n_act > 0) {
@@ -879,8 +945,13 @@
     uint32_t *mslot = d_mslot0, *midx = d_midx0;
     if (text_only) {
       if (M > 0) {
-        hipLaunchKernelGGL(trie_token_range_kernel, dim3(cdiv(M, kBlock)), dim3(kBlock), 0, st, d_node_of_slot, c->d_elig_node,
-                           c->d_elig_subtree, M, d_rng_lo, d_rng_hi, d_rng_long);
+        if (early_refine) {
+          hipLaunchKernelGGL(trie_token_range_list_kernel, dim3(cdiv(M, kBlock)), dim3(kBlock), 0, st, d_node_of_slot, c->d_elig_node,
+                             c->d_elig_subtree, M, d_rng_lo, d_rng_hi, d_rng_long, d_tok_group, d_ghead);
+        } else {
+          hipLaunchKernelGGL(trie_token_range_kernel, dim3(cdiv(M, kBlock)), dim3(kBlock), 0, st, d_node_of_slot, c->d_elig_node,
+                             c->d_elig_subtree, M, d_rng_lo, d_rng_hi, d_rng_long);
+        }
         hipLaunchKernelGGL(virtual_marks_kernel, dim3(cdiv(M, kBlock)), dim3(kBlock), 0, st, d_rng_lo, d_rng_hi, M, c->d_elig_id,
                            c->d_elig_info, d_mslot0, d_mid, d_minfo, d_rf, d_rb);
       }
@@ -1228,7 +1299,7 @@
       S.reserved0 = 1;
     }
 #endif
-    fetch_scalars(c, kScalarFree18);
+    fetch_scalars(c, kScalarSplitTotals);
     const size_t n_ids = n_text > 0 ? c->h_scalars[kScalarIds] : 0;
     S.n_ids = static_cast<int64_t>(n_ids);
     S.walk.n_wide_words = wide_ran ? static_cast<int64_t>(c->h_scalars[kScalarWideWords]) : 0;
@@ -1250,6 +1321,7 @@
       S.ms_walk = span(kMarkScanned, kMarkWalked);
       S.ms_total = span(kMarkStart, kMarkWalked) + S.ms_normalize;
       S.ms_radix_scatter = c->rstats.spans.resolve();
+      S.sched.ms_sort_to_scan = span(kMarkRound0, kMarkLcp);
     }
     c->d_ids = d_ids;
     c->dbg.sym = d_sym;
@@ -1271,6 +1343,7 @@
     symbols_and_keys();
     if (v->stage_timing) WP_HIP(hipEventRecord(c->ev[kMarkSymbols], st));
     sort_round0();
+    if (v->stage_timing) WP_HIP(hipEventRecord(c->ev[kMarkRound0], st));
     ranks_round0();
     refine();
     if (v->stage_timing) WP_HIP(hipEventRecord(c->ev[kMarkSorted], st));
diff --git a/wordpiece_amd/csrc/prune.h b/wordpiece_amd/csrc/prune.h
--- a/wordpiece_amd/csrc/prune.h
+++ b/wordpiece_amd/csrc/prune.h
@@ -197,6 +197,120 @@
     out.gclaim[g] = claim_slot;
     if (out.gcand) out.gcand[g] = crun;
   }
+}
+
+constexpr uint8_t kEarlyShort = 0;
+constexpr uint8_t kEarlyGroup = 1;
+constexpr uint8_t kEarlyWinner = 2;
+constexpr uint8_t kEarlyNone = 3;
+constexpr uint8_t kEarlySingle = 5;
+constexpr uint32_t kClaimNoGroup = 0xfffffffeu;
+
+template <typename SymT>
+__global__ __launch_bounds__(kBlock) void need_groups_early_kernel(size_t n, const SymT *__restrict__ sym,
+                                                                   const uint32_t *__restrict__ vocab_cps,
+                                                                   const uint32_t *__restrict__ tok_start,
+                                                                   const uint32_t *__restrict__ tok_info, int M,
+                                                                   const uint32_t *__restrict__ lut_excl, DevCode code,
+                                                                   uint32_t *__restrict__ claim, NeededList out,
+                                                                   uint32_t *__restrict__ tok_slot,
+                                                                   uint32_t *__restrict__ tok_run,
+                                                                   uint8_t *__restrict__ tok_state, CandRuns cr) {
+  const int m = static_cast<int>((static_cast<size_t>(blockIdx.x) * kBlock + threadIdx.x) >> 6);
+  if (m >= M) return;
+  uint64_t key = 0;
+  int bits = 0;
+  const uint32_t len = tok_info[m] & 0x0fffffffu;
+  const uint32_t *cps = vocab_cps + tok_start[m];
+  uint32_t whole = 0;
+  const bool is_long = wave_token_key(cps, len, lut_excl, code, key, bits, whole);
+  if (lane_id() != 0) return;
+  if (!is_long) {
+    tok_state[m] = kEarlyShort;
+    return;
+  }
+  const uint32_t s = cand_find(cr.table, cr.bits, static_cast<uint32_t>(key));
+  const bool found = wp_in_bounds(s != ~0u, kSiteCandRun) && s != ~0u;
+  const uint32_t lo = found ? cr.lo[s] : 0u, run = found ? cr.hi[s] - lo : 0u;
+  tok_slot[m] = s;
+  tok_run[m] = run;
+  if (run < 2) {
+    tok_state[m] = run ? static_cast<uint8_t>(kEarlySingle + suffix_vs_token(sym, n, cr.pos[lo], cps, len, lut_excl)) : kEarlyNone;
+    return;
+  }
+  const bool won = atomicCAS(&claim[s], kClaimEmpty, static_cast<uint32_t>(m)) == kClaimEmpty;
+  atomicMax(&out.claim_need[s], min(len, out.need_depth - 1u) + 1u);
+  if (!won) {
+    tok_state[m] = kEarlyGroup;
+    return;
+  }
+  uint32_t g = kClaimNoGroup;
+  if (whole < out.need_depth) {
+    const unsigned long long got = atomicAdd(out.totals, (1ull << 32) | static_cast<unsigned long long>(run));
+    g = static_cast<uint32_t>(got >> 32);
+    out.ghead[g] = static_cast<uint32_t>(got);
+    out.gdepth[g] = whole;
+    out.gclaim[g] = s;
+    out.gcand[g] = lo;
+  }
+  claim[s] = g;
+  tok_state[m] = kEarlyWinner;
+}
+
+__global__ __launch_bounds__(kBlock) void need_ranges_kernel(const Key0 *__restrict__ keys, size_t ns,
+                                                             const uint32_t *__restrict__ vocab_cps,
+                                                             const uint32_t *__restrict__ tok_start,
+                                                             const uint32_t *__restrict__ tok_info, int M,
+                                                             const uint32_t *__restrict__ lut_excl, DevCode code,
+                                                             const uint32_t *__restrict__ claim,
+                                                             uint32_t *__restrict__ gfirst, uint32_t *__restrict__ rng_lo,
+                                                             uint32_t *__restrict__ rng_hi, uint8_t *__restrict__ rng_long,
+                                                             uint32_t *__restrict__ tok_group) {
+  const int m = static_cast<int>((static_cast<size_t>(blockIdx.x) * kBlock + threadIdx.x) >> 6);
+  const int lane = lane_id();
+  if (m >= M) return;
+  uint64_t key = 0;
+  int bits = 0;
+  const uint32_t len = tok_info[m] & 0x0fffffffu;
+  uint32_t whole = 0;
+  const bool is_long = wave_token_key(vocab_cps + tok_start[m], len, lut_excl, code, key, bits, whole);
+  const size_t first = wave_key_lower_bound(keys, 0, ns, key, 2);
+  if (!is_long) {
+    const uint64_t step = 1ull << (kKeyBits - bits);
+    const uint64_t above = key + step;
+    const size_t ubd = (bits == 0 || (above >> kKeyBits) != 0) ? ns : wave_key_gallop(keys, first, ns, above);
+    if (lane == 0) {
+      rng_lo[m] = static_cast<uint32_t>(first);
+      rng_hi[m] = static_cast<uint32_t>(ubd);
+      rng_long[m] = 0;
+      tok_group[m] = kClaimNoGroup;
+    }
+    return;
+  }
+#ifdef WP_DEBUG_BOUNDS
+  const size_t last = wave_key_gallop(keys, first, ns, key + 1);
+#endif
+  if (lane != 0) return;
+  const uint32_t state = rng_long[m], s = rng_lo[m], run = rng_hi[m];
+#ifdef WP_DEBUG_BOUNDS
+  wp_in_bounds(run == last - first, kSiteCandRun);
+#endif
+  uint32_t lb = static_cast<uint32_t>(first), ubd = lb, g = kClaimNoGroup;
+  uint8_t lng = 0;
+  if (state == kEarlyGroup || state == kEarlyWinner) {
+    ubd = lb + run;
+    lng = 1;
+    g = claim[s];
+    if (state == kEarlyWinner && g != kClaimNoGroup) gfirst[g] = lb;
+  } else if (state != kEarlyNone) {
+    const int cmp = static_cast<int>(state) - static_cast<int>(kEarlySingle);
+    lb = cmp < 0 ? lb + 1u : lb;
+    ubd = static_cast<uint32_t>(first) + (cmp <= 0 ? 1u : 0u);
+  }
+  rng_lo[m] = lb;
+  rng_hi[m] = ubd;
+  rng_long[m] = lng;
+  tok_group[m] = g;
 }
 
 __global__ __launch_bounds__(kBlock) void needed_need_kernel(NeededList out) {
@@ -234,7 +348,7 @@
       const uint32_t md = (lo + hi) >> 1;
       if (out.ghead[md] <= p) lo = md; else hi = md;
     }
-    const uint32_t k = out.gfirst[lo] + static_cast<uint32_t>(p - out.ghead[lo]);
+    const uint32_t k = out.gfirst ? out.gfirst[lo] + static_cast<uint32_t>(p - out.ghead[lo]) : static_cast<uint32_t>(p);
     if (!wp_in_bounds(k < n, kSiteListSlot)) continue;
     uint32_t v;
     if (out.cand_pos) {
diff --git a/wordpiece_amd/csrc/suffix_array.h b/wordpiece_amd/csrc/suffix_array.h
--- a/wordpiece_amd/csrc/suffix_array.h
+++ b/wordpiece_amd/csrc/suffix_array.h
@@ -240,6 +240,27 @@
   for (int j = 0; j < kSpItems; j++) {
     if (v[j] != kRankUnchanged && wp_in_bounds(d[j] < out_n, kSiteRankStore)) out[d[j]] = v[j];
   }
+}
+
+__global__ __launch_bounds__(kBlock) void scatter_list_ranks_kernel(const uint32_t *__restrict__ dst,
+                                                                    const RankEntry *__restrict__ val,
+                                                                    const uint32_t *__restrict__ gid,
+                                                                    const uint32_t *__restrict__ gfirst,
+                                                                    const uint32_t *__restrict__ ghead, size_t m,
+                                                                    RankEntry *__restrict__ out, size_t out_n) {
+  const size_t k = static_cast<size_t>(blockIdx.x) * kBlock + threadIdx.x;
+  if (k >= m) return;
+  const uint32_t g = gid[k], d = dst[k];
+  const RankEntry v = val[k] + (gfirst[g] - ghead[g]);
+  if (wp_in_bounds(d < out_n && v < out_n, kSiteRankStore)) out[d] = v;
+}
+__global__ __launch_bounds__(kBlock) void list_rank_base_kernel(RankEntry *__restrict__ val, const uint32_t *__restrict__ gid,
+                                                                const uint32_t *__restrict__ gfirst,
+                                                                const uint32_t *__restrict__ ghead, size_t m) {
+  const size_t k = static_cast<size_t>(blockIdx.x) * kBlock + threadIdx.x;
+  if (k >= m) return;
+  const uint32_t g = gid[k];
+  val[k] += gfirst[g] - ghead[g];
 }
 
 constexpr int kWinBits = 15;
diff --git a/wordpiece_amd/csrc/trie.h b/wordpiece_amd/csrc/trie.h
--- a/wordpiece_amd/csrc/trie.h
+++ b/wordpiece_amd/csrc/trie.h
@@ -1,6 +1,7 @@
 #pragma once
 #include "decode.h"
 #include "primitives.h"
+#include "prune.h"
 
 namespace wp {
 
@@ -143,4 +144,32 @@
   rng_hi[m] = lo;
 }
 
+__global__ __launch_bounds__(kBlock) void trie_token_range_list_kernel(const uint32_t *__restrict__ node_of_entry,
+                                                                       const uint32_t *__restrict__ tok_node,
+                                                                       const uint32_t *__restrict__ tok_subtree, int M,
+                                                                       uint32_t *__restrict__ rng_lo, uint32_t *__restrict__ rng_hi,
+                                                                       const uint8_t *__restrict__ rng_long,
+                                                                       const uint32_t *__restrict__ tok_group,
+                                                                       const uint32_t *__restrict__ ghead) {
+  const int m = blockIdx.x * kBlock + threadIdx.x;
+  if (m >= M || !rng_long[m]) return;
+  const uint32_t g = tok_group[m];
+  if (g == kClaimNoGroup) return;
+  const uint32_t base = rng_lo[m], glo = ghead[g], ghi = glo + (rng_hi[m] - base);
+  const uint32_t a = tok_node[m], b = a + tok_subtree[m];
+  uint32_t lo = glo, hi = ghi;
+  while (lo < hi) {
+    const uint32_t md = lo + ((hi - lo) >> 1);
+    if (node_of_entry[md] < a) lo = md + 1; else hi = md;
+  }
+  const uint32_t first = lo;
+  hi = ghi;
+  while (lo < hi) {
+    const uint32_t md = lo + ((hi - lo) >> 1);
+    if (node_of_entry[md] < b) lo = md + 1; else hi = md;
+  }
+  rng_lo[m] = base + (first - glo);
+  rng_hi[m] = base + (lo - glo);
 }
+
+}
```

Result: faster. 31130 (median of 6 runs) (+6.4%).
